# fboehm/DBSLMM

Hardware: AMD Instinct MI355X
Metric: SNPs solved/sec (whole node) + max-|Δβ| vs CPU ref, 1M SNP × 10k indiv (higher is better)
Workload: dtype f64

## Files before the change

dbslmm_amd/__init__.py:

```python
from __future__ import annotations

import ctypes as C
from dataclasses import dataclass, field

import numpy as np

from . import _lib
from ._lib import (WORKLOAD_LEN, BLOCK_EMPTY, BLOCK_MONOMORPHIC, BLOCK_NOT_CONVERGED, BLOCK_NOT_PD,
                   BLOCK_OK, KERNEL_NAMES, SOLVER_AUTO, SOLVER_FACTOR, SOLVER_PCG, DbslmmError)

__all__ = ["Context", "Plan", "DBSLMMFIT", "BlockProblem", "bed_maf", "read_snp_std", "valid_blocks",
           "DbslmmError", "BLOCK_OK", "BLOCK_EMPTY", "BLOCK_NOT_PD", "BLOCK_MONOMORPHIC",
           "BLOCK_NOT_CONVERGED", "KERNEL_NAMES", "SOLVER_AUTO", "SOLVER_FACTOR", "SOLVER_PCG"]


def _ptr(a):
    return None if a is None else a.ctypes.data_as(C.c_void_p)


class Context:

    def __init__(self, device=0):
        self.lib = _lib.load()
        h = C.c_void_p()
        if isinstance(device, (list, tuple)):
            ids = np.ascontiguousarray(device, dtype=np.int32)
            rc = self.lib.dbslmm_ctx_create_multi(len(ids), _ptr(ids), C.byref(h))
        else:
            rc = self.lib.dbslmm_ctx_create(int(device), C.byref(h))
        if rc != 0:
            raise DbslmmError(f"dbslmm_ctx_create(device={device}) failed rc={rc}")
        self.h = h
        self.device = device

    @property
    def num_devices(self) -> int:
        return int(self.lib.dbslmm_ctx_num_devices(self.h))

    def cache_bed(self, bed):
        if bed is None:
            self._cached_bed = None
            self.check(self.lib.dbslmm_ctx_cache_bed(self.h, None, 0), "ctx_cache_bed")
            return
        b = np.ascontiguousarray(bed, dtype=np.uint8)
        self.check(self.lib.dbslmm_ctx_cache_bed(self.h, _ptr(b), b.size), "ctx_cache_bed")
        self._cached_bed = b

    def row_stats(self, bed, n_ref: int, n_rows: int) -> np.ndarray:
        b = np.ascontiguousarray(bed, dtype=np.uint8)
        out = np.zeros((n_rows, 3), dtype=np.int32)
        self.check(self.lib.dbslmm_bed_row_stats(self.h, _ptr(b), b.size, n_ref, n_rows, _ptr(out)),
                   "bed_row_stats")
        return out

    def check(self, rc: int, what: str):
        if rc != 0:
            msg = self.lib.dbslmm_last_error(self.h).decode(errors="replace")
            raise DbslmmError(f"{what} failed rc={rc}: {msg}")

    def close(self):
        if self.h:
            self.lib.dbslmm_ctx_destroy(self.h)
            self.h = None

    def __del__(self):
        try:
            self.close()
        except Exception:
            pass


@dataclass
class BlockProblem:
    bed: np.ndarray
    n_ref: int
    n_obs: int
    sigma_s: float
    s_ptr: np.ndarray
    s_pos: np.ndarray
    z_s: np.ndarray
    l_ptr: np.ndarray | None = None
    l_pos: np.ndarray | None = None
    z_l: np.ndarray | None = None
    tau: float = 0.8
    opts: dict = field(default_factory=dict)

    def __post_init__(self):
        self.bed = np.ascontiguousarray(self.bed, dtype=np.uint8)
        self.s_ptr = np.ascontiguousarray(self.s_ptr, dtype=np.int64)
        self.s_pos = np.ascontiguousarray(self.s_pos, dtype=np.int32)
        self.z_s = np.ascontiguousarray(self.z_s, dtype=np.float64)
        if self.l_ptr is not None:
            self.l_ptr = np.ascontiguousarray(self.l_ptr, dtype=np.int64)
            self.l_pos = np.ascontiguousarray(self.l_pos, dtype=np.int32)
            self.z_l = np.ascontiguousarray(self.z_l, dtype=np.float64)
        nb = len(self.s_ptr) - 1
        if self.l_ptr is not None and len(self.l_ptr) != nb + 1:
            raise ValueError("s_ptr and l_ptr must have the same number of blocks")

    @property
    def num_block(self) -> int:
        return len(self.s_ptr) - 1

    @property
    def n_s(self) -> int:
        return int(self.s_ptr[-1])

    @property
    def n_l(self) -> int:
        return 0 if self.l_ptr is None else int(self.l_ptr[-1])

    def c_struct(self) -> _lib.Problem:
        unknown = set(self.opts) - {f[0] for f in _lib.Options._fields_}
        if unknown:
            raise ValueError(f"unknown dbslmm_options fields: {sorted(unknown)}")
        self._opts = _lib.Options(**self.opts)
        return _lib.Problem(
            _ptr(self.bed), self.bed.size, self.n_ref, self.n_obs, self.sigma_s, self.tau,
            self.num_block, _ptr(self.s_ptr), _ptr(self.s_pos), _ptr(self.z_s),
            _ptr(self.l_ptr), _ptr(self.l_pos), _ptr(self.z_l), C.pointer(self._opts))


class Plan:

    def __init__(self, ctx: Context, prob: BlockProblem):
        self.ctx, self.prob = ctx, prob
        self._cs = prob.c_struct()
        h = C.c_void_p()
        ctx.check(ctx.lib.dbslmm_plan_create(ctx.h, C.byref(self._cs), C.byref(h)), "plan_create")
        self.h = h

    @classmethod
    def units(cls, ctx: Context, prob: BlockProblem, unit_device, device_index: int):
        self = cls.__new__(cls)
        self.ctx, self.prob = ctx, prob
        ud = np.ascontiguousarray(unit_device, dtype=np.int32)
        if ud.ndim != 2 or ud.shape[0] != prob.num_block:
            raise ValueError("unit_device: [num_block, n_copies]")
        self._cs = prob.c_struct()
        self._ud = ud
        h = C.c_void_p()
        ctx.check(ctx.lib.dbslmm_plan_create_units(ctx.h, C.byref(self._cs), ud.shape[1], _ptr(ud),
                                                   int(device_index), C.byref(h)), "plan_create_units")
        self.h = h
        return self

    def run(self):
        self.ctx.check(self.ctx.lib.dbslmm_plan_run(self.h), "plan_run")

    def sync(self):
        self.ctx.check(self.ctx.lib.dbslmm_plan_sync(self.h), "plan_sync")

    def set_sigma(self, sigma_s: float):
        self.ctx.check(self.ctx.lib.dbslmm_plan_set_sigma(self.h, float(sigma_s)), "plan_set_sigma")

    def run_multi(self, sigmas, out=None):
        p = self.prob
        sig = np.ascontiguousarray(sigmas, dtype=np.float64)
        n = len(sig)
        if out is not None:
            bs, bl, st = out
            if (bs.shape != (n, p.n_s) or bl.shape != (n, p.n_l) or st.shape != (n, p.num_block)
                    or bs.dtype != np.float64 or bl.dtype != np.float64 or st.dtype != np.int32
                    or not all(a.flags.c_contiguous for a in out)):
                raise ValueError("out: C-contiguous float64 (n, n_s), (n, n_l) and int32 (n, num_block)")
        else:
            bs = np.zeros((n, p.n_s))
            bl = np.zeros((n, p.n_l))
            st = np.zeros((n, p.num_block), dtype=np.int32)
        self.ctx.check(self.ctx.lib.dbslmm_plan_run_multi(self.h, _ptr(sig), n, _ptr(bs), _ptr(bl),
                                                          _ptr(st)), "plan_run_multi")
        return [(bs[i], bl[i], st[i]) for i in range(n)]

    def enable_timing(self, on: bool = True):
        self.ctx.check(self.ctx.lib.dbslmm_plan_enable_timing(self.h, int(on)), "plan_enable_timing")

    def kernel_ms(self):
        out = np.zeros(len(KERNEL_NAMES))
        n = np.zeros(1, dtype=np.int32)
        self.ctx.check(self.ctx.lib.dbslmm_plan_kernel_ms(self.h, _ptr(out), _ptr(n)), "plan_kernel_ms")
        return out, int(n[0])

    def workload(self) -> dict:
        w = np.zeros(WORKLOAD_LEN)
        self.ctx.check(self.ctx.lib.dbslmm_plan_workload(self.h, _ptr(w)), "plan_workload")
        keys = ("snps", "unpack_read_bytes", "unpack_write_bytes", "gram_ops_alg",
                "gram_ops_exec", "chol_flops_large", "blocks", "gram_tiles", "chol_flops_small",
                "blocks_large", "chol_flops_tiled", "blocks_tiled", "tiled_launches", "trsv_bytes",
                "cheb_iters", "cheb_base", "h2f_pass_bytes", "pcg_route", "pcg_iters", "pcg_chip_bytes",
                "pcg_partial_bytes", "pcg_block_bytes")
        return dict(zip(keys, w.tolist()))

    def block_iters(self) -> np.ndarray:
        out = np.zeros(max(1, self.prob.num_block), dtype=np.int32)
        self.ctx.check(self.ctx.lib.dbslmm_plan_block_iters(self.h, _ptr(out)), "plan_block_iters")
        return out[:self.prob.num_block]

    def shard_info(self) -> np.ndarray:
        out = np.zeros(self.prob.num_block, dtype=np.int32)
        self.ctx.check(self.ctx.lib.dbslmm_plan_shard_info(self.h, _ptr(out)), "plan_shard_info")
        return out

    def block_matrix(self, block: int, copy: int = 0) -> np.ndarray:
        ld = C.c_int32()
        self.ctx.check(self.ctx.lib.dbslmm_plan_block_matrix(self.h, int(block), int(copy), None,
                                                             C.byref(ld)), "plan_block_matrix")
        out = np.empty((ld.value, ld.value))
        self.ctx.check(self.ctx.lib.dbslmm_plan_block_matrix(self.h, int(block), int(copy), _ptr(out),
                                                             None), "plan_block_matrix")
        return out

    def download(self):
        p = self.prob
        bs = np.zeros(p.n_s)
        bl = np.zeros(p.n_l)
        st = np.zeros(p.num_block, dtype=np.int32)
        self.ctx.check(self.ctx.lib.dbslmm_plan_download(self.h, _ptr(bs), _ptr(bl), _ptr(st)),
                       "plan_download")
        return bs, bl, st

    def variance(self, test_bed: np.ndarray, indicator, s_pos, l_pos=None) -> np.ndarray:
        tb = np.ascontiguousarray(test_bed, dtype=np.uint8)
        ind = np.ascontiguousarray(indicator, dtype=np.int32)
        sp = np.ascontiguousarray(s_pos, dtype=np.int32)
        lp = None if l_pos is None else np.ascontiguousarray(l_pos, dtype=np.int32)
        if sp.size != self.prob.n_s or (self.prob.n_l and (lp is None or lp.size != self.prob.n_l)):
            raise ValueError("test s_pos / l_pos must align with the plan's small / large SNPs")
        n_test = int((ind != 0).sum())
        out = np.zeros(n_test * self.prob.num_block)
        nt = np.zeros(1, dtype=np.int32)
        tp = _lib.TestPanel(_ptr(tb), tb.size, ind.size, _ptr(ind), _ptr(sp), _ptr(lp))
        self.ctx.check(self.ctx.lib.dbslmm_plan_variance(self.h, C.byref(tp), _ptr(out), _ptr(nt)),
                       "plan_variance")
        return out.reshape(self.prob.num_block, n_test).T

    def close(self):
        if self.h:
            self.ctx.lib.dbslmm_plan_destroy(self.h)
            self.h = None

    def __del__(self):
        try:
            self.close()
        except Exception:
            pass


class DBSLMMFIT:

    def __init__(self, device=0):
        self.ctx = Context(device)

    def est(self, prob: BlockProblem):
        bs = np.zeros(prob.n_s)
        bl = np.zeros(prob.n_l)
        st = np.zeros(prob.num_block, dtype=np.int32)
        cs = prob.c_struct()
        self.ctx.check(self.ctx.lib.dbslmm_est(self.ctx.h, C.byref(cs), _ptr(bs), _ptr(bl), _ptr(st)),
                       "dbslmm_est")
        return bs, bl, st


def bed_maf(ctx: Context, bed: np.ndarray, n_ref: int, n_snp: int) -> np.ndarray:
    bed = np.ascontiguousarray(bed, dtype=np.uint8)
    maf = np.zeros(n_snp)
    ctx.check(ctx.lib.dbslmm_bed_maf(ctx.h, _ptr(bed), bed.size, n_ref, n_snp, _ptr(maf)), "bed_maf")
    return maf


def read_snp_std(ctx: Context, bed: np.ndarray, n_ref: int, rows) -> tuple[np.ndarray, np.ndarray]:
    bed = np.ascontiguousarray(bed, dtype=np.uint8)
    rows = np.ascontiguousarray(rows, dtype=np.int32)
    out = np.zeros(n_ref * len(rows))
    maf = np.zeros(len(rows))
    ctx.check(ctx.lib.dbslmm_read_snp_std(ctx.h, _ptr(bed), bed.size, n_ref, _ptr(rows), len(rows),
                                          _ptr(out), _ptr(maf)), "read_snp_std")
    return out.reshape(len(rows), n_ref).T, maf


def valid_blocks(ctx: Context, bed: np.ndarray, n_ref: int, ptr, pos, z1, z2):
    bed = np.ascontiguousarray(bed, dtype=np.uint8)
    ptr = np.ascontiguousarray(ptr, dtype=np.int64)
    pos = np.ascontiguousarray(pos, dtype=np.int32)
    z1 = np.ascontiguousarray(z1, dtype=np.float64)
    z2 = np.ascontiguousarray(z2, dtype=np.float64)
    nb = len(ptr) - 1
    nume = np.zeros(nb)
    deno = np.zeros(nb)
    ctx.check(ctx.lib.dbslmm_valid_blocks(ctx.h, _ptr(bed), bed.size, n_ref, nb, _ptr(ptr), _ptr(pos),
                                          _ptr(z1), _ptr(z2), _ptr(nume), _ptr(deno)), "valid_blocks")
    return nume, deno
```

dbslmm_amd/_lib.py:

```python
from __future__ import annotations

import ctypes as C
import os

HERE = os.path.dirname(os.path.abspath(__file__))
LIB_PATH = os.path.join(HERE, "libdbslmm_hip.so")

EXPORTS = (
    "dbslmm_abi_version", "dbslmm_ctx_create", "dbslmm_ctx_destroy", "dbslmm_last_error",
    "dbslmm_est", "dbslmm_plan_create", "dbslmm_plan_run", "dbslmm_plan_sync",
    "dbslmm_plan_download", "dbslmm_plan_set_sigma", "dbslmm_plan_destroy", "dbslmm_plan_run_multi",
    "dbslmm_plan_enable_timing", "dbslmm_plan_kernel_ms", "dbslmm_plan_workload",
    "dbslmm_bed_maf", "dbslmm_read_snp_std", "dbslmm_valid_blocks", "dbslmm_plan_variance",
    "dbslmm_ctx_create_multi", "dbslmm_ctx_num_devices", "dbslmm_plan_shard_info",
    "dbslmm_ctx_cache_bed", "dbslmm_ctx_cache_bed_fd", "dbslmm_plan_block_matrix",
    "dbslmm_shard_plan", "dbslmm_plan_create_units", "dbslmm_shard_plan_problem",
    "dbslmm_plan_block_iters", "dbslmm_bed_row_stats",
)

ABI_VERSION = 16
K_UNPACK, K_GRAM, K_CHOL_LARGE, K_CHOL_SMALL, K_CHOL_TILED, K_TRSV, K_PCG, K_PCG_BLOCK = 0, 1, 2, 3, 4, 5, 6, 7
KERNEL_NAMES = ("dbslmm_unpack_stats", "dbslmm_gram", "dbslmm_chol_large", "dbslmm_chol_small",
                "dbslmm_tchol", "dbslmm_trsv", "dbslmm_pcg", "dbslmm_pcg_block")
WORKLOAD_LEN = 22
BLOCK_OK, BLOCK_EMPTY, BLOCK_NOT_PD, BLOCK_MONOMORPHIC, BLOCK_NOT_CONVERGED = 0, 1, 2, 3, 4
SOLVER_AUTO, SOLVER_FACTOR, SOLVER_PCG = 0, 1, 2


class Options(C.Structure):
    _fields_ = [
        ("tiled_min", C.c_int32), ("gram_big_min", C.c_int32), ("gram_huge_min", C.c_int32),
        ("h2f_mode", C.c_int32), ("cheb_tol", C.c_double), ("lead_min", C.c_int32),
        ("large_cheb", C.c_int32), ("cheb_fused", C.c_int32), ("debug_delay_us", C.c_int32),
        ("debug_stop", C.c_int32), ("sub_split", C.c_int32), ("sub_grid_lead", C.c_int32),
        ("sub_grid_rest", C.c_int32), ("shard_copies", C.c_int32), ("h2f_iter", C.c_int32),
        ("solver", C.c_int32), ("pcg_tol", C.c_double), ("pcg_maxit", C.c_int32),
        ("pcg_whole", C.c_int32),
    ]


class Problem(C.Structure):
    _fields_ = [
        ("bed", C.c_void_p), ("bed_len", C.c_int64), ("n_ref", C.c_int32), ("n_obs", C.c_int32),
        ("sigma_s", C.c_double), ("tau", C.c_double), ("num_block", C.c_int32),
        ("s_ptr", C.c_void_p), ("s_pos", C.c_void_p), ("z_s", C.c_void_p),
        ("l_ptr", C.c_void_p), ("l_pos", C.c_void_p), ("z_l", C.c_void_p),
        ("opts", C.POINTER(Options)),
    ]


class TestPanel(C.Structure):
    _fields_ = [
        ("bed", C.c_void_p), ("bed_len", C.c_int64), ("n_total", C.c_int32),
        ("indicator", C.c_void_p), ("s_pos", C.c_void_p), ("l_pos", C.c_void_p),
    ]


_lib = None


class DbslmmError(RuntimeError):
    pass


def load(path: str | None = None):
    global _lib
    if _lib is not None:
        return _lib
    p = path or os.environ.get("DBSLMM_LIB_PATH") or LIB_PATH
    if not os.path.exists(p):
        raise DbslmmError(f"{p} not found: build it with `python -c 'import __graft_entry__ as g; g.build()'`"
                          " (or `make -C dbslmm_amd/csrc`)")
    L = C.CDLL(p)
    V, P = C.c_void_p, C.POINTER
    L.dbslmm_abi_version.restype = C.c_int
    L.dbslmm_ctx_create.argtypes = [C.c_int, P(V)]
    L.dbslmm_ctx_create_multi.argtypes = [C.c_int32, V, P(V)]
    L.dbslmm_ctx_num_devices.argtypes = [V]
    L.dbslmm_plan_shard_info.argtypes = [V, V]
    L.dbslmm_ctx_destroy.argtypes = [V]
    L.dbslmm_ctx_destroy.restype = None
    L.dbslmm_last_error.argtypes = [V]
    L.dbslmm_last_error.restype = C.c_char_p
    L.dbslmm_est.argtypes = [V, P(Problem), V, V, V]
    L.dbslmm_plan_create.argtypes = [V, P(Problem), P(V)]
    L.dbslmm_plan_run.argtypes = [V]
    L.dbslmm_plan_sync.argtypes = [V]
    L.dbslmm_plan_download.argtypes = [V, V, V, V]
    L.dbslmm_plan_set_sigma.argtypes = [V, C.c_double]
    L.dbslmm_plan_run_multi.argtypes = [V, V, C.c_int32, V, V, V]
    L.dbslmm_plan_destroy.argtypes = [V]
    L.dbslmm_plan_destroy.restype = None
    L.dbslmm_plan_enable_timing.argtypes = [V, C.c_int]
    L.dbslmm_plan_kernel_ms.argtypes = [V, V, V]
    L.dbslmm_plan_workload.argtypes = [V, V]
    L.dbslmm_bed_maf.argtypes = [V, V, C.c_int64, C.c_int32, C.c_int64, V]
    L.dbslmm_bed_row_stats.argtypes = [V, V, C.c_int64, C.c_int32, C.c_int64, V]
    L.dbslmm_read_snp_std.argtypes = [V, V, C.c_int64, C.c_int32, V, C.c_int32, V, V]
    L.dbslmm_valid_blocks.argtypes = [V, V, C.c_int64, C.c_int32, C.c_int32, V, V, V, V, V, V]
    L.dbslmm_plan_variance.argtypes = [V, P(TestPanel), V, V]
    L.dbslmm_ctx_cache_bed.argtypes = [V, V, C.c_int64]
    L.dbslmm_ctx_cache_bed_fd.argtypes = [V, C.c_int, C.c_int64, V]
    L.dbslmm_shard_plan.argtypes = [C.c_int32, V, C.c_int32, C.c_int32, C.c_int32, V, V]
    L.dbslmm_plan_create_units.argtypes = [V, P(Problem), C.c_int32, V, C.c_int32, P(V)]
    L.dbslmm_shard_plan_problem.argtypes = [P(Problem), V, C.c_int32, C.c_int32, V, V]
    L.dbslmm_plan_block_iters.argtypes = [V, V]
    if hasattr(L, "dbslmm_plan_block_matrix"):
        L.dbslmm_plan_block_matrix.argtypes = [V, C.c_int32, C.c_int32, V, V]
    if L.dbslmm_abi_version() != ABI_VERSION:
        raise DbslmmError("ABI version mismatch")
    _lib = L
    return L
```

dbslmm_amd/csrc/pcg.hip:

```cpp
#include <hip/hip_runtime.h>
#include <stdint.h>

namespace pcg {
constexpr int kT = 128;
constexpr int kRunMax = 8;
constexpr int kMaxNC = 4;
constexpr int kWaves = 4;
constexpr int kVS = kT + 8;
constexpr int kNDot = 5;
constexpr int kQS = 8;
constexpr int kThreads = 256;
constexpr int kFTb = 8;
constexpr int kFRows = kFTb * kT;
constexpr int kFPer = kFRows / kThreads;
constexpr int wave_lds_doubles(int nc) { return 3 * nc * kVS + 4 * nc * 64; }
constexpr size_t lds_bytes(int nc) { return sizeof(double) * kWaves * wave_lds_doubles(nc); }
}

struct PcgBlk {
    int32_t blk, row0, m, ms;
    int32_t ld, Tb, Ns, sco;
    int64_t matoff, vo, po, dof;
    int64_t off16;
    int32_t nc;
    int32_t mshift;
    int32_t fused;
    int32_t pad_;
};

struct PcgArgs {
    const PcgBlk* blk;
    const uint16_t* G16;
    const double* M;
    const int32_t* flags;
    const double* S;
    const double* rsd;
    const double* z;
    const int32_t* slot_out;
    const int32_t* blk_id;
    const double* dshift;
    double *X, *R, *P, *Sv, *W;
    double* U;
    double* part;
    double* dot;
    double* qs;
    int32_t* cnv;
    int32_t* itb;
    int32_t* done;
    int32_t* active;
    double* beta_s;
    double* beta_l;
    int32_t* status;
    int64_t vstride;
    int64_t ns, nl, nbk;
    double tau, rn, c0, tol, inv_sqrt_n;
    int32_t ncopy;
    int32_t run;
    int32_t seed;
};

namespace pcg {

__device__ __forceinline__ void wave_fence() {
    __builtin_amdgcn_fence(__ATOMIC_RELEASE, "wavefront");
    __builtin_amdgcn_wave_barrier();
    __builtin_amdgcn_fence(__ATOMIC_ACQUIRE, "wavefront");
}

template <int Ctrl>
__device__ __forceinline__ double dpp_mov(double v) {
    const uint64_t b = __builtin_bit_cast(uint64_t, v);
    const int lo = __builtin_amdgcn_mov_dpp(static_cast<int>(b & 0xffffffffu), Ctrl, 0xf, 0xf, false);
    const int hi = __builtin_amdgcn_mov_dpp(static_cast<int>(b >> 32), Ctrl, 0xf, 0xf, false);
    return __builtin_bit_cast(double, (static_cast<uint64_t>(static_cast<uint32_t>(hi)) << 32) | static_cast<uint32_t>(lo));
}
template <int X>
__device__ __forceinline__ uint32_t swap_xor(uint32_t x, bool up) {
    if constexpr (X == 16) {
        const auto r = __builtin_amdgcn_permlane16_swap(x, x, false, false);
        return up ? r[0] : r[1];
    } else {
        const auto r = __builtin_amdgcn_permlane32_swap(x, x, false, false);
        return up ? r[0] : r[1];
    }
}
template <int X>
__device__ __forceinline__ double lane_xor(double v) {
#ifndef PCG_NO_DPP
    if constexpr (X == 1) return dpp_mov<0xB1>(v);
    else if constexpr (X == 2) return dpp_mov<0x4E>(v);
    else if constexpr (X == 4) return dpp_mov<0x1B>(dpp_mov<0x141>(v));
    else if constexpr (X == 8) return dpp_mov<0x128>(v);
#ifndef PCG_NO_PERMLANE
    else if constexpr (X == 16 || X == 32) {
        const uint64_t b = __builtin_bit_cast(uint64_t, v);
        const bool up = (__lane_id() & X) != 0;
        const uint32_t lo = swap_xor<X>(static_cast<uint32_t>(b & 0xffffffffu), up);
        const uint32_t hi = swap_xor<X>(static_cast<uint32_t>(b >> 32), up);
        return __builtin_bit_cast(double, (static_cast<uint64_t>(hi) << 32) | lo);
    }
#endif
    else
#endif
        return __shfl_xor(v, X);
}

template <int X2, int X1, int X0>
__device__ __forceinline__ double rscatter8(const double (&v)[8], int lane) {
    const bool h2 = (lane & X2) != 0, h1 = (lane & X1) != 0, h0 = (lane & X0) != 0;
    double u[4], w[2];
#pragma unroll
    for (int q = 0; q < 4; ++q) {
        const double send = h2 ? v[q] : v[q + 4], keep = h2 ? v[q + 4] : v[q];
        u[q] = keep + lane_xor<X2>(send);
    }
#pragma unroll
    for (int q = 0; q < 2; ++q) {
        const double send = h1 ? u[q] : u[q + 2], keep = h1 ? u[q + 2] : u[q];
        w[q] = keep + lane_xor<X1>(send);
    }
    const double send = h0 ? w[0] : w[1], keep = h0 ? w[1] : w[0];
    return keep + lane_xor<X0>(send);
}

__device__ __forceinline__ double wave_sum(double v) {
    v += lane_xor<32>(v);
    v += lane_xor<16>(v);
    v += lane_xor<8>(v);
    v += lane_xor<4>(v);
    v += lane_xor<2>(v);
    v += lane_xor<1>(v);
    return v;
}



__device__ __forceinline__ double ordered_sum(const double* __restrict__ p, int64_t st, int s0, int s1, double acc) {
    for (int s = s0; s < s1; s += 8) {
        double t[8];
#pragma unroll
        for (int u = 0; u < 8; ++u) t[u] = s + u < s1 ? p[static_cast<int64_t>(s + u) * st] : 0.0;
#pragma unroll
        for (int u = 0; u < 8; ++u) acc += t[u];
    }
    return acc;
}

__device__ __forceinline__ bool on_u16(const PcgArgs& a, const PcgBlk& B) {
    return a.G16 != nullptr && (a.flags[B.blk] & 1) == 0;
}

__device__ __forceinline__ double jdiag(const PcgArgs& a, const PcgBlk& B, int i, double dc) {
    return B.mshift ? 1.0 : i < B.ms ? a.c0 + dc : a.c0;
}
__device__ __forceinline__ double col_shift(const PcgArgs& a, const PcgBlk& B, int k) {
    return a.dshift[B.mshift ? a.seed : k];
}

__device__ __forceinline__ double cvt_lo(uint32_t w) {
    double g;
    uint32_t t;
    asm volatile("v_and_b32 %1, 0xffff, %2\n\tv_cvt_f64_u32 %0, %1" : "=v"(g), "=&v"(t) : "v"(w));
    return g;
}
__device__ __forceinline__ double cvt_hi(uint32_t w) {
    double g;
    uint32_t t;
    asm volatile("v_lshrrev_b32 %1, 16, %2\n\tv_cvt_f64_u32 %0, %1" : "=v"(g), "=&v"(t) : "v"(w));
    return g;
}

typedef uint32_t pcg_u4 __attribute__((ext_vector_type(4)));

__device__ __forceinline__ __amdgpu_buffer_rsrc_t g16_rsrc(const uint16_t* base, uint32_t bytes) {
    const uint64_t gb = reinterpret_cast<uint64_t>(base);
    const uint32_t lo = static_cast<uint32_t>(__builtin_amdgcn_readfirstlane(static_cast<int>(gb & 0xffffffffu)));
    const uint32_t hi = static_cast<uint32_t>(__builtin_amdgcn_readfirstlane(static_cast<int>(gb >> 32)));
    const int nb = __builtin_amdgcn_readfirstlane(static_cast<int>(bytes));
    return __builtin_amdgcn_make_buffer_rsrc(reinterpret_cast<void*>((static_cast<uint64_t>(hi) << 32) | lo),
                                             static_cast<short>(0), nb, 0x00020000);
}
constexpr uint32_t kG16Oob = 0x80000000u;

__device__ __forceinline__ void quad_mul16(const pcg_u4 (&raw)[8], bool diagq, int lane, int nc,
                                           const double* vI, const double* vJ, double* rsum, double* csum) {
    const int rg = lane >> 3, cg = lane & 7;
#pragma unroll 1
    for (int k = 0; k < nc; ++k) {
        double vi[8], vj[8], racc[8], cacc[8];
#pragma unroll
        for (int q = 0; q < 8; ++q) {
            vi[q] = vI[k * kVS + 8 * rg + q];
            vj[q] = vJ[k * kVS + 8 * cg + q];
            racc[q] = cacc[q] = 0.0;
        }
        if (!diagq) {
#pragma unroll
            for (int r = 0; r < 8; ++r)
#pragma unroll
                for (int c = 0; c < 8; ++c) {
                    const uint32_t w = raw[r][c >> 1];
                    const double g = (c & 1) ? cvt_hi(w) : cvt_lo(w);
                    racc[r] = __builtin_fma(g, vj[c], racc[r]);
                    cacc[c] = __builtin_fma(g, vi[r], cacc[c]);
                }
        } else {
#pragma unroll
            for (int r = 0; r < 8; ++r)
#pragma unroll
                for (int c = 0; c < 8; ++c) {
                    const uint32_t w = raw[r][c >> 1];
                    const double g = (c & 1) ? cvt_hi(w) : cvt_lo(w);
                    const int dd = 8 * (cg - rg) + c - r;
                    racc[r] = __builtin_fma(dd <= 0 ? g : 0.0, vj[c], racc[r]);
                    cacc[c] = __builtin_fma(dd < 0 ? g : 0.0, vi[r], cacc[c]);
                }
        }
        rsum[k * 64 + lane] += rscatter8<4, 2, 1>(racc, lane);
        csum[k * 64 + lane] += rscatter8<32, 16, 8>(cacc, lane);
    }
}

__device__ __forceinline__ void quad_mul64(const double* __restrict__ base, int64_t ld, int rows_ok, int cols_ok,
                                           bool diagq, int lane, int nc, const double* vI, const double* vJ,
                                           double* rsum, double* csum) {
    const int rg = lane >> 3, cg = lane & 7;
#pragma unroll 1
    for (int k = 0; k < nc; ++k) {
        double vi[8], vj[8], racc[8], cacc[8];
#pragma unroll
        for (int q = 0; q < 8; ++q) {
            vi[q] = vI[k * kVS + 8 * rg + q];
            vj[q] = vJ[k * kVS + 8 * cg + q];
            racc[q] = cacc[q] = 0.0;
        }
#pragma unroll 1
        for (int r = 0; r < 8; ++r)
#pragma unroll
            for (int c = 0; c < 8; ++c) {
                const double g = (r < rows_ok && c < cols_ok) ? base[r * ld + c] : 0.0;
                const int dd = 8 * (cg - rg) + c - r;
                const double gr = !diagq || dd <= 0 ? g : 0.0, gc = !diagq || dd < 0 ? g : 0.0;
#pragma unroll
                for (int q = 0; q < 8; ++q)
                    if (q == r) racc[q] = __builtin_fma(gr, vj[c], racc[q]);
                cacc[c] = __builtin_fma(gc, vi[r], cacc[c]);
            }
        rsum[k * 64 + lane] += rscatter8<4, 2, 1>(racc, lane);
        csum[k * 64 + lane] += rscatter8<32, 16, 8>(cacc, lane);
    }
}

__device__ __forceinline__ void stage_v(const PcgArgs& a, const PcgBlk& B, int T, int nc, int lane, double* v) {
    for (int k = 0; k < nc; ++k) {
        const double* src = a.U + k * a.vstride + B.vo + static_cast<int64_t>(T) * kT;
        const double x0 = src[lane], x1 = src[lane + 64];
        v[k * kVS + lane] = x0;
        v[k * kVS + lane + 64] = x1;
    }
}

__device__ __forceinline__ bool quad_active(const PcgBlk& B, int I, int J, int q) {
    const int qi = q >> 1, qj = q & 1;
    return !(J == I && qj > qi) && I * kT + 64 * qi < B.m && J * kT + 64 * qj < B.m;
}
__device__ __forceinline__ bool next_quad(const PcgBlk& B, int I, int J1, int& J, int& q) {
    for (;;) {
        if (++q == 4) {
            q = 0;
            if (++J > J1) return false;
        }
        if (quad_active(B, I, J, q)) return true;
    }
}

template <bool U16>
__device__ void symv_item(const PcgArgs& a, int4 item, int lane, double* vI, double* vJb, double* rsum,
                          double* csum) {
    const PcgBlk B = a.blk[item.x];
    if (a.done[item.x] || on_u16(a, B) != U16) return;
    const int I = item.y, J0 = item.z, J1 = item.w, nc = B.nc;
    const int64_t ld16 = static_cast<int64_t>(B.Tb) * kT;
    const int rg = lane >> 3, cg = lane & 7;
    auto vj_of = [&](int J) -> double* { return J == I ? vI : vJb + ((J - J0) & 1) * nc * kVS; };
    const __amdgpu_buffer_rsrc_t g16 =
        g16_rsrc(a.G16 + B.off16 + static_cast<int64_t>(I) * kT * ld16, U16 ? static_cast<uint32_t>(kT * ld16 * 2) : 0u);
    auto load = [&](int J, int q, pcg_u4 (&raw)[8], bool none) {
        if constexpr (U16) {
            const int i0 = 64 * (q >> 1) + 8 * rg, j0 = J * kT + 64 * (q & 1) + 8 * cg;
            const bool skip = none || j0 >= B.m || (J == I && (q == 0 || q == 3) && cg > rg);
            const uint32_t o = static_cast<uint32_t>((static_cast<int64_t>(i0) * ld16 + j0) * 2);
#pragma unroll
            for (int r = 0; r < 8; ++r)
                raw[r] = __builtin_amdgcn_raw_buffer_load_b128(
                    g16, (skip || I * kT + i0 + r >= B.m) ? kG16Oob : o + static_cast<uint32_t>(r * ld16 * 2), 0, 0);
        }
    };
    auto mult = [&](int J, int q, const pcg_u4 (&raw)[8]) {
        const int qi = q >> 1, qj = q & 1;
        const bool dq = J == I && qi == qj;
        const double* vj = vj_of(J);
        double* rs = rsum + qi * nc * 64;
        double* cs = csum + qj * nc * 64;
        if constexpr (U16) {
            quad_mul16(raw, dq, lane, nc, vI + 64 * qi, vj + 64 * qj, rs, cs);
        } else {
            const int ib = I * kT + 64 * qi + 8 * rg, jb = J * kT + 64 * qj + 8 * cg;
            quad_mul64(a.M + B.matoff + static_cast<int64_t>(ib) * B.ld + jb, B.ld, B.m - ib, B.m - jb, dq,
                       lane, nc, vI + 64 * qi, vj + 64 * qj, rs, cs);
        }
    };
    auto flush = [&](int J) {
        double* dst = a.part + B.po + (static_cast<int64_t>(J) * B.Ns + I) * nc * kT;
        for (int qj = 0; qj < 2; ++qj)
            for (int k = 0; k < nc; ++k) {
                dst[k * kT + 64 * qj + 8 * cg + rg] = csum[(qj * nc + k) * 64 + lane];
                csum[(qj * nc + k) * 64 + lane] = 0.0;
            }
    };
    pcg_u4 ra[8], rb[8];
    int J = J0, q = 0;
    load(J, q, ra, false);
    stage_v(a, B, I, nc, lane, vI);
    if (J != I) stage_v(a, B, J, nc, lane, vj_of(J));
    for (int t = 0; t < 2 * nc; ++t) rsum[t * 64 + lane] = csum[t * 64 + lane] = 0.0;
    wave_fence();
    auto step = [&](pcg_u4 (&cur)[8], pcg_u4 (&nxt)[8]) -> bool {
        int Jn = J, qn = q;
        const bool more = next_quad(B, I, J1, Jn, qn);
        load(more ? Jn : J, more ? qn : q, nxt, !more);
        if (more && Jn != J && Jn != I) stage_v(a, B, Jn, nc, lane, vj_of(Jn));
        mult(J, q, cur);
        if (!more || Jn != J) flush(J);
        wave_fence();
        J = Jn;
        q = qn;
        return more;
    };
    while (step(ra, rb) && step(rb, ra)) {
    }
    double* dst = a.part + B.po + (static_cast<int64_t>(I) * B.Ns + B.Tb + J0 / a.run) * nc * kT;
    for (int qi = 0; qi < 2; ++qi)
        for (int k = 0; k < nc; ++k) dst[k * kT + 64 * qi + 8 * rg + cg] = rsum[(qi * nc + k) * 64 + lane];
}

}

extern "C" __global__ __launch_bounds__(pcg::kThreads) void dbslmm_pcg_init(PcgArgs a, const int2* __restrict__ rows) {
    using namespace pcg;
    __shared__ double red[kThreads / 64][kMaxNC];
    __shared__ int mono_s;
    const int2 it = rows[blockIdx.x];
    const int bi = it.x, I = it.y, tid = threadIdx.x;
    const PcgBlk B = a.blk[bi];
    const bool u16 = on_u16(a, B);
    const int n = a.ncopy, nc = B.nc;
    if (I == 0) {
        if (tid == 0) mono_s = 0;
        __syncthreads();
        bool mono = false;
        for (int i = tid; i < B.m; i += kThreads) mono |= !(a.rsd[B.row0 + i] < INFINITY);
        if (mono) atomicOr(&mono_s, 1);
        __syncthreads();
        if (tid < n) {
            a.cnv[B.sco + tid] = 0;
            double* q = a.qs + static_cast<int64_t>(B.sco + tid) * kQS;
            q[4] = q[5] = 1.0;
        }
        if (tid == 0) {
            a.itb[bi] = 0;
            const bool fz = B.fused && u16;
            a.done[bi] = mono_s ? 2 : fz ? 3 : 0;
            if (!mono_s && !fz) atomicAdd(a.active, 1);
        }
    }
    const int r = tid & (kT - 1), h = tid >> 7, i = I * kT + r;
    const bool in = i < B.m;
    double sv[kMaxNC];
#pragma unroll
    for (int k = 0; k < kMaxNC; ++k) sv[k] = 0.0;
    for (int c = h; c < n; c += 2) {
        const int64_t o = c * a.vstride + B.vo + i;
        const double rhs = in ? a.z[B.row0 + i] : 0.0;
        a.X[o] = 0.0;
        a.P[o] = 0.0;
        if (c < nc) {
            a.Sv[o] = 0.0;
            a.W[o] = 0.0;
            a.R[o] = rhs;
            double uv = 0.0;
            if (in) {
                uv = rhs / jdiag(a, B, i, col_shift(a, B, c));
                if (u16) uv *= a.rsd[B.row0 + i];
            }
            a.U[o] = uv;
        }
    }
#pragma unroll
    for (int k = 0; k < kMaxNC; ++k)
        if (k < nc && (k & 1) == h && in && u16) {
            const double rhs = a.z[B.row0 + i];
            sv[k] = a.S[B.row0 + i] * a.rsd[B.row0 + i] * (rhs / jdiag(a, B, i, col_shift(a, B, k)));
        }
#pragma unroll
    for (int k = 0; k < kMaxNC; ++k) sv[k] = wave_sum(sv[k]);
    if ((tid & 63) == 0)
#pragma unroll
        for (int k = 0; k < kMaxNC; ++k) red[tid >> 6][k] = sv[k];
    __syncthreads();
    if (tid < nc) {
        const int hk = tid & 1;
        a.dot[B.dof + (static_cast<int64_t>(I) * kNDot + 4) * n + tid] = red[2 * hk][tid] + red[2 * hk + 1][tid];
    }
}

template <bool U16>
__device__ __forceinline__ void symv_body(const PcgArgs& a, const int4* __restrict__ items, int32_t n_items) {
    using namespace pcg;
    extern __shared__ double vlds[];
    const int wave = threadIdx.x >> 6, lane = threadIdx.x & 63;
    const int e = blockIdx.x * kWaves + wave;
    if (e >= n_items) return;
    const int nc = a.ncopy;
    double* w = vlds + wave * wave_lds_doubles(nc);
    symv_item<U16>(a, items[e], lane, w, w + nc * kVS, w + 3 * nc * kVS, w + 3 * nc * kVS + 2 * nc * 64);
}
#ifndef PCG_SYMV_WAVES
#define PCG_SYMV_WAVES 2
#endif
extern "C" __global__ __launch_bounds__(pcg::kThreads) __attribute__((amdgpu_waves_per_eu(PCG_SYMV_WAVES, 8)))
void dbslmm_pcg_symv16(PcgArgs a, const int4* __restrict__ items, int32_t n_items) {
    symv_body<true>(a, items, n_items);
}
extern "C" __global__ __launch_bounds__(pcg::kThreads)
void dbslmm_pcg_symv64(PcgArgs a, const int4* __restrict__ items, int32_t n_items) {
    symv_body<false>(a, items, n_items);
}

extern "C" __global__ __launch_bounds__(pcg::kThreads) void dbslmm_pcg_rows(PcgArgs a, const int2* __restrict__ rows) {
    using namespace pcg;
    __shared__ double red[kThreads / 64][kMaxNC][4];
    __shared__ double sig[kMaxNC];
    const int2 it = rows[blockIdx.x];
    const int bi = it.x, I = it.y, tid = threadIdx.x;
    if (a.done[bi]) return;
    const PcgBlk B = a.blk[bi];
    const bool u16 = on_u16(a, B);
    const int n = a.ncopy, nc = B.nc;
    if (tid < nc)
        sig[tid] = ordered_sum(a.dot + B.dof + 4 * n + tid, kNDot * n, 0, B.Tb, 0.0);
    __syncthreads();
    const int r = tid & (kT - 1), h = tid >> 7, i = I * kT + r;
    const bool in = i < B.m;
    const double Si = in ? a.S[B.row0 + i] : 0.0, ri = in ? a.rsd[B.row0 + i] : 0.0;
    const int nrun = (I + a.run) / a.run;
    double dv[kMaxNC][4];
#pragma unroll
    for (int k = 0; k < kMaxNC; ++k)
#pragma unroll
        for (int f = 0; f < 4; ++f) dv[k][f] = 0.0;
#pragma unroll
    for (int k = 0; k < kMaxNC; ++k) {
        if (k >= n || (k & 1) != h) continue;
        const int64_t o = k * a.vstride + B.vo + i;
        if (k < nc) {
            const double* pp = a.part + B.po + static_cast<int64_t>(I) * B.Ns * nc * kT + k * kT + r;
            double y = ordered_sum(pp, nc * kT, I, B.Tb, 0.0);
            y = ordered_sum(pp, nc * kT, B.Tb, B.Tb + nrun, y);
            const double dc = col_shift(a, B, k);
            const double rv = a.R[o];
            const double u = in ? rv / jdiag(a, B, i, dc) : 0.0;
            const double sh = i < B.ms ? dc : 0.0;
            double w = 0.0;
            if (in) {
                if (u16) w = a.tau * a.rn * ri * __builtin_fma(-Si, sig[k] * a.rn, y) + (1.0 - a.tau + sh) * u;
                else w = y + sh * u;
            }
            a.W[o] = w;
            dv[k][0] = rv * u;
            dv[k][1] = w * u;
            dv[k][2] = rv * rv;
        }
        const double xv = a.X[o];
        dv[k][3] = xv * xv;
    }
#pragma unroll
    for (int k = 0; k < kMaxNC; ++k)
#pragma unroll
        for (int f = 0; f < 4; ++f) dv[k][f] = wave_sum(dv[k][f]);
    if ((tid & 63) == 0)
#pragma unroll
        for (int k = 0; k < kMaxNC; ++k)
#pragma unroll
            for (int f = 0; f < 4; ++f) red[tid >> 6][k][f] = dv[k][f];
    __syncthreads();
    if (tid < 4 * n) {
        const int k = tid >> 2, f = tid & 3, hk = k & 1;
        if (f == 3 || k < nc)
            a.dot[B.dof + (static_cast<int64_t>(I) * kNDot + f) * n + k] = red[2 * hk][k][f] + red[2 * hk + 1][k][f];
    }
    if (I == 0 && tid == 0) a.itb[bi] += 1;
}

extern "C" __global__ __launch_bounds__(pcg::kThreads) void dbslmm_pcg_update(PcgArgs a, const int2* __restrict__ rows) {
    using namespace pcg;
    __shared__ double tot[kMaxNC][4];
    __shared__ double coef[kMaxNC][3];
    __shared__ double seedc[2];
    __shared__ int run_s[kMaxNC];
    __shared__ double red[kThreads / 64][kMaxNC];
    const int2 it = rows[blockIdx.x];
    const int bi = it.x, I = it.y, tid = threadIdx.x;
    if (a.done[bi]) return;
    const PcgBlk B = a.blk[bi];
    const bool u16 = on_u16(a, B);
    const int n = a.ncopy, nc = B.nc;
    const int itn = a.itb[bi] - 1;
    const int par = itn & 1;
    if (tid < 4 * n) {
        const int k = tid >> 2, f = tid & 3;
        tot[k][f] = (f == 3 || k < nc) ? ordered_sum(a.dot + B.dof + f * n + k, kNDot * n, 0, B.Tb, 0.0) : 0.0;
    }
    __syncthreads();
    if (B.mshift) {
        if (tid == 0) {
            const double gam = tot[0][0], del = tot[0][1];
            const double* q = a.qs + static_cast<int64_t>(B.sco) * kQS;
            double al, be = 0.0;
            if (itn == 0) {
                al = gam / del;
            } else {
                be = gam / q[2 * par];
                al = gam / (del - be * gam / q[2 * par + 1]);
            }
            seedc[0] = al;
            seedc[1] = be;
        }
        __syncthreads();
        if (tid < n) {
            const int c = tid;
            double* q = a.qs + static_cast<int64_t>(B.sco + c) * kQS;
            const double al = seedc[0], be = seedc[1];
            const double zk = q[4 + 2 * par], zk1 = q[4 + 2 * par + 1];
            const double rr = tot[0][2] * zk * zk, xx = tot[c][3];
            const double t = a.tol * (a.dshift[c] + 1.0 - a.tau);
            const bool conv = a.cnv[B.sco + c] != 0 || rr == 0.0 || rr <= t * t * xx;
            const double e = a.dshift[c] - a.dshift[a.seed];
            const double cp = itn == 0 ? 0.0 : al * be / a.qs[static_cast<int64_t>(B.sco) * kQS + 2 * par + 1];
            const double zn = zk * zk1 / ((1.0 + cp + al * e) * zk1 - cp * zk);
            coef[c][0] = al * zn / zk;
            coef[c][1] = zk1 != 0.0 ? (zk / zk1) * (zk / zk1) * be : 0.0;
            coef[c][2] = zk;
            run_s[c] = conv ? 0 : 1;
            if (I == 0) {
                if (conv && a.cnv[B.sco + c] == 0) a.cnv[B.sco + c] = itn + 1;
                q[4 + 2 * (par ^ 1)] = zn;
                q[4 + 2 * (par ^ 1) + 1] = zk;
            }
        }
        __syncthreads();
        if (I == 0 && tid == 0) {
            double* q = a.qs + static_cast<int64_t>(B.sco) * kQS;
            q[2 * (par ^ 1)] = tot[0][0];
            q[2 * (par ^ 1) + 1] = seedc[0];
        }
    } else {
        if (tid < n) {
            const int k = tid;
            const double gam = tot[k][0], del = tot[k][1], rr = tot[k][2], xx = tot[k][3];
            const double lam = B.ms == B.m ? a.dshift[k] + 1.0 - a.tau : 1.0 - a.tau;
            const double t = a.tol * lam;
            const bool conv = a.cnv[B.sco + k] != 0 || rr == 0.0 || rr <= t * t * xx;
            double al = 0.0, be = 0.0;
            if (!conv) {
                double* q = a.qs + static_cast<int64_t>(B.sco + k) * kQS;
                if (itn == 0) {
                    al = gam / del;
                } else {
                    be = gam / q[2 * par];
                    al = gam / (del - be * gam / q[2 * par + 1]);
                }
                if (I == 0) {
                    q[2 * (par ^ 1)] = gam;
                    q[2 * (par ^ 1) + 1] = al;
                }
            } else if (I == 0 && a.cnv[B.sco + k] == 0) {
                a.cnv[B.sco + k] = itn + 1;
            }
            coef[k][0] = al;
            coef[k][1] = be;
            coef[k][2] = 1.0;
            run_s[k] = conv ? 0 : 1;
        }
        __syncthreads();
    }
    int running = 0;
    for (int k = 0; k < n; ++k) running += run_s[k];
    if (running == 0) {
        if (I == 0 && tid == 0) {
            a.done[bi] = 1;
            atomicSub(a.active, 1);
        }
        return;
    }
    const int r = tid & (kT - 1), h = tid >> 7, i = I * kT + r;
    const bool in = i < B.m;
    double sv[kMaxNC];
#pragma unroll
    for (int k = 0; k < kMaxNC; ++k) sv[k] = 0.0;
    if (B.mshift) {
        if (in) {
            const int64_t o0 = B.vo + i;
            const double rv = a.R[o0];
#pragma unroll
            for (int c = 0; c < kMaxNC; ++c) {
                if (c >= n || (c & 1) != h || !run_s[c]) continue;
                const int64_t o = c * a.vstride + o0;
                const double p = __builtin_fma(coef[c][1], a.P[o], coef[c][2] * rv);
                a.P[o] = p;
                a.X[o] = __builtin_fma(coef[c][0], p, a.X[o]);
            }
            if (h == 0) {
                const double al = seedc[0], be = seedc[1];
                const double sn = __builtin_fma(be, a.Sv[o0], a.W[o0]);
                const double rn = __builtin_fma(-al, sn, rv);
                a.Sv[o0] = sn;
                a.R[o0] = rn;
                a.U[o0] = u16 ? rn * a.rsd[B.row0 + i] : rn;
                if (u16) sv[0] = a.S[B.row0 + i] * a.rsd[B.row0 + i] * rn;
            }
        }
    } else {
#pragma unroll
        for (int k = 0; k < kMaxNC; ++k) {
            if (k >= n || (k & 1) != h || !run_s[k] || !in) continue;
            const int64_t o = k * a.vstride + B.vo + i;
            const double al = coef[k][0], be = coef[k][1];
            const double dg = jdiag(a, B, i, a.dshift[k]);
            const double u = a.R[o] / dg;
            const double p = __builtin_fma(be, a.P[o], u);
            const double s = __builtin_fma(be, a.Sv[o], a.W[o]);
            const double x = __builtin_fma(al, p, a.X[o]);
            const double rn = __builtin_fma(-al, s, a.R[o]);
            a.P[o] = p;
            a.Sv[o] = s;
            a.X[o] = x;
            a.R[o] = rn;
            a.U[o] = u16 ? (rn / dg) * a.rsd[B.row0 + i] : rn / dg;
            if (u16) sv[k] = a.S[B.row0 + i] * a.rsd[B.row0 + i] * (rn / dg);
        }
    }
#pragma unroll
    for (int k = 0; k < kMaxNC; ++k) sv[k] = wave_sum(sv[k]);
    if ((tid & 63) == 0)
#pragma unroll
        for (int k = 0; k < kMaxNC; ++k) red[tid >> 6][k] = sv[k];
    __syncthreads();
    if (tid < nc && (B.mshift || run_s[tid])) {
        const int hk = tid & 1;
        a.dot[B.dof + (static_cast<int64_t>(I) * kNDot + 4) * n + tid] = red[2 * hk][tid] + red[2 * hk + 1][tid];
    }
}

#ifndef PCG_BLOCK_DEPTH
#define PCG_BLOCK_DEPTH 3
#endif
namespace pcg {
template <int N>
__device__ __forceinline__ void block_sum(double (&v)[N], double* red, int tid) {
#pragma unroll
    for (int k = 0; k < N; ++k) v[k] = wave_sum(v[k]);
    __syncthreads();
    if ((tid & 63) == 0)
#pragma unroll
        for (int k = 0; k < N; ++k) red[(tid >> 6) * N + k] = v[k];
    __syncthreads();
#pragma unroll
    for (int k = 0; k < N; ++k) v[k] = ((red[k] + red[N + k]) + red[2 * N + k]) + red[3 * N + k];
}
constexpr size_t block_lds_bytes(int n) {
    return sizeof(double) * ((5 + 2 * n) * kFRows + 4 * (3 + kMaxNC) + 12 + 3 * kMaxNC + 4);
}
}

__device__ __forceinline__ void pcg_block_solve(const PcgArgs& a, int bi, int cc, int32_t maxit) {
    using namespace pcg;
    extern __shared__ double blds[];
    double* yw = blds;
    double* Ul = blds + 4 * kFRows;
    const int n = a.ncopy;
    double* Xl = Ul + kFRows;
    double* Pl = Xl + n * kFRows;
    double* red = Pl + n * kFRows;
    if (a.done[bi] != 3) return;
    const PcgBlk B = a.blk[bi];
    const int tid = threadIdx.x, lane = tid & 63, wave = tid >> 6;
    const int m = B.m, Tb = B.Tb;
    const bool msh = cc < 0;
    const int nx = msh ? n : 1;
    const double dc = msh ? col_shift(a, B, 0) : a.dshift[cc];
    double r[kFPer], sv[kFPer], wv[kFPer], Sr[kFPer], Rr[kFPer], sg[1] = {0.0};
#pragma unroll
    for (int q = 0; q < kFPer; ++q) {
        const int i = tid + kThreads * q;
        const bool in = i < m;
        r[q] = in ? a.z[B.row0 + i] : 0.0;
        Sr[q] = in ? a.S[B.row0 + i] : 0.0;
        Rr[q] = in ? a.rsd[B.row0 + i] : 0.0;
        sv[q] = wv[q] = 0.0;
        double u = 0.0;
        if (in) {
            u = (r[q] / jdiag(a, B, i, dc)) * Rr[q];
            sg[0] += Sr[q] * u;
        }
        Ul[i] = u;
        for (int w = 0; w < 4; ++w) yw[w * kFRows + i] = 0.0;
        for (int c = 0; c < nx; ++c) Xl[c * kFRows + i] = Pl[c * kFRows + i] = 0.0;
    }
    block_sum(sg, red, tid);
    double sig = sg[0];
    const int Q = (m + 63) / 64;
    const int nq = Q * (Q + 1) / 2;
    const int64_t ld16 = static_cast<int64_t>(Tb) * kT;
    const int rg = lane >> 3, cg = lane & 7;
    auto quad_of = [&](int t, int& qi, int& qj) {
        qi = static_cast<int>((sqrtf(8.0f * t + 1.0f) - 1.0f) * 0.5f);
        while (qi * (qi + 1) / 2 > t) --qi;
        while ((qi + 1) * (qi + 2) / 2 <= t) ++qi;
        qj = t - qi * (qi + 1) / 2;
    };
    const __amdgpu_buffer_rsrc_t g16 = g16_rsrc(a.G16 + B.off16, static_cast<uint32_t>(ld16 * ld16 * 2));
    auto load = [&](int t, pcg_u4 (&raw)[8]) {
        int qi, qj;
        quad_of(t, qi, qj);
        const int r0 = 64 * qi + 8 * rg, c0 = 64 * qj + 8 * cg;
        const bool skip = t >= nq || c0 >= m || (qi == qj && cg > rg);
        const uint32_t o = static_cast<uint32_t>((r0 * static_cast<int>(ld16) + c0) * 2);
#pragma unroll
        for (int rr = 0; rr < 8; ++rr)
            raw[rr] = __builtin_amdgcn_raw_buffer_load_b128(
                g16, (skip || r0 + rr >= m) ? kG16Oob : o + static_cast<uint32_t>(rr * ld16 * 2), 0, 0);
    };
    auto mult = [&](int t, const pcg_u4 (&raw)[8]) {
        int qi, qj;
        quad_of(t, qi, qj);
        const bool dq = qi == qj;
        double vi[8], vj[8], racc[8], cacc[8];
#pragma unroll
        for (int q = 0; q < 8; ++q) {
            vi[q] = Ul[64 * qi + 8 * rg + q];
            vj[q] = Ul[64 * qj + 8 * cg + q];
            racc[q] = cacc[q] = 0.0;
        }
        if (!dq) {
// ... 36 lines not shown
    for (; it < maxit; ++it) {
        __syncthreads();
        {
#if PCG_BLOCK_DEPTH == 3
            pcg_u4 ra[8], rb[8], rc[8];
            int t = wave;
            load(t, ra);
            load(t + 4, rb);
            while (t < nq) {
                load(t + 8, rc);
                mult(t, ra);
                t += 4;
                if (t >= nq) break;
                load(t + 8, ra);
                mult(t, rb);
                t += 4;
                if (t >= nq) break;
                load(t + 8, rb);
                mult(t, rc);
                t += 4;
            }
#else
            pcg_u4 ra[8], rb[8];
            int t = wave;
            load(t, ra);
            while (t < nq) {
                load(t + 4, rb);
                mult(t, ra);
                t += 4;
                if (t >= nq) break;
                load(t + 4, ra);
                mult(t, rb);
                t += 4;
            }
#endif
        }
        __syncthreads();
        double d[3 + kMaxNC];
#pragma unroll
        for (int k = 0; k < 3 + kMaxNC; ++k) d[k] = 0.0;
#pragma unroll
        for (int q = 0; q < kFPer; ++q) {
            const int i = tid + kThreads * q;
            double y = 0.0;
            if (i < Tb * kT) {
                y = ((yw[i] + yw[kFRows + i]) + yw[2 * kFRows + i]) + yw[3 * kFRows + i];
#pragma unroll
                for (int w = 0; w < 4; ++w) yw[w * kFRows + i] = 0.0;
            }
            if (i < m) {
                const double Si = Sr[q], ri = Rr[q];
                const double u = r[q] / jdiag(a, B, i, dc);
                const double sh = i < B.ms ? dc : 0.0;
                const double w = a.tau * a.rn * ri * __builtin_fma(-Si, sig * a.rn, y) + (1.0 - a.tau + sh) * u;
                wv[q] = w;
                d[0] += r[q] * u;
                d[1] += w * u;
                d[2] += r[q] * r[q];
                for (int c = 0; c < nx; ++c) {
                    const double xv = Xl[c * kFRows + i];
                    d[3 + c] += xv * xv;
                }
            }
        }
        block_sum(d, red, tid);
        if (tid == 0) {
            const double gam = d[0], del = d[1], rr = d[2];
            double al, be = 0.0;
            if (it == 0) {
                al = gam / del;
            } else {
                be = gam / st[0];
                al = gam / (del - be * gam / st[1]);
            }
            int running = 0;
            if (msh) {
                const double cp = it == 0 ? 0.0 : al * be / st[1];
                for (int c = 0; c < n; ++c) {
                    const double zk = st[4 + c], zk1 = st[8 + c];
                    const double t = a.tol * (a.dshift[c] + 1.0 - a.tau);
                    const double rrc = rr * zk * zk;
                    if (!flag[c] && (rrc == 0.0 || rrc <= t * t * d[3 + c])) {
                        flag[c] = 1;
                        a.cnv[B.sco + c] = it + 1;
                    }
                    const double e = a.dshift[c] - a.dshift[a.seed];
                    const double zn = zk * zk1 / ((1.0 + cp + al * e) * zk1 - cp * zk);
                    st[12 + 3 * c] = al * zn / zk;
                    st[12 + 3 * c + 1] = zk1 != 0.0 ? (zk / zk1) * (zk / zk1) * be : 0.0;
                    st[12 + 3 * c + 2] = zk;
                    st[8 + c] = zk;
                    st[4 + c] = zn;
                    running += flag[c] ? 0 : 1;
                }
            } else {
                const double lam = B.ms == B.m ? dc + 1.0 - a.tau : 1.0 - a.tau;
                const double t = a.tol * lam;
                if (rr == 0.0 || rr <= t * t * d[3]) {
                    flag[0] = 1;
                    a.cnv[B.sco + cc] = it + 1;
                }
                running = flag[0] ? 0 : 1;
            }
            st[0] = gam;
            st[1] = al;
            st[2] = al;
            st[3] = be;
            flag[kMaxNC] = running;
        }
        __syncthreads();
        if (flag[kMaxNC] == 0) break;
        const double al = st[2], be = st[3];
        double sg2[1] = {0.0};
#pragma unroll
        for (int q = 0; q < kFPer; ++q) {
            const int i = tid + kThreads * q;
            if (i >= m) continue;
            const double rsd_i = Rr[q];
            double rn;
            if (msh) {
                for (int c = 0; c < n; ++c) {
                    if (flag[c]) continue;
                    const int o = c * kFRows + i;
                    const double pv = __builtin_fma(st[12 + 3 * c + 1], Pl[o], st[12 + 3 * c + 2] * r[q]);
                    Pl[o] = pv;
                    Xl[o] = __builtin_fma(st[12 + 3 * c], pv, Xl[o]);
                }
                const double sn = __builtin_fma(be, sv[q], wv[q]);
                rn = __builtin_fma(-al, sn, r[q]);
                sv[q] = sn;
                r[q] = rn;
                Ul[i] = rn * rsd_i;
            } else {
                const double dg = jdiag(a, B, i, dc);
                const double u = r[q] / dg;
                const double pv = __builtin_fma(be, Pl[i], u);
                const double sn = __builtin_fma(be, sv[q], wv[q]);
                Pl[i] = pv;
                Xl[i] = __builtin_fma(al, pv, Xl[i]);
                rn = __builtin_fma(-al, sn, r[q]);
                sv[q] = sn;
                r[q] = rn;
                Ul[i] = (rn / dg) * rsd_i;
            }
            sg2[0] += Sr[q] * Ul[i];
        }
        block_sum(sg2, red, tid);
        sig = sg2[0];
    }
#pragma unroll
    for (int q = 0; q < kFPer; ++q) {
        const int i = tid + kThreads * q;
        if (i < m)
            for (int c = 0; c < nx; ++c) a.X[(msh ? c : cc) * a.vstride + B.vo + i] = Xl[c * kFRows + i];
    }
    if (tid == 0) atomicMax(a.itb + bi, it + (it < maxit ? 1 : 0));
}

extern "C" __global__ __launch_bounds__(pcg::kThreads)
#if PCG_BLOCK_DEPTH == 3
__attribute__((amdgpu_waves_per_eu(1, 8), amdgpu_num_vgpr(312)))
#else
__attribute__((amdgpu_waves_per_eu(2, 8)))
#endif
void dbslmm_pcg_block(PcgArgs a, const int2* __restrict__ list, int32_t n_list, int32_t* __restrict__ next,
                      int32_t maxit) {
    __shared__ int e_s;
    for (;;) {
        __syncthreads();
        if (threadIdx.x == 0) e_s = atomicAdd(next, 1);
        __syncthreads();
        const int e = e_s;
        if (e >= n_list) break;
        pcg_block_solve(a, list[e].x, list[e].y, maxit);
    }
}

extern "C" __global__ __launch_bounds__(pcg::kThreads) void dbslmm_pcg_final(PcgArgs a, const int2* __restrict__ rows) {
    using namespace pcg;
    const int2 it = rows[blockIdx.x];
    const int bi = it.x, I = it.y, tid = threadIdx.x;
    const PcgBlk B = a.blk[bi];
    const bool mono = a.done[bi] == 2;
    const int r = tid & (kT - 1), h = tid >> 7, i = I * kT + r;
    if (i < B.m) {
        const int so = a.slot_out[B.row0 + i];
        for (int k = h; k < a.ncopy; k += 2) {
            const double bv = mono ? __builtin_nan("") : a.X[k * a.vstride + B.vo + i] * a.inv_sqrt_n;
            if (so >= 0) a.beta_s[k * a.ns + so] = bv;
            else a.beta_l[k * a.nl - 1 - so] = bv;
        }
    }
    if (I == 0 && tid < a.ncopy) {
        const int st = mono ? DBSLMM_BLOCK_MONOMORPHIC
                            : a.cnv[B.sco + tid] == 0 ? DBSLMM_BLOCK_NOT_CONVERGED : DBSLMM_BLOCK_OK;
        a.status[tid * a.nbk + a.blk_id[B.blk]] = st;
    }
}
```

dbslmm_amd/csrc/plan.hip:

```cpp
#include <hip/hip_runtime.h>
#include <unistd.h>

#include <algorithm>
#include <atomic>
#include <cmath>
#include <condition_variable>
#include <cstdio>
#include <cstdlib>
#include <cstring>
#include <numeric>
#include <string>
#include <memory>
#include <mutex>
#include <chrono>
#include <thread>
#include <unordered_map>
#include <vector>

#include "../../include/dbslmm_hip.h"

#include "kernels.hip"
#include "chol.hip"
#include "chol_tiled.hip"
#include "variance.hip"
#include "trsv.hip"
#include "pcg.hip"

namespace {
constexpr int kEvPerRun = 12;
constexpr size_t kCholLargeLds = sizeof(double) * chol::kLargeDoubles;
constexpr size_t kCholChebLds = sizeof(double) * chol::kChebLdsDoubles;
constexpr size_t kTiledLds = sizeof(double) * chol::kTiledDoubles;
constexpr size_t kRegionLds = sizeof(double) * chol::kRegionDoubles;
constexpr size_t kTrail3Lds = sizeof(double) * chol::kTrail3k16Doubles;
constexpr int kTiledMinDefault = 384;
constexpr int kTiledMinSmall = 256;
constexpr int kBedPad = 64;
constexpr int kGramBigMinDefault = 96;
constexpr int kGramHugeMinDefault = 384;
constexpr int kTChebMaxM = 4096;
constexpr int kLeadMinDefault = 1536;
constexpr int kXcd = 8;
constexpr int kEpochsPerRun = 1 << 14;

struct TLaunch {
    int kind;
    int step;
    int32_t off;
    int32_t n;
    int32_t items;
    int32_t nk = 1;
    int strm = 0;
};
constexpr int kTlRecord = 6, kTlWait = 7;
constexpr int kSuper = 2;
constexpr int kWideSuper = 4;
constexpr int kWideMin = 4096;
constexpr int kTiledMaxM = 255 * 128;
constexpr int kGramSq = 4;
constexpr int kTrailSq = 8;

int64_t round_up(int64_t x, int64_t a) { return (x + a - 1) / a * a; }
struct PanelImage {
    std::shared_ptr<uint8_t> mem;
    int64_t pitch = 0;
    int32_t n_rows = 0, n_ref = 0;
    int64_t image_bytes() const { return (static_cast<int64_t>(n_rows) + 1) * pitch; }
    const v4i* rows() const { return reinterpret_cast<const v4i*>(mem.get() + image_bytes()); }
};
std::mutex g_capture_mu;
}

struct dbslmm_ctx {
    int device = 0;
    hipStream_t stream = nullptr;
    hipStream_t stream2 = nullptr;
    hipStream_t stream3 = nullptr;
    hipStream_t stream4 = nullptr, stream5 = nullptr;
    hipEvent_t fork = nullptr, join = nullptr, join3 = nullptr, fork2 = nullptr, join4 = nullptr;
    int n_cu = 256;
    std::string err;
    const uint8_t* bed_host = nullptr;
    int64_t bed_host_len = 0;
    std::shared_ptr<uint8_t> bed_cache;
    PanelImage img_cache;
    bool bed_from_fd = false;
    std::vector<dbslmm_ctx*> subs;
    std::thread setup;
    std::mutex setup_mu;
    bool setup_ok = true;
};
struct dbslmm_plan;
struct DeviceShard {
    dbslmm_plan* plan = nullptr;
    dbslmm_ctx* ctx = nullptr;
    dbslmm_ctx* own_ctx = nullptr;
    int device_index = 0;
    int copy = -1;
    std::vector<int32_t> blocks;
    std::vector<int64_t> s_idx, l_idx;
    std::vector<int> run_copies;
    std::vector<double> dl_s, dl_l;
    std::vector<int32_t> dl_st;
};
struct dbslmm_mplan {
    std::vector<DeviceShard> shards;
    int32_t n_copies = 1;
    bool partial = false;
    std::vector<int32_t> unit_device;
};

struct dbslmm_plan {
    dbslmm_ctx* ctx = nullptr;
    dbslmm_mplan* mp = nullptr;
    int32_t n_ref = 0, n_obs = 0, num_block = 0;
    double sigma_s = 0.0, tau = 0.8;
    int64_t n_s = 0, n_l = 0, kpad = 0, bed_len = 0;
    int32_t n_slots = 0, n_nonempty = 0, n_tiles = 0;
    int64_t M_elems = 0;
    PanelImage img;
    const uint8_t* d_img = nullptr;
    int32_t *d_slot_pos = nullptr, *d_slot_block = nullptr, *d_slot_out = nullptr;
    double *d_z = nullptr, *d_S = nullptr, *d_mu = nullptr, *d_rsd = nullptr, *d_y = nullptr;
    int32_t *d_flags = nullptr, *d_status = nullptr, *d_order = nullptr, *d_blk_id = nullptr;
    int32_t n_large = 0, n_small = 0;
    int32_t n_tiled = 0;
    int32_t* d_tlist = nullptr;
    std::vector<TLaunch> tl;
    std::vector<TLaunch> tl_rest;
    hipGraphExec_t graph_exec = nullptr;
    int32_t *d_row0 = nullptr, *d_m = nullptr, *d_ms = nullptr, *d_ld = nullptr;
    int64_t* d_matoff = nullptr;
    GramTile* d_tiles = nullptr;
    GramTile* d_btiles = nullptr;
    int32_t n_btiles = 0;
    GramTile* d_htiles = nullptr;
    int32_t n_htiles = 0;
    int32_t n_htiles_lead = 0;
    int32_t n_htiles_tiled = 0;
    bool early_fork = false;
    double* d_M = nullptr;
    double *d_beta_s = nullptr, *d_beta_l = nullptr;
    double* d_dshift = nullptr;
    int32_t n_copies = 0;
    int64_t nbk = 1;
    std::vector<TLaunch> tl_multi;
    int32_t* d_tlist_multi = nullptr;
    int32_t multi_n = 0;
    hipGraphExec_t graph_multi = nullptr;
    int32_t var_copy = 0;
    std::vector<int32_t> h_ld;
    std::vector<int32_t> h_m;
    std::vector<int32_t> h_tb;
    std::vector<int32_t> h_empty;
    std::vector<int32_t> h_blk_id;
    std::vector<int64_t> h_matoff;
    void* h_pin = nullptr;
    size_t h_pin_bytes = 0;
    std::vector<int32_t> h_slot_out;
    double sigma_run = 0.0;
    double wl[DBSLMM_WORKLOAD_LEN] = {0};
    bool timing = false;
    std::vector<hipEvent_t> ev;
    std::vector<hipEvent_t> dl_ev;
    std::vector<hipEvent_t> tev;
    std::vector<hipEvent_t> tev_rest;
    int32_t *d_tri_f = nullptr, *d_tri_b = nullptr, *d_foff = nullptr, *d_tflags = nullptr, *d_tb = nullptr;
    int32_t n_titems = 0, n_tflags = 0;
    int32_t* d_tepi = nullptr;
    int32_t* d_cheb_items = nullptr;
    int32_t n_cheb_items = 0, cheb_items_K = -1;
    int32_t trsv_epoch = 0;
    int32_t tiled_min = 0;
    int32_t h2f_mode = 0;
    double cheb_tol = 1e-9;
    bool large_cheb_ok = true;
    bool cheb_fused = false;
    bool h2f_cg = false;
    double* d_cgrec = nullptr;
    int32_t* d_cgconv = nullptr;
    int32_t* d_cgit = nullptr;
    bool cg_ran = false;
    int32_t debug_delay_us = 0;
    int32_t debug_stop = 0;
    int64_t n_runs = 0;
    bool sub_split = false;
    int32_t n_titems_lead = 0, n_tb_lead = 0, sub_grid_lead = 0, sub_grid_rest = 0;
    bool sub_block = false;
    int32_t* d_tcheb_blocks = nullptr;
    int32_t n_tcheb = 0, tcheb_vld = 0;
    bool trsv_pending = false;
    bool trsv_failed = false;
    unsigned long long* d_stamps = nullptr;
    double* d_cheb = nullptr;
    double* d_coef = nullptr;
    int32_t coef_cap = 0;
    std::vector<double> h_coef;
    std::vector<hipGraphExec_t> graph_copy;
    std::vector<hipGraphExec_t> graph_rest;
    int32_t cheb_base = -1;
    bool cheb_pending_var = false;
    int runs_pending = 0;
    double ms_acc[DBSLMM_K_COUNT] = {0, 0, 0, 0, 0, 0};
    int32_t ms_runs = 0;
    bool ran = false;
    bool stopped = false;
    int32_t m_copies = 0;
    std::vector<int32_t> h_ms, h_row0;
    bool has_large = false;
    int32_t solver = 0;
    double pcg_tol = 1e-12;
    int32_t pcg_maxit = 1000;
    bool force_factor = false;
    bool pcg_g16 = false;
    int32_t pcg_m_blocks = -1;
    uint16_t* d_G16 = nullptr;
    int64_t* d_off16 = nullptr;
    int32_t* d_ld16 = nullptr;
    std::vector<int64_t> h_off16;
    int32_t pcg_n = 0;
    PcgBlk* d_pblk = nullptr;
    int4* d_pitem = nullptr;
    int2* d_prow = nullptr;
    int32_t n_pblk = 0, n_pitem = 0, n_prow = 0;
    int32_t n_pitem_chip = 0, n_prow_chip = 0;
    bool pcg_trim = false;
    int32_t pcg_run = pcg::kRunMax;
    bool pcg_fused = true;
    int2* d_pflist = nullptr;
    int32_t* d_pfnext = nullptr;
    int32_t n_pflist = 0;
    std::vector<char> h_pfused;
    std::vector<int32_t> h_pnseq;
    bool pcg_join = false;
    double *d_pvec = nullptr, *d_ppart = nullptr, *d_pdot = nullptr, *d_pqs = nullptr;
    int32_t *d_pcnv = nullptr, *d_pitb = nullptr, *d_pdone = nullptr, *d_pact = nullptr;
    int64_t pcg_vstride = 0;
    int32_t* h_pmon = nullptr;
    int32_t pcg_it = 0;
    int32_t pcg_need = -1;
    int32_t pcg_iters_max = 0;
    bool pcg_pending = false;
    bool pcg_ran = false;
    bool pcg_pending_var = false;
    std::vector<char> run_route;
    std::vector<double> h_pmat, h_ppart;
    std::vector<char> h_pmiss;
    double pcg_cbytes = 0.0, pcg_pbytes = 0.0, pcg_fbytes = 0.0;
    PcgArgs pcg_args{};
    hipEvent_t pcg_ev_end = nullptr;
};

#define HIP_TRY(ctx, expr)                                                               \
    do {                                                                                 \
        hipError_t e_ = (expr);                                                          \
        if (e_ != hipSuccess) {                                                          \
            (ctx)->err = std::string(#expr) + " (plan.hip:" + std::to_string(__LINE__) + "): " + \
                         hipGetErrorString(e_);                                          \
            return DBSLMM_E_HIP;                                                         \
        }                                                                                \
    } while (0)

#define ARG_CHECK(ctx, cond, msg)                   \
    do {                                            \
        if (!(cond)) {                              \
            (ctx)->err = msg;                       \
            return DBSLMM_E_ARG;                    \
        }                                           \
    } while (0)

static bool key_of_other_n_ref(dbslmm_ctx* ctx, const uint8_t* bed, int64_t bed_len, int32_t n_ref) {
    if (!ctx->bed_from_fd || bed != ctx->bed_host || bed_len != ctx->bed_host_len || ctx->bed_cache ||
        !ctx->img_cache.mem || ctx->img_cache.n_ref == n_ref)
        return false;
    ctx->err = "the image cached from a file descriptor was built for n_ref = " +
               std::to_string(ctx->img_cache.n_ref) + "; cache it again to use n_ref = " + std::to_string(n_ref);
    return true;
}
#define KEY_CHECK(ctx, bed, bed_len, nref)                                              \
    do {                                                                                \
        if (key_of_other_n_ref(ctx, bed, bed_len, nref)) return DBSLMM_E_STATE;         \
    } while (0)

static int mp_create(dbslmm_ctx* ctx, const dbslmm_problem* pr, dbslmm_plan** out);
static void mp_destroy(dbslmm_plan* p);
static int mp_download(dbslmm_plan* p, int copy, double* beta_s, double* beta_l, int32_t* block_status);
static int mp_download_all(dbslmm_plan* p, int n, double* beta_s, double* beta_l, int32_t* block_status);
static int mp_run(dbslmm_plan* p, const double* sigmas, int n, bool wait);
static int mp_sync(dbslmm_plan* p);
static int mp_block_iters(dbslmm_plan* p, int32_t* iters);
static int mp_variance(dbslmm_plan* p, const dbslmm_test_panel* tp, double* diags, int32_t* n_test_out);
static int mp_bed_maf(dbslmm_ctx* ctx, const uint8_t* bed, int32_t n_ref, int64_t n_snp, double* maf);
#define ON_FIRST_DEVICE(ctx, call)                                       \
    do {                                                                 \
        if (!(ctx)->subs.empty()) {                                      \
            dbslmm_ctx* ctx0_ = (ctx)->subs[0];                          \
            const int rc_ = call;                                        \
            if (rc_ != DBSLMM_OK) (ctx)->err = ctx0_->err;               \
            return rc_;                                                  \
        }                                                                \
    } while (0)

template <class P>
static void backoff_wait(P pred) {
    for (int i = 0; !pred(); ++i) {
        if (i < 256) std::this_thread::yield();
        else std::this_thread::sleep_for(std::chrono::microseconds(20));
    }
}

template <class Fill>
static hipError_t upload_pipelined(void* dst, size_t n, hipStream_t st, Fill fill) {
    constexpr size_t kChunk = size_t(16) << 20;
    constexpr int kStageBufs = 4;
    void* stage[kStageBufs] = {};
    hipEvent_t done[kStageBufs] = {};
    hipError_t e = hipSuccess;
    for (int b = 0; b < kStageBufs && e == hipSuccess; ++b) {
        e = hipHostMalloc(&stage[b], kChunk, hipHostMallocDefault);
        if (e == hipSuccess) e = hipEventCreateWithFlags(&done[b], hipEventDisableTiming);
    }
    const unsigned T = std::max(1u, std::min(16u, std::thread::hardware_concurrency()));
    const size_t nchunk = (n + kChunk - 1) / kChunk;
    std::atomic<int64_t> go{-1};
    std::atomic<bool> bad{false}, stop{false};
    std::unique_ptr<std::atomic<unsigned>[]> parts(new std::atomic<unsigned>[nchunk]);
    for (size_t k = 0; k < nchunk; ++k) parts[k].store(0, std::memory_order_relaxed);
    std::vector<std::thread> th;
    if (e == hipSuccess)
        for (unsigned t = 0; t < T; ++t)
            th.emplace_back([&, t] {
                for (size_t k = 0; k < nchunk; ++k) {
                    backoff_wait([&] {
                        return go.load(std::memory_order_acquire) >= static_cast<int64_t>(k) ||
                               stop.load(std::memory_order_relaxed);
                    });
                    if (go.load(std::memory_order_acquire) < static_cast<int64_t>(k)) return;
                    const size_t off = k * kChunk, len = std::min(kChunk, n - off);
                    const size_t part = (len + T - 1) / T, a0 = std::min(len, t * part), z = std::min(len, a0 + part);
                    if (!(a0 >= z || fill(static_cast<char*>(stage[k % kStageBufs]) + a0, off + a0, z - a0)))
                        bad.store(true, std::memory_order_relaxed);
                    parts[k].fetch_add(1, std::memory_order_release);
                }
            });
    int64_t released = -1;
    auto release_free = [&](size_t k) {
        for (size_t k2 = std::max<int64_t>(released + 1, k); k2 < std::min(nchunk, k + kStageBufs); ++k2) {
            if (k2 >= static_cast<size_t>(kStageBufs) && k2 != k &&
                hipEventQuery(done[k2 % kStageBufs]) != hipSuccess)
                break;
            released = static_cast<int64_t>(k2);
        }
        go.store(released, std::memory_order_release);
    };
    for (size_t k = 0; k < nchunk && e == hipSuccess; ++k) {
        const int b = static_cast<int>(k % kStageBufs);
        if (released < static_cast<int64_t>(k)) {
            if (k >= static_cast<size_t>(kStageBufs) && (e = hipEventSynchronize(done[b])) != hipSuccess) break;
            released = static_cast<int64_t>(k) - 1;
        }
        release_free(k);
        backoff_wait([&] { return parts[k].load(std::memory_order_acquire) == T; });
        if (bad.load(std::memory_order_relaxed)) { e = hipErrorInvalidValue; break; }
        const size_t off = k * kChunk, len = std::min(kChunk, n - off);
        e = hipMemcpyAsync(static_cast<char*>(dst) + off, stage[b], len, hipMemcpyHostToDevice, st);
        if (e == hipSuccess) e = hipEventRecord(done[b], st);
    }
    stop.store(true, std::memory_order_relaxed);
    for (auto& t : th) t.join();
    const hipError_t e2 = hipStreamSynchronize(st);
    for (int b = 0; b < kStageBufs; ++b) {
        if (done[b]) (void)hipEventDestroy(done[b]);
        if (stage[b]) (void)hipHostFree(stage[b]);
    }
    return e != hipSuccess ? e : e2;
}

static hipError_t upload_staged(void* dst, const void* src, size_t n, hipStream_t st) {
    if (n <= (size_t(128) << 20)) {
        const hipError_t e = hipMemcpyAsync(dst, src, n, hipMemcpyHostToDevice, st);
        return e != hipSuccess ? e : hipStreamSynchronize(st);
    }
    return upload_pipelined(dst, n, st, [src](char* d, size_t off, size_t len) {
        memcpy(d, static_cast<const char*>(src) + off, len);
        return true;
    });
}

static hipError_t upload_staged_fd(void* dst, int fd, size_t n, hipStream_t st) {
    if (n <= (size_t(32) << 20)) {
        std::vector<char> h(n);
        size_t got = 0;
        while (got < n) {
            const ssize_t r = pread(fd, h.data() + got, n - got, static_cast<off_t>(got));
            if (r <= 0) return hipErrorInvalidValue;
            got += static_cast<size_t>(r);
        }
        const hipError_t e = hipMemcpyAsync(dst, h.data(), n, hipMemcpyHostToDevice, st);
        return e != hipSuccess ? e : hipStreamSynchronize(st);
    }
    return upload_pipelined(dst, n, st, [fd](char* d, size_t off, size_t len) {
        size_t got = 0;
        while (got < len) {
            const ssize_t r = pread(fd, d + got, len - got, static_cast<off_t>(off + got));
            if (r <= 0) return false;
            got += static_cast<size_t>(r);
        }
        return true;
    });
}

static void par_memcpy(void* dst, const void* src, size_t n) {
    constexpr size_t kMin = size_t(2) << 20;
    const unsigned hw = std::max(1u, std::min(8u, std::thread::hardware_concurrency()));
    const unsigned nt = static_cast<unsigned>(std::min<size_t>(hw, std::max<size_t>(1, n / kMin)));
    if (nt <= 1) { if (n) memcpy(dst, src, n); return; }
    const size_t part = (n + nt - 1) / nt;
    std::vector<std::thread> th;
    for (unsigned t = 1; t < nt; ++t) {
        const size_t a = t * part, z = std::min(n, a + part);
        if (a < z) th.emplace_back([=] { memcpy(static_cast<char*>(dst) + a, static_cast<const char*>(src) + a, z - a); });
    }
    memcpy(dst, src, std::min(n, part));
    for (auto& t : th) t.join();
}

static hipError_t bed_to_device(dbslmm_ctx* ctx, uint8_t* dst, const uint8_t* bed, int64_t bed_len) {
    hipError_t e = hipMemsetAsync(dst + bed_len, 0, kBedPad, ctx->stream);
    if (e != hipSuccess) return e;
    e = hipStreamSynchronize(ctx->stream);
    return e != hipSuccess ? e : upload_staged(dst, bed, bed_len, ctx->stream);
}

static std::shared_ptr<uint8_t> dev_shared(uint8_t* d, int dev) {
    return std::shared_ptr<uint8_t>(d, [dev](uint8_t* q) {
        (void)hipSetDevice(dev);
        (void)hipFree(q);
    });
}

static hipError_t image_from_verbatim(dbslmm_ctx* ctx, const uint8_t* d_bed, int64_t bed_len, int32_t n_ref,
                                      PanelImage* out) {
    const int64_t bps = n_ref / 4 + (n_ref % 4 ? 1 : 0);
    const int64_t n_rows = (bed_len - 3) / bps;
    if (n_rows >= INT32_MAX) return hipErrorInvalidValue;
    const int64_t pitch = round_up(n_ref, gram::kKpadAlign) / 4;
    uint8_t* d = nullptr;
    hipError_t e = hipMalloc(&d, static_cast<size_t>(n_rows + 1) * (pitch + sizeof(v4i)));
    if (e != hipSuccess) return e;
    PanelImage im;
    im.mem = dev_shared(d, ctx->device);
    im.pitch = pitch;
    im.n_rows = static_cast<int32_t>(n_rows);
    im.n_ref = n_ref;
    hipLaunchKernelGGL(dbslmm_bed_repitch, dim3(static_cast<unsigned>((n_rows + 1 + 3) / 4)), dim3(256), 0,
                       ctx->stream, d_bed, n_ref, bps, im.n_rows, d, pitch, const_cast<v4i*>(im.rows()));
    if ((e = hipGetLastError()) != hipSuccess || (e = hipStreamSynchronize(ctx->stream)) != hipSuccess) return e;
    *out = std::move(im);
    return hipSuccess;
}

static hipError_t panel_image(dbslmm_ctx* ctx, const uint8_t* bed, int64_t bed_len, int32_t n_ref,
                              PanelImage* out) {
    if (bed == ctx->bed_host && bed_len == ctx->bed_host_len) {
        if (ctx->img_cache.mem && ctx->img_cache.n_ref == n_ref) {
            *out = ctx->img_cache;
            return hipSuccess;
        }
        if (ctx->bed_cache) {
            const hipError_t e = image_from_verbatim(ctx, ctx->bed_cache.get(), bed_len, n_ref, &ctx->img_cache);
            if (e != hipSuccess) return e;
            ctx->bed_cache.reset();
            *out = ctx->img_cache;
            return hipSuccess;
        }
    }
    uint8_t* d_bed = nullptr;
    hipError_t e = hipMalloc(&d_bed, bed_len + kBedPad);
    if (e != hipSuccess) return e;
    if ((e = bed_to_device(ctx, d_bed, bed, bed_len)) == hipSuccess) e = image_from_verbatim(ctx, d_bed, bed_len, n_ref, out);
    (void)hipFree(d_bed);
    return e;
}

template <typename T>
static hipError_t dev_upload(T** dst, const std::vector<T>& src, hipStream_t st) {
    size_t bytes = std::max<size_t>(sizeof(T), src.size() * sizeof(T));
    hipError_t e = hipMalloc(reinterpret_cast<void**>(dst), bytes);
    if (e != hipSuccess || src.empty()) return e;
    e = hipMemcpyAsync(*dst, src.data(), src.size() * sizeof(T), hipMemcpyHostToDevice, st);
    return e != hipSuccess ? e : hipStreamSynchronize(st);
}

static void build_tiled(const std::vector<int32_t>& mv, const std::vector<int32_t>& tb0, int copies,
                        int nb, std::vector<TLaunch>& tl, std::vector<int32_t>& tlist) {
    struct Blk { int32_t bq; int T64, Tz64, T2, Tz2, nr, R, S, off; };
    int Rmax = 1;
    const int run2 = chol::kRun2;
    std::vector<Blk> bl;
    int G = 0, Kmax = 0;
    for (int c = 0; c < copies; ++c)
        for (int32_t b : tb0) {
            Blk k;
            k.bq = b + c * nb;
            k.T64 = (mv[b] + chol::kBT - 1) / chol::kBT;
            k.Tz64 = mv[b] / chol::kBT;
            k.T2 = (mv[b] + 127) / 128;
            k.Tz2 = mv[b] / 128;
            k.nr = (k.T64 + 1) / 2;
            k.R = mv[b] >= kWideMin ? kWideSuper : kSuper;
            Rmax = std::max(Rmax, k.R);
            k.S = (k.nr + k.R - 1) / k.R;
            G = std::max(G, k.S);
            Kmax = std::max(Kmax, k.T64);
            bl.push_back(k);
        }
    for (auto& k : bl) k.off = 0;
    auto push_pairs = [&](int kind, const std::vector<int32_t>& v) {
        if (v.empty()) return;
        TLaunch L{kind, 0, static_cast<int32_t>(tlist.size()), static_cast<int32_t>(v.size() / 2),
                  static_cast<int32_t>(v.size() / 2)};
        tlist.insert(tlist.end(), v.begin(), v.end());
        tl.push_back(L);
    };
    auto region_launch = [&](const std::vector<int32_t>& v) { push_pairs(4, v); };
    auto panel_launch = [&](const std::vector<int32_t>& v) { push_pairs(1, v); };
    auto sync = [&](int kind, int ev, int strm) {
        TLaunch L{kind, ev, 0, 0, 0};
        L.strm = strm;
        tl.push_back(L);
    };
    auto trailing_launch = [&](std::vector<std::vector<int32_t>>& q, int run, int strm) {
        TLaunch L{5, 0, static_cast<int32_t>(tlist.size()), run, 0};
        L.strm = strm;
        size_t qmax = 0;
        for (const auto& v : q) qmax = std::max(qmax, v.size() / 2);
        for (size_t i = 0; i < qmax; ++i)
            for (int x = 0; x < kXcd; ++x) {
                if (2 * i < q[x].size()) {
                    tlist.push_back(q[x][2 * i]);
                    tlist.push_back(q[x][2 * i + 1]);
                } else {
                    tlist.push_back(-1);
                    tlist.push_back(0);
                }
            }
        L.items = static_cast<int32_t>((tlist.size() - L.off) / 2);
        if (L.items > 0) tl.push_back(L);
    };
    {
        std::vector<int32_t> v;
        for (const auto& k : bl)
            if (k.off == 0) { v.push_back(k.bq); v.push_back(0); }
        region_launch(v);
    }
    for (int g = 0; g < G; ++g) {
        auto active = [&](const Blk& k) { return g >= k.off && g - k.off < k.S; };
        std::vector<int32_t> v;
        for (const auto& k : bl)
            if (active(k)) {
                const int r0 = (g - k.off) * k.R;
                for (int i = 2 * r0 + 2; i <= k.Tz64; ++i) { v.push_back((k.bq << 16) | i); v.push_back(r0 << 8); }
            }
        panel_launch(v);
        for (int j = 1; j < Rmax; ++j) {
            std::vector<int32_t> rv, pv;
            for (const auto& k : bl)
                if (active(k) && j < k.R) {
                    const int r = (g - k.off) * k.R + j;
                    if (r >= k.nr) continue;
                    rv.push_back(k.bq);
                    rv.push_back((r << 8) | j);
                    for (int i = 2 * r + 2; i <= k.Tz64; ++i) { pv.push_back((k.bq << 16) | i); pv.push_back((r << 8) | j); }
                }
            region_launch(rv);
            panel_launch(pv);
// ... 92 lines not shown
        return DBSLMM_E_HIP;
    }
    return DBSLMM_OK;
}

extern "C" {

int dbslmm_abi_version(void) { return DBSLMM_ABI_VERSION; }

int dbslmm_ctx_create(int device, dbslmm_ctx** out) {
    if (!out) return DBSLMM_E_ARG;
    *out = nullptr;
    int n = 0;
    if (hipGetDeviceCount(&n) != hipSuccess || n <= 0) return DBSLMM_E_HIP;
    if (device < 0 || device >= n) return DBSLMM_E_ARG;
    auto* c = new dbslmm_ctx();
    c->device = device;
    if (hipSetDevice(device) != hipSuccess ||
        hipStreamCreateWithFlags(&c->stream, hipStreamNonBlocking) != hipSuccess ||
        hipDeviceGetAttribute(&c->n_cu, hipDeviceAttributeMultiprocessorCount, device) != hipSuccess) {
        dbslmm_ctx_destroy(c);
        return DBSLMM_E_HIP;
    }
    c->setup = std::thread([c, device] {
        int prio_lo = 0, prio_hi = 0;
        c->setup_ok =
            hipSetDevice(device) == hipSuccess &&
            hipDeviceGetStreamPriorityRange(&prio_lo, &prio_hi) == hipSuccess &&
            hipStreamCreateWithPriority(&c->stream2, hipStreamNonBlocking, prio_hi) == hipSuccess &&
            hipStreamCreateWithPriority(&c->stream3, hipStreamNonBlocking, prio_hi) == hipSuccess &&
            hipStreamCreateWithFlags(&c->stream4, hipStreamNonBlocking) == hipSuccess &&
            hipStreamCreateWithFlags(&c->stream5, hipStreamNonBlocking) == hipSuccess &&
            hipEventCreateWithFlags(&c->fork, hipEventDisableTiming) == hipSuccess &&
            hipEventCreateWithFlags(&c->fork2, hipEventDisableTiming) == hipSuccess &&
            hipEventCreateWithFlags(&c->join4, hipEventDisableTiming) == hipSuccess &&
            hipEventCreateWithFlags(&c->join, hipEventDisableTiming) == hipSuccess &&
            hipEventCreateWithFlags(&c->join3, hipEventDisableTiming) == hipSuccess &&
            hipFuncSetAttribute(reinterpret_cast<const void*>(dbslmm_chol_large),
                                hipFuncAttributeMaxDynamicSharedMemorySize,
                                static_cast<int>(kCholLargeLds)) == hipSuccess &&
            hipFuncSetAttribute(reinterpret_cast<const void*>(dbslmm_chol_cheb),
                                hipFuncAttributeMaxDynamicSharedMemorySize,
                                static_cast<int>(kCholChebLds)) == hipSuccess &&
            hipFuncSetAttribute(reinterpret_cast<const void*>(dbslmm_gram_big),
                                hipFuncAttributeMaxDynamicSharedMemorySize, gram::kLdsBytes) == hipSuccess &&
            hipFuncSetAttribute(reinterpret_cast<const void*>(dbslmm_gram_huge),
                                hipFuncAttributeMaxDynamicSharedMemorySize, gram::kHLdsBytes) == hipSuccess &&
            hipFuncSetAttribute(reinterpret_cast<const void*>(dbslmm_pcg_block),
                                hipFuncAttributeMaxDynamicSharedMemorySize,
                                static_cast<int>(pcg::block_lds_bytes(pcg::kMaxNC))) == hipSuccess &&
            hipFuncSetAttribute(reinterpret_cast<const void*>(dbslmm_tchol_region),
                                hipFuncAttributeMaxDynamicSharedMemorySize,
                                static_cast<int>(kRegionLds)) == hipSuccess &&
            hipFuncSetAttribute(reinterpret_cast<const void*>(dbslmm_tchol_panel),
                                hipFuncAttributeMaxDynamicSharedMemorySize,
                                static_cast<int>(kTiledLds)) == hipSuccess &&
            hipFuncSetAttribute(reinterpret_cast<const void*>(dbslmm_tchol_trailing3k16),
                                hipFuncAttributeMaxDynamicSharedMemorySize,
                                static_cast<int>(kTrail3Lds)) == hipSuccess &&
            set_trsv_lds<1>() == hipSuccess && set_trsv_lds<2>() == hipSuccess;
        double* d_warm = nullptr;
        if (c->setup_ok && hipMalloc(&d_warm, sizeof(double)) == hipSuccess) {
            hipLaunchKernelGGL(dbslmm_set_scalar, dim3(1), dim3(1), 0, c->stream2, d_warm, 0.0);
            c->setup_ok = hipStreamSynchronize(c->stream2) == hipSuccess;
            (void)hipFree(d_warm);
        }
    });
    *out = c;
    return DBSLMM_OK;
}

void dbslmm_ctx_destroy(dbslmm_ctx* ctx) {
    if (!ctx) return;
    if (ctx->setup.joinable()) ctx->setup.join();
    for (dbslmm_ctx* s : ctx->subs) dbslmm_ctx_destroy(s);
    if (ctx->device < 0) {
        delete ctx;
        return;
    }
    (void)hipSetDevice(ctx->device);
    ctx->bed_cache.reset();
    ctx->img_cache = PanelImage{};
    if (ctx->stream) (void)hipStreamDestroy(ctx->stream);
    if (ctx->stream2) (void)hipStreamDestroy(ctx->stream2);
    if (ctx->stream3) (void)hipStreamDestroy(ctx->stream3);
    if (ctx->stream4) (void)hipStreamDestroy(ctx->stream4);
    if (ctx->stream5) (void)hipStreamDestroy(ctx->stream5);
    if (ctx->fork2) (void)hipEventDestroy(ctx->fork2);
    if (ctx->join4) (void)hipEventDestroy(ctx->join4);
    if (ctx->fork) (void)hipEventDestroy(ctx->fork);
    if (ctx->join) (void)hipEventDestroy(ctx->join);
    if (ctx->join3) (void)hipEventDestroy(ctx->join3);
    delete ctx;
}

const char* dbslmm_last_error(const dbslmm_ctx* ctx) { return ctx ? ctx->err.c_str() : "null context"; }

int dbslmm_ctx_cache_bed(dbslmm_ctx* ctx, const uint8_t* bed, int64_t bed_len) {
    if (!ctx) return DBSLMM_E_ARG;
    if (!ctx->subs.empty()) return DBSLMM_OK;
    ARG_CHECK(ctx, (bed == nullptr) == (bed_len == 0) && bed_len >= 0, "bed / bed_len");
    HIP_TRY(ctx, hipSetDevice(ctx->device));
    ctx->bed_cache.reset();
    ctx->img_cache = PanelImage{};
    ctx->bed_host = nullptr;
    ctx->bed_host_len = 0;
    ctx->bed_from_fd = false;
    if (!bed) return DBSLMM_OK;
    uint8_t* d = nullptr;
    HIP_TRY(ctx, hipMalloc(&d, bed_len + kBedPad));
    ctx->bed_cache = dev_shared(d, ctx->device);
    HIP_TRY(ctx, hipMemsetAsync(d + bed_len, 0, kBedPad, ctx->stream));
    HIP_TRY(ctx, upload_staged(d, bed, bed_len, ctx->stream));
    ctx->bed_host = bed;
    ctx->bed_host_len = bed_len;
    return DBSLMM_OK;
}

int dbslmm_ctx_cache_bed_fd(dbslmm_ctx* ctx, int fd, int64_t bed_len, const uint8_t* key) {
    if (!ctx) return DBSLMM_E_ARG;
    if (!ctx->subs.empty()) return DBSLMM_OK;
    ARG_CHECK(ctx, fd >= 0 && key && bed_len > 0, "fd / bed_len / key");
    HIP_TRY(ctx, hipSetDevice(ctx->device));
    ctx->bed_cache.reset();
    ctx->img_cache = PanelImage{};
    ctx->bed_host = nullptr;
    ctx->bed_host_len = 0;
    ctx->bed_from_fd = false;
    uint8_t* d = nullptr;
    HIP_TRY(ctx, hipMalloc(&d, bed_len + kBedPad));
    ctx->bed_cache = dev_shared(d, ctx->device);
    HIP_TRY(ctx, hipMemsetAsync(d + bed_len, 0, kBedPad, ctx->stream));
    if (upload_staged_fd(d, fd, static_cast<size_t>(bed_len), ctx->stream) != hipSuccess) {
        ctx->bed_cache.reset();
        ctx->err = "reading / uploading the .bed from its file descriptor failed";
        return DBSLMM_E_HIP;
    }
    ctx->bed_host = key;
    ctx->bed_host_len = bed_len;
    ctx->bed_from_fd = true;
    return DBSLMM_OK;
}

void dbslmm_plan_destroy(dbslmm_plan* p) {
    if (!p) return;
    if (p->mp) {
        mp_destroy(p);
        delete p;
        return;
    }
    (void)hipSetDevice(p->ctx->device);
    if (p->h_pin) (void)hipHostFree(p->h_pin);
    if (p->h_pmon) (void)hipHostFree(p->h_pmon);
    p->img = PanelImage{};
    void* bufs[] = {p->d_slot_pos, p->d_slot_block, p->d_slot_out, p->d_z,
                    p->d_S, p->d_mu, p->d_rsd, p->d_y, p->d_flags, p->d_status, p->d_order,
                    p->d_blk_id, p->d_row0, p->d_m, p->d_ms, p->d_ld, p->d_matoff, p->d_tiles,
                    p->d_M, p->d_beta_s, p->d_beta_l, p->d_tlist, p->d_btiles, p->d_htiles, p->d_dshift,
                    p->d_tlist_multi, p->d_tri_f, p->d_tri_b, p->d_foff, p->d_tflags, p->d_tb,
                    p->d_cheb, p->d_coef, p->d_stamps, p->d_tepi, p->d_cheb_items,
                    p->d_tcheb_blocks, p->d_cgrec, p->d_cgconv, p->d_cgit, p->d_G16, p->d_pblk,
                    p->d_pitem, p->d_prow, p->d_pvec, p->d_ppart, p->d_pdot, p->d_pqs, p->d_pcnv,
                    p->d_pitb, p->d_pdone, p->d_pact, p->d_off16, p->d_ld16, p->d_pflist, p->d_pfnext};
    for (void* b : bufs)
        if (b) {
            const hipError_t e = hipFree(b);
#ifdef DBSLMM_DIAG
            if (e != hipSuccess) fprintf(stderr, "plan_destroy: hipFree(%p) -> %s\n", b, hipGetErrorString(e));
#endif
            (void)e;
        }
    for (hipEvent_t e : p->ev) (void)hipEventDestroy(e);
    for (hipEvent_t e : p->dl_ev) (void)hipEventDestroy(e);
    for (hipEvent_t e : p->tev) (void)hipEventDestroy(e);
    for (hipEvent_t e : p->tev_rest) (void)hipEventDestroy(e);
    if (p->graph_exec) (void)hipGraphExecDestroy(p->graph_exec);
    if (p->graph_multi) (void)hipGraphExecDestroy(p->graph_multi);
    for (hipGraphExec_t g : p->graph_copy)
        if (g) (void)hipGraphExecDestroy(g);
    for (hipGraphExec_t g : p->graph_rest)
        if (g) (void)hipGraphExecDestroy(g);
    delete p;
}

int dbslmm_plan_create(dbslmm_ctx* ctx, const dbslmm_problem* pr, dbslmm_plan** out) {
    if (!ctx) return DBSLMM_E_ARG;
    if (!ctx->subs.empty()) return mp_create(ctx, pr, out);
    ARG_CHECK(ctx, pr && out, "null problem/out");
    *out = nullptr;
    if (const int rc = ctx_ready(ctx)) return rc;
    ARG_CHECK(ctx, pr->bed && pr->n_ref > 1 && pr->n_obs > 0 && pr->num_block >= 0, "bad sizes");
    ARG_CHECK(ctx, 9 * round_up(pr->n_ref, gram::kKpadAlign) < (int64_t(1) << 24),
              "n_ref must be at most 1,863,936 (exact FP4 Gram accumulation)");
    ARG_CHECK(ctx, pr->s_ptr && (pr->s_ptr[pr->num_block] == 0 || (pr->s_pos && pr->z_s)), "bad small CSR");
    ARG_CHECK(ctx, pr->sigma_s > 0.0 && std::isfinite(pr->sigma_s), "sigma_s must be > 0");
    const int64_t bps = pr->n_ref / 4 + (pr->n_ref % 4 ? 1 : 0);
    const int64_t n_snp_bed = (pr->bed_len - 3) / bps;
    ARG_CHECK(ctx, pr->bed_len >= 3 + bps, "bed image shorter than one SNP row");
    KEY_CHECK(ctx, pr->bed, pr->bed_len, pr->n_ref);
    const bool has_l = pr->l_ptr != nullptr;
    if (has_l) ARG_CHECK(ctx, pr->l_ptr[pr->num_block] == 0 || (pr->l_pos && pr->z_l), "bad large CSR");

    auto* p = new dbslmm_plan();
    p->ctx = ctx;
    p->n_ref = pr->n_ref;
    p->n_obs = pr->n_obs;
    p->num_block = pr->num_block;
    p->sigma_s = pr->sigma_s;
    p->tau = pr->tau;
    p->kpad = round_up(pr->n_ref, gram::kKpadAlign);
    p->bed_len = pr->bed_len;
    const dbslmm_options op = pr->opts ? *pr->opts : dbslmm_options{};
    ARG_CHECK(ctx, op.tiled_min >= 0 && op.gram_big_min >= 0 && op.gram_huge_min >= 0 &&
                   (op.h2f_mode == 0 || op.h2f_mode == 1) && op.cheb_tol >= 0.0 &&
                   (op.large_cheb == 0 || op.large_cheb == -1) && (op.cheb_fused == 0 || op.cheb_fused == 1) &&
                   op.debug_delay_us >= -100000 && op.debug_delay_us <= 100000 &&
                   (op.debug_stop == 0 || op.debug_stop == 1) && op.sub_split >= -1 && op.sub_split <= 2 &&
                   op.sub_grid_lead >= 0 && op.sub_grid_rest >= 0 && op.shard_copies >= 0 &&
                   op.shard_copies <= 64 && op.h2f_iter >= 0 && op.h2f_iter <= 2 && op.solver >= 0 &&
                   op.solver <= 2 && op.pcg_tol >= 0.0 && op.pcg_maxit >= 0, "bad dbslmm_options");
    p->solver = op.solver;
    p->pcg_fused = op.pcg_whole >= 0;
    if (op.pcg_tol > 0.0) p->pcg_tol = std::max(1e-15, op.pcg_tol);
    if (op.pcg_maxit > 0) p->pcg_maxit = op.pcg_maxit;
    p->pcg_g16 = 4 * static_cast<int64_t>(pr->n_ref) <= 65535;
    p->h2f_mode = op.h2f_mode;
    p->cheb_fused = op.cheb_fused == 1;
    p->h2f_cg = op.h2f_iter != 1;
    p->debug_delay_us = op.debug_delay_us;
    p->debug_stop = op.debug_stop;
    if (op.cheb_tol > 0.0) p->cheb_tol = std::max(1e-16, op.cheb_tol);
    p->n_s = pr->s_ptr[pr->num_block];
    p->n_l = has_l ? pr->l_ptr[pr->num_block] : 0;

    std::vector<int32_t> slot_pos, slot_block, slot_out, row0, mv, msv, ldv, blk_id;
    std::vector<double> z;
    std::vector<int64_t> matoff;
    std::vector<GramTile> tiles;
    const int64_t gram_big_min = op.gram_big_min > 0 ? op.gram_big_min : kGramBigMinDefault;
    const int64_t gram_huge_min = op.gram_huge_min > 0 ? op.gram_huge_min
                                  : p->kpad >= 4096 ? kGramHugeMinDefault : 2 * kGramHugeMinDefault;
    std::vector<std::vector<GramTile>> xq(kXcd), hq(kXcd), lq(kXcd), nq(kXcd);
    std::vector<double> xload(kXcd, 0.0), hload(kXcd, 0.0), lload(kXcd, 0.0), nload(kXcd, 0.0);
    int64_t moff = 0;
    double ops_alg = 0, ops_exec = 0, chol_flops_large = 0, chol_flops_small = 0, chol_flops_tiled = 0;
    int64_t tiled_min = kTiledMinDefault;
    if (op.tiled_min > 0) {
        tiled_min = std::max<int64_t>(64, op.tiled_min);
    } else {
        int64_t mmax = 0;
        for (int b = 0; b < pr->num_block; ++b)
            mmax = std::max<int64_t>(mmax, pr->s_ptr[b + 1] - pr->s_ptr[b] +
                                               (has_l ? pr->l_ptr[b + 1] - pr->l_ptr[b] : 0));
        if (mmax < 512) tiled_min = kTiledMinSmall;
    }
    p->tiled_min = static_cast<int32_t>(std::min<int64_t>(tiled_min, INT32_MAX));
    int64_t lead_min = INT64_MAX;
    {
        int64_t mmax = 0, n_lead = 0, n_rest = 0;
        for (int b = 0; b < pr->num_block; ++b)
            mmax = std::max<int64_t>(mmax, pr->s_ptr[b + 1] - pr->s_ptr[b] +
                                               (has_l ? pr->l_ptr[b + 1] - pr->l_ptr[b] : 0));
        if (op.lead_min >= 0) {
            lead_min = op.lead_min > 0 ? op.lead_min : std::max<int64_t>(kLeadMinDefault, mmax / 8);
            lead_min = std::max({lead_min, tiled_min, gram_huge_min});
            for (int b = 0; b < pr->num_block; ++b) {
                const int64_t m = pr->s_ptr[b + 1] - pr->s_ptr[b] + (has_l ? pr->l_ptr[b + 1] - pr->l_ptr[b] : 0);
                if (m >= lead_min) ++n_lead;
                else if (m >= tiled_min) ++n_rest;
            }
            if (n_lead == 0 || n_rest == 0) lead_min = INT64_MAX;
        }
    }
    std::vector<char> is_tiled;
    for (int b = 0; b < pr->num_block; ++b) {
        const int64_t s0 = pr->s_ptr[b], ms = pr->s_ptr[b + 1] - s0;
        const int64_t l0 = has_l ? pr->l_ptr[b] : 0, ml = has_l ? pr->l_ptr[b + 1] - l0 : 0;
        if (ms < 0 || ml < 0) { ctx->err = "CSR offsets not monotone"; dbslmm_plan_destroy(p); return DBSLMM_E_ARG; }
        const int64_t m = ms + ml;
        if (m == 0) { p->h_empty.push_back(b); continue; }
        const int nb = static_cast<int>(row0.size());
        const bool tiled = m >= tiled_min;
        if (tiled && (m >= kTiledMaxM || nb >= 32767)) {
            ctx->err = "LD block too large for the tiled path (m must be < 32640 SNPs)";
            dbslmm_plan_destroy(p);
            return DBSLMM_E_ARG;
        }
        is_tiled.push_back(tiled);
        const int64_t ld = round_up(m + 1, tiled ? 2 * chol::kBT : kTile);
        row0.push_back(static_cast<int32_t>(slot_pos.size()));
        mv.push_back(static_cast<int32_t>(m));
        msv.push_back(static_cast<int32_t>(ms));
        ldv.push_back(static_cast<int32_t>(ld));
        blk_id.push_back(b);
        matoff.push_back(moff);
        moff += ld * ld;
        for (int64_t i = 0; i < ms; ++i) {
            const int32_t r = pr->s_pos[s0 + i];
            if (r < 0 || r >= n_snp_bed) { ctx->err = "small SNP bed row out of range"; dbslmm_plan_destroy(p); return DBSLMM_E_ARG; }
            slot_pos.push_back(r);
            slot_block.push_back(nb);
            slot_out.push_back(static_cast<int32_t>(s0 + i));
            z.push_back(pr->z_s[s0 + i]);
        }
        for (int64_t i = 0; i < ml; ++i) {
            const int32_t r = pr->l_pos[l0 + i];
            if (r < 0 || r >= n_snp_bed) { ctx->err = "large SNP bed row out of range"; dbslmm_plan_destroy(p); return DBSLMM_E_ARG; }
            slot_pos.push_back(r);
            slot_block.push_back(nb);
            slot_out.push_back(static_cast<int32_t>(-1 - (l0 + i)));
            z.push_back(pr->z_l[l0 + i]);
        }
        for (int64_t i = m; i < ld; ++i) {
            slot_pos.push_back(-1);
            slot_block.push_back(nb);
            slot_out.push_back(INT32_MIN);
            z.push_back(0.0);
        }
        if (m >= gram_huge_min) {
            const int T = static_cast<int>((m + gram::kHT - 1) / gram::kHT);
            auto& q = m >= lead_min ? lq : tiled ? hq : nq;
            auto& ld_ = m >= lead_min ? lload : tiled ? hload : nload;
            for (int si = 0; si < T; si += kGramSq)
                for (int sj = 0; sj <= si; sj += kGramSq) {
                    const int x = static_cast<int>(std::min_element(ld_.begin(), ld_.end()) - ld_.begin());
                    for (int ti = si; ti < std::min(T, si + kGramSq); ++ti)
                        for (int tj = sj; tj < std::min(ti + 1, sj + kGramSq); ++tj) {
                            q[x].push_back({nb, ti, tj, 0});
                            ld_[x] += 1;
                        }
                }
            int64_t sub = 0;
            for (int ti = 0; ti < T; ++ti)
                for (int tj = 0; tj <= ti; ++tj) {
                    const int64_t rv = std::min<int64_t>(gram::kHT, m - int64_t(gram::kHT) * ti);
                    const int64_t cv = std::min<int64_t>(gram::kHT, m - int64_t(gram::kHT) * tj);
                    const int64_t ni = (rv + 31) / 32, nj = (cv + 31) / 32;
                    sub += ti != tj ? ni * nj : ni * (ni + 1) / 2;
                }
            ops_exec += 2.0 * p->kpad * 32 * 32 * sub;
        } else if (m >= gram_big_min) {
            const int T = static_cast<int>((m + gram::kGT - 1) / gram::kGT);
            const int x = static_cast<int>(std::min_element(xload.begin(), xload.end()) - xload.begin());
            for (int ti = 0; ti < T; ++ti)
                for (int tj = 0; tj <= ti; ++tj) xq[x].push_back({nb, ti, tj, 0});
            xload[x] += T * (T + 1) / 2;
            ops_exec += 2.0 * p->kpad * gram::kGT * gram::kGT * (T * (T - 1) / 2 + 0.75 * T);
        } else {
            const int T = static_cast<int>((m + kTile - 1) / kTile);
            for (int ti = 0; ti < T; ++ti)
                for (int tj = 0; tj <= ti; ++tj) tiles.push_back({nb, ti, tj, 0});
            ops_exec += 2.0 * p->kpad * kTile * kTile * (T * (T + 1) / 2);
        }
        ops_alg += static_cast<double>(pr->n_ref) * m * (m + 1);
        (tiled ? chol_flops_tiled : ld > chol::kSmallLd ? chol_flops_large : chol_flops_small) +=
            m * static_cast<double>(m) * m / 3.0 + 2.0 * m * m;
    }
    p->n_nonempty = static_cast<int32_t>(row0.size());
    p->n_slots = static_cast<int32_t>(slot_pos.size());
    p->h_ms = msv;
    p->h_row0 = row0;
    for (size_t b = 0; b < mv.size(); ++b) p->has_large = p->has_large || mv[b] > msv[b];
    p->h_slot_out = slot_out;
    p->n_tiles = static_cast<int32_t>(tiles.size());
    std::vector<GramTile> btiles;
    {
        size_t qmax = 0;
        for (const auto& q : xq) qmax = std::max(qmax, q.size());
        btiles.assign(qmax * kXcd, GramTile{-1, 0, 0, 0});
        for (int x = 0; x < kXcd; ++x)
            for (size_t i = 0; i < xq[x].size(); ++i) btiles[i * kXcd + x] = xq[x][i];
        p->n_btiles = static_cast<int32_t>(btiles.size());
    }
    std::vector<GramTile> htiles;
    for (const auto* qs : {&lq, &hq, &nq}) {
        size_t qmax = 0;
        for (const auto& q : *qs) qmax = std::max(qmax, q.size());
        const size_t base = htiles.size();
        htiles.resize(base + qmax * kXcd, GramTile{-1, 0, 0, 0});
        for (int x = 0; x < kXcd; ++x)
            for (size_t i = 0; i < (*qs)[x].size(); ++i) htiles[base + i * kXcd + x] = (*qs)[x][i];
        if (qs == &lq) p->n_htiles_lead = static_cast<int32_t>(htiles.size());
        if (qs == &hq) p->n_htiles_tiled = static_cast<int32_t>(htiles.size());
    }
    {
        bool all_huge = true, any_tiled = false;
        for (size_t b = 0; b < mv.size(); ++b) {
            any_tiled = any_tiled || is_tiled[b];
            if (is_tiled[b] && mv[b] < gram_huge_min) all_huge = false;
        }
        p->early_fork = all_huge && any_tiled && op.lead_min >= 0;
    }
    p->n_htiles = static_cast<int32_t>(htiles.size());
    p->M_elems = moff;
    p->h_ld = ldv;
    p->h_blk_id = blk_id;
    p->h_matoff = matoff;
    std::vector<int32_t> order(p->n_nonempty);
    std::iota(order.begin(), order.end(), 0);
    std::stable_sort(order.begin(), order.end(), [&](int a, int c) { return mv[a] > mv[c]; });
    order.erase(std::remove_if(order.begin(), order.end(), [&](int b) { return is_tiled[b] != 0; }),
                order.end());
    int32_t large_ld_max = 0;
    for (int32_t b : order) {
        (ldv[b] > chol::kSmallLd ? p->n_large : p->n_small)++;
        if (ldv[b] > chol::kSmallLd) large_ld_max = std::max(large_ld_max, ldv[b]);
    }
    p->large_cheb_ok = op.large_cheb == 0 && large_ld_max <= chol::kChebMaxM;
    std::vector<int32_t> tlist;
    {
        std::vector<int32_t> tb, tb_lead, tb_rest;
        for (int b = 0; b < p->n_nonempty; ++b)
            if (is_tiled[b]) {
                tb.push_back(b);
                (mv[b] >= lead_min ? tb_lead : tb_rest).push_back(b);
            }
        p->n_tiled = static_cast<int32_t>(tb.size());
        p->h_m = mv;
        p->h_tb = tb;
        if (tb_lead.empty()) {
            build_tiled(mv, tb, 1, p->n_nonempty, p->tl, tlist);
        } else {
            build_tiled(mv, tb_lead, 1, p->n_nonempty, p->tl, tlist);
            build_tiled(mv, tb_rest, 1, p->n_nonempty, p->tl_rest, tlist);
        }
    }
    std::vector<int32_t> tri_f, tri_b, foff(std::max(1, p->n_nonempty), 0), tcheb_list;
    {
        int32_t nf = 0, tmax = 0;
        for (int32_t b : p->h_tb) {
            foff[b] = nf;
            const int T = (mv[b] + trsv::kT - 1) / trsv::kT;
            nf += T;
            tmax = std::max(tmax, T);
        }
        p->n_tflags = nf;
        (void)tmax;
        p->sub_split = op.sub_split >= 0 && !p->tl_rest.empty() && !p->cheb_fused;
        {
            double lb = 0.0, ab = 0.0;
            for (int32_t b : p->h_tb) {
                const double T = (mv[b] + trsv::kT - 1) / trsv::kT, by = T * (T + 1) / 2;
                ab += by;
                if (mv[b] >= lead_min) lb += by;
            }
            const double share = ab > 0 ? lb / ab : 0.0;
            const int g = static_cast<int>(std::lround(ctx->n_cu * 2.05 * share * std::sqrt(share)));
            p->sub_grid_lead = op.sub_grid_lead > 0 ? op.sub_grid_lead
                                                    : std::clamp(g, std::max(1, ctx->n_cu / 16), std::max(1, ctx->n_cu / 2));
        }
        p->sub_grid_rest = op.sub_grid_rest > 0 ? op.sub_grid_rest : std::max(1, ctx->n_cu - p->sub_grid_lead);
        auto grp_of = [&](int32_t b) { return p->sub_split && mv[b] < lead_min ? 1 : 0; };
        struct It { int grp; double key; int T; int32_t b, I; };
        std::vector<It> v;
        constexpr double alpha = 0.25;
        int tmx = 1;
        for (int32_t b : p->h_tb) tmx = std::max(tmx, (mv[b] + trsv::kT - 1) / trsv::kT);
        for (int32_t b : p->h_tb) {
            const int T = (mv[b] + trsv::kT - 1) / trsv::kT;
            for (int I = 0; I < T; ++I) v.push_back({grp_of(b), static_cast<double>(I) / T - alpha * T / tmx, T, b, I});
        }
        std::stable_sort(v.begin(), v.end(), [&](const It& x, const It& y) {
            return x.grp != y.grp ? x.grp < y.grp : x.key != y.key ? x.key < y.key : x.T > y.T;
        });
        p->n_titems_lead = static_cast<int32_t>(std::count_if(v.begin(), v.end(), [](const It& x) { return x.grp == 0; }));
        if (p->sub_split) {
            std::stable_partition(p->h_tb.begin(), p->h_tb.end(), [&](int32_t b) { return grp_of(b) == 0; });
            p->n_tb_lead = static_cast<int32_t>(std::count_if(p->h_tb.begin(), p->h_tb.end(),
                                                              [&](int32_t b) { return grp_of(b) == 0; }));
        }
        if (p->sub_split && op.sub_split == 2) {
            std::vector<int32_t> rb(p->h_tb.begin() + p->n_tb_lead, p->h_tb.end());
            int32_t tmax_r = 0;
            for (int32_t b : rb) tmax_r = std::max(tmax_r, (mv[b] + trsv::kT - 1) / trsv::kT);
            if (!rb.empty() && tmax_r * trsv::kT <= kTChebMaxM) {
                std::stable_sort(rb.begin(), rb.end(), [&](int32_t x, int32_t y) { return mv[x] > mv[y]; });
                tcheb_list = rb;
                p->sub_block = true;
                p->n_tcheb = static_cast<int32_t>(rb.size());
                p->tcheb_vld = tmax_r * trsv::kT;
            }
        }
        for (const It& x : v) {
            tri_f.push_back(x.b);
            tri_f.push_back(x.I);
            tri_b.push_back(x.b);
            tri_b.push_back(x.T - 1 - x.I);
        }
        p->n_titems = static_cast<int32_t>(tri_f.size() / 2);
        double tb = 0.0;
        for (int32_t b : p->h_tb) {
            const double T = (mv[b] + trsv::kT - 1) / trsv::kT;
            tb += T * (T + 1) / 2 * trsv::kT * trsv::kT * sizeof(double);
        }
        p->wl[13] = tb;
    }
    const double n_snp = static_cast<double>(p->n_s + p->n_l);
    p->wl[0] = n_snp;
    p->wl[1] = static_cast<double>(p->n_slots) * (sizeof(int32_t) + sizeof(v4i) + sizeof(int32_t));
    p->wl[2] = static_cast<double>(p->n_slots) * 3 * sizeof(double) + static_cast<double>(p->n_nonempty) * sizeof(int32_t);
    p->wl[3] = ops_alg;
    p->wl[4] = ops_exec;
    p->wl[5] = chol_flops_large;
    p->wl[6] = p->n_nonempty;
    p->wl[7] = p->n_tiles + p->n_btiles + p->n_htiles;
    p->wl[8] = chol_flops_small;
    p->wl[9] = p->n_large;
    p->wl[10] = chol_flops_tiled;
    p->wl[11] = p->n_tiled;
    p->wl[12] = static_cast<double>(std::count_if(p->tl.begin(), p->tl.end(),
                                                  [](const TLaunch& L) { return L.kind < kTlRecord; }) +
                                    std::count_if(p->tl_rest.begin(), p->tl_rest.end(),
                                                  [](const TLaunch& L) { return L.kind < kTlRecord; }));
    p->wl[14] = 0;
    p->wl[15] = -1;

    hipError_t e = hipSetDevice(ctx->device);
    auto fail = [&](const char* what) {
        ctx->err = std::string(what) + ": " + hipGetErrorString(e);
        dbslmm_plan_destroy(p);
        return DBSLMM_E_HIP;
    };
    if (e != hipSuccess) return fail("hipSetDevice");
    if ((e = panel_image(ctx, pr->bed, pr->bed_len, pr->n_ref, &p->img)) != hipSuccess) return fail("upload bed");
    p->d_img = p->img.mem.get();
    if ((e = dev_upload(&p->d_slot_pos, slot_pos, ctx->stream)) != hipSuccess) return fail("upload slots");
    if ((e = dev_upload(&p->d_slot_block, slot_block, ctx->stream)) != hipSuccess) return fail("upload slots");
    if ((e = dev_upload(&p->d_slot_out, slot_out, ctx->stream)) != hipSuccess) return fail("upload slots");
    if ((e = dev_upload(&p->d_z, z, ctx->stream)) != hipSuccess) return fail("upload z");
    if ((e = dev_upload(&p->d_row0, row0, ctx->stream)) != hipSuccess) return fail("upload blocks");
    if ((e = dev_upload(&p->d_m, mv, ctx->stream)) != hipSuccess) return fail("upload blocks");
    if ((e = dev_upload(&p->d_ms, msv, ctx->stream)) != hipSuccess) return fail("upload blocks");
    if ((e = dev_upload(&p->d_ld, ldv, ctx->stream)) != hipSuccess) return fail("upload blocks");
    if ((e = dev_upload(&p->d_matoff, matoff, ctx->stream)) != hipSuccess) return fail("upload blocks");
    if ((e = dev_upload(&p->d_blk_id, blk_id, ctx->stream)) != hipSuccess) return fail("upload blocks");
    if ((e = dev_upload(&p->d_order, order, ctx->stream)) != hipSuccess) return fail("upload order");
    if ((e = dev_upload(&p->d_tiles, tiles, ctx->stream)) != hipSuccess) return fail("upload tiles");
    if ((e = dev_upload(&p->d_btiles, btiles, ctx->stream)) != hipSuccess) return fail("upload tiles");
    if ((e = dev_upload(&p->d_htiles, htiles, ctx->stream)) != hipSuccess) return fail("upload tiles");
    if ((e = dev_upload(&p->d_tlist, tlist, ctx->stream)) != hipSuccess) return fail("upload tiled lists");
    if ((e = dev_upload(&p->d_tri_f, tri_f, ctx->stream)) != hipSuccess) return fail("upload trsv lists");
    if ((e = dev_upload(&p->d_tri_b, tri_b, ctx->stream)) != hipSuccess) return fail("upload trsv lists");
    if ((e = dev_upload(&p->d_foff, foff, ctx->stream)) != hipSuccess) return fail("upload trsv lists");
    if ((e = dev_upload(&p->d_tb, p->h_tb, ctx->stream)) != hipSuccess) return fail("upload trsv lists");
    if (!tcheb_list.empty() && (e = dev_upload(&p->d_tcheb_blocks, tcheb_list, ctx->stream)) != hipSuccess)
        return fail("upload trsv lists");
    if ((e = hipMalloc(&p->d_tflags, (p->n_tflags + 3) * sizeof(int32_t))) != hipSuccess) return fail("hipMalloc trsv flags");
    if ((e = hipMemsetAsync(p->d_tflags, 0, (p->n_tflags + 3) * sizeof(int32_t), ctx->stream)) != hipSuccess) return fail("hipMemset trsv flags");
    if ((e = hipMalloc(&p->d_tepi, std::max(1, p->n_tflags) * sizeof(int32_t))) != hipSuccess) return fail("hipMalloc trsv flags");
    if ((e = hipMemsetAsync(p->d_tepi, 0, std::max(1, p->n_tflags) * sizeof(int32_t), ctx->stream)) != hipSuccess) return fail("hipMemset trsv flags");
// ... 457 lines not shown
            a.n_items = grp.n_items;
            trsv::CGArgs ca{};
            if (cg) {
                a.mode = 2;
                a.conv = p->d_cgconv;
                ca.tb = p->d_tb + grp.tb_off;
                ca.row0 = p->d_row0;
                ca.m = p->d_m;
                ca.ms = p->d_ms;
                ca.blk_id = p->d_blk_id;
                ca.slot_out = p->d_slot_out;
                ca.st_base = a.status;
                ca.nr = nr;
                ca.vs = vs;
                ca.Z = Z;
                ca.X = X;
                ca.R = R;
                ca.D = D;
                ca.S = S;
                for (int j = 0; j < nr; ++j) {
                    ca.delta[j] = cp.coef[cp.coef_off[g] + 3 * j + 2];
                    ca.floor_s[j] = cp.db + ca.delta[j] + 1.0 - p->tau;
                    ca.cix[j] = cix[j];
                }
                ca.floor_l = 1.0 - p->tau;
                ca.tol = p->cheb_tol;
                ca.rec = p->d_cgrec;
                ca.conv = p->d_cgconv;
                ca.iters = p->d_cgit;
                ca.inv_sqrt_n = isn;
                ca.beta_s = p->d_beta_s;
                ca.beta_l = p->d_beta_l;
                ca.ns_stride = p->n_s;
                ca.nl_stride = p->n_l;
                ca.status = p->d_status;
                ca.st_stride = p->nbk;
            }
            for (int k = 0; k < K; ++k) {
                for (int pass = 0; pass < 2; ++pass) {
                    const bool fwd = pass == 0;
                    if (const int rc = next_epoch(p, 1)) return rc;
                    a.epoch = p->trsv_epoch;
                    a.items = (fwd ? p->d_tri_f : p->d_tri_b) + 2 * grp.item_off;
                    a.src = fwd ? R : Y;
                    a.dst = fwd ? Y : Z;
                    a.coef = coef + static_cast<int64_t>(k) * nr * 3;
                    a.last = k == K - 1;
                    if (nr == 1) launch_trsv<1>(fwd, a.grid, st, a);
                    else launch_trsv<2>(fwd, a.grid, st, a);
                    HIP_TRY(ctx, hipGetLastError());
                    p->trsv_pending = true;
                }
                if (cg) {
                    ca.k = k;
                    ca.last = k == K - 1;
                    hipLaunchKernelGGL(dbslmm_cg_update, dim3(grp.n_tb), dim3(trsv::kCGThreads), 0, st, ca);
                    HIP_TRY(ctx, hipGetLastError());
                }
            }
            continue;
        }
        a.fused = 1;
        a.items = p->d_cheb_items;
        a.n_items = p->n_cheb_items;
        a.grid = std::max(1, std::min(ctx->n_cu, p->n_cheb_items));
        a.epoch = p->trsv_epoch + 1;
        if (const int rc = next_epoch(p, 2 * K)) return rc;
        if (nr == 1) hipLaunchKernelGGL(dbslmm_trsv_cheb<1>, dim3(a.grid), dim3(trsv::kThreads), trsv::kLdsBytes, st, a);
        else hipLaunchKernelGGL(dbslmm_trsv_cheb<2>, dim3(a.grid), dim3(trsv::kThreads), trsv::kLdsBytes, st, a);
        HIP_TRY(ctx, hipGetLastError());
        p->trsv_pending = true;
    }
    return DBSLMM_OK;
}

static int run_tcheb(dbslmm_plan* p, double isn, const ChebPlan& cp, hipStream_t st) {
    dbslmm_ctx* ctx = p->ctx;
    const int64_t vs = std::max<int64_t>(1, p->n_slots);
    const int64_t blk = trsv::kMaxR * vs;
    double *X = p->d_cheb + 2 * blk, *R = X + blk, *D = R + blk, *S = D + blk;
    for (size_t g = 0; g < cp.iters.size(); ++g) {
        const size_t g0 = g * trsv::kMaxR;
        const int nr = static_cast<int>(std::min<size_t>(trsv::kMaxR, cp.others.size() - g0));
        TChebArgs a{};
        a.M = p->d_M + static_cast<int64_t>(cp.base) * p->M_elems;
        a.matoff = p->d_matoff;
        a.ld = p->d_ld;
        a.m = p->d_m;
        a.ms = p->d_ms;
        a.row0 = p->d_row0;
        a.blk_id = p->d_blk_id;
        a.slot_out = p->d_slot_out;
        a.blocks = p->d_tcheb_blocks;
        a.n_blocks = p->n_tcheb;
        a.iters = cp.iters[g];
        a.vld = p->tcheb_vld;
        a.vs = vs;
        a.x_base = p->d_y + static_cast<int64_t>(cp.base) * p->n_slots;
        a.X = X;
        a.R = R;
        a.D = D;
        a.S = S;
        a.coef = p->d_coef + cp.coef_off[g];
        a.inv_sqrt_n = isn;
        a.beta_s = p->d_beta_s;
        a.beta_l = p->d_beta_l;
        a.ns_stride = p->n_s;
        a.nl_stride = p->n_l;
        for (int j = 0; j < trsv::kMaxR; ++j) a.cix[j] = j < nr ? cp.others[g0 + j] : cp.others[g0];
        a.st_base = p->d_status + cp.base * p->nbk;
        a.status = p->d_status;
        a.st_stride = p->nbk;
        const size_t lds = (static_cast<size_t>(nr) * a.vld + trsv::kT * nr) * sizeof(double);
        if (nr == 1) hipLaunchKernelGGL(dbslmm_tcheb<1>, dim3(p->n_tcheb), dim3(trsv::kBThreads), lds, st, a);
        else hipLaunchKernelGGL(dbslmm_tcheb<2>, dim3(p->n_tcheb), dim3(trsv::kBThreads), lds, st, a);
        HIP_TRY(ctx, hipGetLastError());
    }
    return DBSLMM_OK;
}

constexpr double kPcgDmin = 2.0;
static bool pcg_route(const dbslmm_plan* p, const double* sigmas, int n) {
    if (p->force_factor || p->solver == 1 || p->n_nonempty == 0 || p->debug_stop) return false;
    if (n > pcg::kMaxNC || !(p->tau > 0.0 && p->tau <= 1.0) || (p->tau >= 1.0 && p->has_large)) return false;
    if (p->solver == 2) return true;
    for (int c = 0; c < n; ++c)
        if (1.0 / (sigmas[c] * static_cast<double>(p->n_obs)) < kPcgDmin) return false;
    return true;
}

static int pcg_layout(dbslmm_plan* p, int n) {
    dbslmm_ctx* ctx = p->ctx;
    if (p->pcg_g16 && !p->d_G16) {
        std::vector<int64_t> off;
        std::vector<int32_t> ldv;
        int64_t o = 0;
        for (int b = 0; b < p->n_nonempty; ++b) {
            const int64_t l = (p->h_m[b] + pcg::kT - 1) / pcg::kT * pcg::kT;
            off.push_back(o);
            ldv.push_back(static_cast<int32_t>(l));
            o += l * l;
        }
        const size_t e = static_cast<size_t>(o) + 256;
        HIP_TRY(ctx, hipMalloc(&p->d_G16, e * sizeof(uint16_t)));
        HIP_TRY(ctx, hipMemsetAsync(p->d_G16, 0, e * sizeof(uint16_t), ctx->stream));
        HIP_TRY(ctx, dev_upload(&p->d_off16, off, ctx->stream));
        HIP_TRY(ctx, dev_upload(&p->d_ld16, ldv, ctx->stream));
        p->h_off16 = off;
    }
    if (!p->h_pmon) HIP_TRY(ctx, hipHostMalloc(&p->h_pmon, (1 + std::max(1, p->n_nonempty)) * sizeof(int32_t),
                                               hipHostMallocDefault));
    if (p->pcg_n == n) return DBSLMM_OK;
    void* old[] = {p->d_pblk, p->d_pitem, p->d_prow, p->d_pvec, p->d_ppart, p->d_pdot, p->d_pqs, p->d_pcnv,
                   p->d_pitb, p->d_pdone, p->d_pact, p->d_pflist};
    HIP_TRY(ctx, hipStreamSynchronize(ctx->stream));
    for (void* q : old)
        if (q) (void)hipFree(q);
    p->d_pflist = nullptr;
    p->pcg_trim = false;
    using namespace pcg;
    std::vector<PcgBlk> blk;
    std::vector<int2> flist;
    std::vector<double> mat, part;
    std::vector<int4> items;
    std::vector<int2> rows;
    int64_t vo = 0, po = 0, dof = 0;
    int32_t sco = 0;
    const double esz = p->pcg_g16 ? 2.0 : 8.0;
    int run = 1;
    p->pcg_run = run;
    for (int b = 0; b < p->n_nonempty; ++b) {
        const int32_t m = p->h_m[b], Tb = (m + kT - 1) / kT, nrun = (Tb + run - 1) / run;
        const bool msh = n > 1 && p->h_ms[b] == m;
        const int32_t nc = msh ? 1 : n;
        const bool fused = p->pcg_fused && Tb <= kFTb && !p->h_off16.empty();
        PcgBlk k{b, p->h_row0[b], m, p->h_ms[b], p->h_ld[b], Tb, Tb + nrun, sco, p->h_matoff[b], vo, po, dof,
                 p->h_off16.empty() ? 0 : p->h_off16[b], nc, msh ? 1 : 0, fused ? 1 : 0, 0};
        if (fused) {
            const int32_t bi = static_cast<int32_t>(blk.size());
            if (nc == 1) flist.push_back(int2{bi, msh ? -1 : 0});
            else for (int c = 0; c < nc; ++c) flist.push_back(int2{bi, c});
        }
        const int bi = static_cast<int>(blk.size());
        blk.push_back(k);
        vo += static_cast<int64_t>(Tb) * kT;
        po += static_cast<int64_t>(Tb) * k.Ns * nc * kT;
        dof += static_cast<int64_t>(Tb) * kNDot * n;
        sco += n;
        for (int I = 0; I < Tb; ++I) {
            rows.push_back(int2{bi, I});
            for (int J0 = 0; J0 <= I; J0 += run) items.push_back(int4{bi, I, J0, std::min(I, J0 + run - 1)});
        }
        mat.push_back(0.5 * m * (m + 1.0) * esz);
        double runs = 0.0;
        for (int I = 0; I < Tb; ++I) runs += I / run + 1;
        part.push_back(fused ? 0.0 : 2.0 * 8.0 * nc * kT * (0.5 * Tb * (Tb + 1.0) + runs));
    }
    std::stable_sort(items.begin(), items.end(), [&](const int4& x, const int4& y) {
        return blk[x.x].fused != blk[y.x].fused ? blk[x.x].fused < blk[y.x].fused : blk[x.x].Tb > blk[y.x].Tb;
    });
    std::stable_sort(flist.begin(), flist.end(), [&](const int2& x, const int2& y) { return blk[x.x].Tb > blk[y.x].Tb; });
    std::stable_sort(rows.begin(), rows.end(), [&](const int2& x, const int2& y) { return blk[x.x].fused < blk[y.x].fused; });
    p->n_prow_chip = p->n_pitem_chip = 0;
    for (const int2& r : rows) p->n_prow_chip += blk[r.x].fused ? 0 : 1;
    for (const int4& e : items) p->n_pitem_chip += blk[e.x].fused ? 0 : 1;
    p->h_pfused.assign(blk.size(), 0);
    p->h_pnseq.assign(blk.size(), 0);
    for (const int2& f : flist) {
        p->h_pfused[f.x] = 1;
        p->h_pnseq[f.x] += 1;
    }
    p->n_pflist = static_cast<int32_t>(flist.size());
    if (!flist.empty()) HIP_TRY(ctx, dev_upload(&p->d_pflist, flist, ctx->stream));
    if (!flist.empty() && !p->d_pfnext) HIP_TRY(ctx, hipMalloc(&p->d_pfnext, 16));
    p->n_pblk = static_cast<int32_t>(blk.size());
    p->n_pitem = static_cast<int32_t>(items.size());
    p->n_prow = static_cast<int32_t>(rows.size());
    p->pcg_vstride = vo;
    p->h_pmat = mat;
    p->h_ppart = part;
    HIP_TRY(ctx, dev_upload(&p->d_pblk, blk, ctx->stream));
    HIP_TRY(ctx, dev_upload(&p->d_pitem, items, ctx->stream));
    HIP_TRY(ctx, dev_upload(&p->d_prow, rows, ctx->stream));
    HIP_TRY(ctx, hipMalloc(&p->d_pvec, std::max<int64_t>(1, 6 * n * vo) * sizeof(double)));
    HIP_TRY(ctx, hipMalloc(&p->d_ppart, std::max<int64_t>(1, po) * sizeof(double)));
    HIP_TRY(ctx, hipMalloc(&p->d_pdot, std::max<int64_t>(1, dof) * sizeof(double)));
    HIP_TRY(ctx, hipMalloc(&p->d_pqs, std::max<int32_t>(1, sco) * pcg::kQS * sizeof(double)));
    HIP_TRY(ctx, hipMalloc(&p->d_pcnv, std::max<int32_t>(1, sco) * sizeof(int32_t)));
    HIP_TRY(ctx, hipMalloc(&p->d_pitb, std::max<int32_t>(1, p->n_pblk) * sizeof(int32_t)));
    HIP_TRY(ctx, hipMalloc(&p->d_pdone, std::max<int32_t>(1, p->n_pblk) * sizeof(int32_t)));
    HIP_TRY(ctx, hipMalloc(&p->d_pact, sizeof(int32_t)));
    p->pcg_n = n;
    return DBSLMM_OK;
}

static int pcg_first_chunk(const dbslmm_plan* p, const double* sigmas, int n) {
    if (p->pcg_need >= 0) return std::min(p->pcg_need, p->pcg_maxit);
    double dmin = INFINITY;
    for (int c = 0; c < n; ++c) dmin = std::min(dmin, 1.0 / (sigmas[c] * static_cast<double>(p->n_obs)));
    const double kap = 1.0 + 12.0 / std::max(1e-3, dmin + 1.0 - p->tau);
    const double q = (std::sqrt(kap) - 1.0) / (std::sqrt(kap) + 1.0);
    const int k = static_cast<int>(std::ceil(std::log(2.0 / p->pcg_tol) / -std::log(q))) + 2 + (p->has_large ? 4 : 0);
    return std::clamp(k, 1, p->pcg_maxit);
}

static int pcg_iters(dbslmm_plan* p, int K) {
    dbslmm_ctx* ctx = p->ctx;
    hipStream_t s = ctx->stream;
    for (int k = 0; k < K; ++k) {
        const int32_t ni = p->pcg_trim ? p->n_pitem_chip : p->n_pitem, nr = p->pcg_trim ? p->n_prow_chip : p->n_prow;
        if (ni == 0 && nr == 0) continue;
        const dim3 g((std::max(1, ni) + pcg::kWaves - 1) / pcg::kWaves);
        if (p->pcg_g16)
            hipLaunchKernelGGL(dbslmm_pcg_symv16, g, dim3(pcg::kThreads), pcg::lds_bytes(p->pcg_n), s, p->pcg_args,
                               p->d_pitem, ni);
        if (!p->pcg_g16 || p->pcg_m_blocks != 0)
            hipLaunchKernelGGL(dbslmm_pcg_symv64, g, dim3(pcg::kThreads), pcg::lds_bytes(p->pcg_n), s, p->pcg_args,
                               p->d_pitem, ni);
        hipLaunchKernelGGL(dbslmm_pcg_rows, dim3(std::max(1, nr)), dim3(pcg::kThreads), 0, s, p->pcg_args, p->d_prow);
        hipLaunchKernelGGL(dbslmm_pcg_update, dim3(std::max(1, nr)), dim3(pcg::kThreads), 0, s, p->pcg_args, p->d_prow);
    }
    HIP_TRY(ctx, hipGetLastError());
    p->pcg_it += K;
    if (p->pcg_join) {
        HIP_TRY(ctx, hipStreamWaitEvent(s, ctx->join, 0));
        p->pcg_join = false;
    }
    hipLaunchKernelGGL(dbslmm_pcg_final, dim3(p->n_prow), dim3(pcg::kThreads), 0, s, p->pcg_args, p->d_prow);
    HIP_TRY(ctx, hipGetLastError());
    HIP_TRY(ctx, hipMemcpyAsync(p->h_pmon, p->d_pact, sizeof(int32_t), hipMemcpyDeviceToHost, s));
    HIP_TRY(ctx, hipMemcpyAsync(p->h_pmon + 1, p->d_pitb, p->n_pblk * sizeof(int32_t), hipMemcpyDeviceToHost, s));
    if (p->pcg_ev_end) HIP_TRY(ctx, hipEventRecord(p->pcg_ev_end, s));
    return DBSLMM_OK;
}

static int pcg_finish(dbslmm_plan* p) {
    dbslmm_ctx* ctx = p->ctx;
    while (p->pcg_pending) {
        HIP_TRY(ctx, hipSetDevice(ctx->device));
        HIP_TRY(ctx, hipStreamSynchronize(ctx->stream));
        int32_t need = 0;
        for (int b = 0; b < p->n_pblk; ++b)
            if (p->h_pfused.empty() || !p->h_pfused[b]) need = std::max(need, p->h_pmon[1 + b]);
        if (p->h_pmon[0] <= 0 || p->pcg_it >= p->pcg_maxit) {
            p->pcg_pending = false;
            p->pcg_need = p->h_pmon[0] <= 0 ? need : p->pcg_maxit;
            p->pcg_iters_max = 0;
            for (int b = 0; b < p->n_pblk; ++b) p->pcg_iters_max = std::max(p->pcg_iters_max, p->h_pmon[1 + b]);
            if (p->pcg_m_blocks < 0) {
                std::vector<int32_t> fl(std::max(1, p->n_nonempty));
                HIP_TRY(ctx, hipMemcpy(fl.data(), p->d_flags, fl.size() * sizeof(int32_t), hipMemcpyDeviceToHost));
                p->pcg_m_blocks = 0;
                p->h_pmiss.assign(p->n_pblk, 0);
                for (int b = 0; b < p->n_nonempty; ++b) {
                    p->pcg_m_blocks += fl[b] & 1;
                    if (b < p->n_pblk) p->h_pmiss[b] = fl[b] & 1;
                }
            }
            p->pcg_trim = true;
            for (int b = 0; b < p->n_pblk && b < static_cast<int>(p->h_pfused.size()); ++b)
                if (p->h_pfused[b] && p->h_pmiss[b]) p->pcg_trim = false;
            p->pcg_cbytes = p->pcg_pbytes = p->pcg_fbytes = 0.0;
            for (int b = 0; b < p->n_pblk && b < static_cast<int>(p->h_pmat.size()); ++b) {
                const double it = p->h_pmon[1 + b];
                const bool miss = !p->h_pmiss.empty() && p->h_pmiss[b];
                const double mb = p->h_pmat[b] * (miss && p->pcg_g16 ? 4.0 : 1.0);
                if (!p->h_pfused.empty() && p->h_pfused[b] && !miss) {
                    p->pcg_fbytes += it * mb * p->h_pnseq[b];
                } else {
                    p->pcg_cbytes += it * mb;
                    p->pcg_pbytes += it * p->h_ppart[b];
                }
            }
            break;
        }
        const int K = std::min(std::max(4, p->pcg_it / 4), p->pcg_maxit - p->pcg_it);
        if (const int rc = pcg_iters(p, K)) return rc;
    }
    return DBSLMM_OK;
}

static int run_pcg(dbslmm_plan* p, const double* sigmas, int n) {
    dbslmm_ctx* ctx = p->ctx;
#ifdef DBSLMM_DIAG
    {
        const hipError_t e = hipGetLastError();
        if (e != hipSuccess) fprintf(stderr, "run_pcg: stale error on entry: %s\n", hipGetErrorString(e));
    }
#endif
    if (const int rc = ensure_copies(p, n, 1)) return rc;
#ifdef DBSLMM_DIAG
    {
        const hipError_t e = hipGetLastError();
        if (e != hipSuccess) fprintf(stderr, "run_pcg: error after ensure_copies: %s\n", hipGetErrorString(e));
    }
#endif
    if (const int rc = pcg_layout(p, n)) return rc;
#ifdef DBSLMM_DIAG
    {
        const hipError_t e = hipGetLastError();
        if (e != hipSuccess) fprintf(stderr, "run_pcg: error after pcg_layout: %s\n", hipGetErrorString(e));
    }
#endif
    hipStream_t s = ctx->stream;
    hipEvent_t* ev = nullptr;
    if (p->timing) {
        const size_t need = kEvPerRun * static_cast<size_t>(p->runs_pending + 1);
        while (p->ev.size() < need) {
            hipEvent_t e;
            HIP_TRY(ctx, hipEventCreate(&e));
            p->ev.push_back(e);
        }
        ev = &p->ev[kEvPerRun * p->runs_pending];
        p->runs_pending++;
        p->run_route.resize(p->runs_pending);
        p->run_route.back() = 1;
    }
    p->pcg_ev_end = ev ? ev[7] : nullptr;
    p->trsv_failed = false;
    p->stopped = false;
    const size_t nbk = static_cast<size_t>(p->nbk);
    HIP_TRY(ctx, hipMemsetAsync(p->d_flags, 0, nbk * sizeof(int32_t), s));
    HIP_TRY(ctx, hipMemsetAsync(p->d_status, 0, n * nbk * sizeof(int32_t), s));
    HIP_TRY(ctx, hipMemsetAsync(p->d_pact, 0, sizeof(int32_t), s));
    if (ev) HIP_TRY(ctx, hipEventRecord(ev[0], s));
    for (int c = 0; c < n; ++c)
        hipLaunchKernelGGL(dbslmm_set_scalar, dim3(1), dim3(1), 0, s, p->d_dshift + c,
                           1.0 / (sigmas[c] * static_cast<double>(p->n_obs)));
    if (p->n_slots > 0)
        hipLaunchKernelGGL(dbslmm_slot_stats, dim3((p->n_slots + 255) / 256), dim3(256), 0, s, p->img.rows(),
                           p->n_ref, p->d_slot_pos, p->d_slot_block, p->n_slots, p->d_S, p->d_mu, p->d_rsd,
                           p->d_flags);
    HIP_TRY(ctx, hipGetLastError());
    if (ev) for (int k : {1, 9, 10}) HIP_TRY(ctx, hipEventRecord(ev[k], s));
    uint16_t* g16 = p->pcg_g16 ? p->d_G16 : nullptr;
    const double nrd = static_cast<double>(p->n_ref), padk = static_cast<double>(p->kpad - p->n_ref);
    auto gram = [&](hipStream_t st, const GramTile* ti, int32_t nt, const GramTile* tb, int32_t nb,
                    const GramTile* th, int32_t nh) {
        if (nh > 0)
            hipLaunchKernelGGL(dbslmm_gram_huge, dim3(nh), dim3(512), gram::kHLdsBytes, st, p->d_img, p->kpad,
                               p->d_slot_pos, p->img.n_rows, th, nh,
                               p->d_row0, p->d_m, p->d_ld, p->d_matoff, p->d_flags, p->d_S, p->d_mu, p->d_rsd, nrd,
                               padk, p->tau, p->d_M, 1, p->M_elems, INT32_MAX, -1, g16, p->d_off16, p->d_ld16);
        if (nt > 0)
            hipLaunchKernelGGL(dbslmm_gram_i8, dim3((nt + 3) / 4), dim3(256), 0, st, p->d_img, p->kpad, p->d_slot_pos,
                               p->img.n_rows, ti, nt, p->d_row0,
                               p->d_m, p->d_ld, p->d_matoff, p->d_flags, p->d_S, p->d_mu, p->d_rsd, nrd, padk, p->tau,
                               p->d_M, 1, p->M_elems, INT32_MAX, -1, g16, p->d_off16, p->d_ld16);
        if (nb > 0)
            hipLaunchKernelGGL(dbslmm_gram_big, dim3(nb), dim3(256), gram::kLdsBytes, st, p->d_img, p->kpad,
                               p->d_slot_pos, p->img.n_rows, tb, nb,
                               p->d_row0, p->d_m, p->d_ld, p->d_matoff, p->d_flags, p->d_S, p->d_mu, p->d_rsd, nrd,
                               padk, p->tau, p->d_M, 1, p->M_elems, INT32_MAX, -1, g16, p->d_off16, p->d_ld16);
        return hipGetLastError();
    };
    HIP_TRY(ctx, gram(s, p->d_tiles, p->n_tiles, p->d_btiles, p->n_btiles, p->d_htiles, p->n_htiles));
    if (ev) for (int k : {2, 5, 6, 8, 11}) HIP_TRY(ctx, hipEventRecord(ev[k], s));
    PcgArgs a{};
    a.blk = p->d_pblk;
    a.G16 = g16;
    a.M = p->d_M;
    a.flags = p->d_flags;
    a.S = p->d_S;
    a.rsd = p->d_rsd;
    a.z = p->d_z;
    a.slot_out = p->d_slot_out;
    a.blk_id = p->d_blk_id;
    a.dshift = p->d_dshift;
    const int64_t vs = static_cast<int64_t>(n) * p->pcg_vstride;
    a.X = p->d_pvec;
    a.R = a.X + vs;
    a.P = a.R + vs;
    a.Sv = a.P + vs;
    a.W = a.Sv + vs;
    a.U = a.W + vs;
    a.part = p->d_ppart;
    a.dot = p->d_pdot;
    a.qs = p->d_pqs;
    a.cnv = p->d_pcnv;
    a.itb = p->d_pitb;
    a.done = p->d_pdone;
    a.active = p->d_pact;
    a.beta_s = p->d_beta_s;
    a.beta_l = p->d_beta_l;
    a.status = p->d_status;
    a.vstride = p->pcg_vstride;
    a.ns = p->n_s;
    a.nl = p->n_l;
    a.nbk = p->nbk;
    a.tau = p->tau;
    a.rn = 1.0 / nrd;
    a.c0 = p->tau * (nrd - 1.0) / nrd + 1.0 - p->tau;
    a.tol = p->pcg_tol;
    a.inv_sqrt_n = 1.0 / std::sqrt(static_cast<double>(p->n_obs));
    a.ncopy = n;
    a.run = p->pcg_run;
    for (int c = 1; c < n; ++c)
        if (sigmas[c] > sigmas[a.seed]) a.seed = c;
    p->pcg_args = a;
    hipLaunchKernelGGL(dbslmm_pcg_init, dim3(p->n_prow), dim3(pcg::kThreads), 0, s, a, p->d_prow);
    HIP_TRY(ctx, hipGetLastError());
    p->pcg_join = false;
    if (p->n_pflist > 0) {
        HIP_TRY(ctx, hipEventRecord(ctx->fork, s));
        HIP_TRY(ctx, hipStreamWaitEvent(ctx->stream2, ctx->fork, 0));
        if (ev) HIP_TRY(ctx, hipEventRecord(ev[3], ctx->stream2));
        const int grid = std::max(1, std::min(p->n_pflist, ctx->n_cu));
        HIP_TRY(ctx, hipMemsetAsync(p->d_pfnext, 0, 16, ctx->stream2));
        hipLaunchKernelGGL(dbslmm_pcg_block, dim3(grid), dim3(pcg::kThreads), pcg::block_lds_bytes(n), ctx->stream2, a,
                           p->d_pflist, p->n_pflist, p->d_pfnext, p->pcg_maxit);
        HIP_TRY(ctx, hipGetLastError());
        if (ev) HIP_TRY(ctx, hipEventRecord(ev[4], ctx->stream2));
        HIP_TRY(ctx, hipEventRecord(ctx->join, ctx->stream2));
        p->pcg_join = true;
    } else if (ev) {
        for (int k : {3, 4}) HIP_TRY(ctx, hipEventRecord(ev[k], s));
    }
    p->pcg_it = 0;
    p->pcg_pending = true;
    if (const int rc = pcg_iters(p, pcg_first_chunk(p, sigmas, n))) return rc;
    p->ran = true;
    p->n_runs++;
    p->sigma_run = sigmas[n - 1];
    p->var_copy = n - 1;
    p->pcg_ran = true;
    p->pcg_pending_var = true;
    p->cheb_base = -1;
    p->cg_ran = false;
    p->cheb_pending_var = false;
    p->wl[14] = 0;
    p->wl[15] = -1;
    p->wl[16] = 0;
    return DBSLMM_OK;
}

static int run_impl(dbslmm_plan* p, bool front, const double* sigmas, int n) {
    dbslmm_ctx* ctx = p->ctx;
    HIP_TRY(ctx, hipSetDevice(ctx->device));
    if (const int rc = pcg_finish(p)) return rc;
    if (front && pcg_route(p, sigmas, n)) return run_pcg(p, sigmas, n);
    if (const int rc = ensure_copies(p, n, n)) return rc;
    if (n > 1) {
        if (p->multi_n != n) {
            std::lock_guard<std::mutex> lk(g_capture_mu);
            std::vector<int32_t> tlist;
            p->tl_multi.clear();
            build_tiled(p->h_m, p->h_tb, n, p->n_nonempty, p->tl_multi, tlist);
            if (p->d_tlist_multi) (void)hipFree(p->d_tlist_multi);
            p->d_tlist_multi = nullptr;
            HIP_TRY(ctx, dev_upload(&p->d_tlist_multi, tlist, ctx->stream));
            if (p->graph_multi) (void)hipGraphExecDestroy(p->graph_multi);
            p->graph_multi = nullptr;
            p->multi_n = n;
        }
    }
    p->trsv_failed = false;
    ChebPlan cp;
    const bool cheb = front && p->n_nonempty > 0 && cheb_plan(p, sigmas, n, cp);
    const int32_t tcopy = cheb ? cp.base : -1;
    const bool large_cheb = cheb && p->large_cheb_ok;
    const int32_t tmin_copy = large_cheb ? chol::kSmallLd : p->tiled_min;
    hipStream_t s = ctx->stream;
    hipEvent_t* ev = nullptr;
    if (p->timing) {
        const size_t need = kEvPerRun * static_cast<size_t>(p->runs_pending + 1);
        while (p->ev.size() < need) {
            hipEvent_t e;
            HIP_TRY(ctx, hipEventCreate(&e));
            p->ev.push_back(e);
        }
        ev = &p->ev[kEvPerRun * p->runs_pending];
        p->runs_pending++;
        p->run_route.resize(p->runs_pending);
        p->run_route.back() = 0;
    }
    p->pcg_ran = false;
    p->pcg_pending_var = false;
    const size_t nbk = static_cast<size_t>(p->nbk);
    if (p->n_tflags > 0 && p->trsv_epoch > INT32_MAX - kEpochsPerRun) {
        HIP_TRY(ctx, hipMemsetAsync(p->d_tflags, 0, p->n_tflags * sizeof(int32_t), s));
        HIP_TRY(ctx, hipMemsetAsync(p->d_tepi, 0, p->n_tflags * sizeof(int32_t), s));
        p->trsv_epoch = 0;
    }
    p->stopped = false;
    if (front) HIP_TRY(ctx, hipMemsetAsync(p->d_flags, 0, nbk * sizeof(int32_t), s));
    HIP_TRY(ctx, hipMemsetAsync(p->d_status, 0, n * nbk * sizeof(int32_t), s));
    if (ev) HIP_TRY(ctx, hipEventRecord(ev[0], s));
    if (front && p->n_slots > 0) {
        hipLaunchKernelGGL(dbslmm_slot_stats, dim3((p->n_slots + 255) / 256), dim3(256), 0, s, p->img.rows(),
                           p->n_ref, p->d_slot_pos, p->d_slot_block, p->n_slots, p->d_S, p->d_mu, p->d_rsd,
                           p->d_flags);
        HIP_TRY(ctx, hipGetLastError());
    }
    if (ev) HIP_TRY(ctx, hipEventRecord(ev[9], s));
    if (!front && n > 1)
        return (ctx->err = "a multi-copy run needs the Gram front", DBSLMM_E_STATE);
    const std::vector<TLaunch>& tl = n > 1 && !cheb ? p->tl_multi : p->tl;
    const bool lead = !p->tl_rest.empty() && (n == 1 || cheb);
    const int fcopy = cheb ? cp.base : 0;
    const double isn = 1.0 / std::sqrt(static_cast<double>(p->n_obs));
    if (p->n_nonempty > 0) {
        for (int c = 0; c < n; ++c) {
            const double dshift = 1.0 / (sigmas[c] * static_cast<double>(p->n_obs));
            hipLaunchKernelGGL(dbslmm_set_scalar, dim3(1), dim3(1), 0, s, p->d_dshift + c, dshift);
        }
        if (cheb) {
            const int rc = cheb_prepare(p, cp, s);
            if (rc != DBSLMM_OK) return rc;
        }
    }
    auto gram_huge = [&](int32_t t0, int32_t nt) {
        hipLaunchKernelGGL(dbslmm_gram_huge, dim3(nt), dim3(512), gram::kHLdsBytes, s, p->d_img,
                           p->kpad, p->d_slot_pos, p->img.n_rows, p->d_htiles + t0, nt, p->d_row0, p->d_m, p->d_ld,
                           p->d_matoff, p->d_flags, p->d_S, p->d_mu, p->d_rsd,
                           static_cast<double>(p->n_ref), static_cast<double>(p->kpad - p->n_ref),
                           p->tau, p->d_M, n, p->M_elems, tmin_copy, tcopy, nullptr, nullptr, nullptr);
    };
    if (front && p->n_htiles_lead > 0) {
        gram_huge(0, p->n_htiles_lead);
        HIP_TRY(ctx, hipGetLastError());
    }
    if (ev) HIP_TRY(ctx, hipEventRecord(ev[10], s));
    if (lead) {
        HIP_TRY(ctx, hipEventRecord(ctx->fork, s));
        debug_spin(p, s, 1);
    }
    if (ev) HIP_TRY(ctx, hipEventRecord(ev[1], s));
    if (front && p->n_htiles_tiled > p->n_htiles_lead) {
        gram_huge(p->n_htiles_lead, p->n_htiles_tiled - p->n_htiles_lead);
        HIP_TRY(ctx, hipGetLastError());
    }
    const bool early = p->early_fork && p->n_nonempty > 0;
    if (early) {
        HIP_TRY(ctx, hipEventRecord(ctx->fork2, s));
        HIP_TRY(ctx, hipStreamWaitEvent(lead ? ctx->stream4 : ctx->stream2, ctx->fork2, 0));
    }
    if (front && p->n_tiles > 0) {
        dim3 grid((p->n_tiles + 3) / 4);
// ... 80 lines not shown
        if (lead) {
            HIP_TRY(ctx, hipStreamWaitEvent(ctx->stream2, ctx->fork, 0));
            if (ev) HIP_TRY(ctx, hipEventRecord(ev[6], ctx->stream2));
            debug_spin(p, ctx->stream2, -1);
            debug_spin(p, ctx->stream4, 1);
            int rc = run_tiled_copy(p, isn, fcopy);
            if (rc == DBSLMM_OK) rc = run_rest_copy(p, isn, fcopy);
            if (rc != DBSLMM_OK) return rc;
        } else if (ev) {
            HIP_TRY(ctx, hipEventRecord(ev[6], ctx->stream2));
        }
        if (!tl.empty()) {
            if (n == 1 || cheb) {
                int rc = lead ? DBSLMM_OK : run_tiled_copy(p, isn, fcopy);
                if (lead && p->sub_split) {
                    const TGroup gr = tgroup_rest(p), gl = tgroup_lead(p);
                    if (rc == DBSLMM_OK && gr.n_items > 0) rc = run_pbwd(p, isn, fcopy, gr);
                    if (ev && cheb) HIP_TRY(ctx, hipEventRecord(ev[11], gr.st));
                    if (rc == DBSLMM_OK && cheb && gr.n_items > 0)
                        rc = p->sub_block ? run_tcheb(p, isn, cp, gr.st) : run_cheb(p, isn, cp, gr);
                    if (rc == DBSLMM_OK) rc = run_pbwd(p, isn, fcopy, gl);
                    if (rc != DBSLMM_OK) return rc;
                    if (cheb) {
                        if (ev) HIP_TRY(ctx, hipEventRecord(ev[8], ctx->stream2));
                        rc = run_cheb(p, isn, cp, gl);
                        if (rc != DBSLMM_OK) return rc;
                    }
                    HIP_TRY(ctx, hipEventRecord(ctx->join4, ctx->stream4));
                    HIP_TRY(ctx, hipStreamWaitEvent(ctx->stream2, ctx->join4, 0));
                } else {
                    if (lead) {
                        HIP_TRY(ctx, hipEventRecord(ctx->join4, ctx->stream4));
                        HIP_TRY(ctx, hipStreamWaitEvent(ctx->stream2, ctx->join4, 0));
                    }
                    if (rc == DBSLMM_OK) rc = run_pbwd(p, isn, fcopy, tgroup_all(p));
                    if (rc != DBSLMM_OK) return rc;
                    if (cheb) {
                        if (ev) HIP_TRY(ctx, hipEventRecord(ev[8], ctx->stream2));
                        if (ev) HIP_TRY(ctx, hipEventRecord(ev[11], ctx->stream2));
                        rc = run_cheb(p, isn, cp, tgroup_all(p));
                        if (rc != DBSLMM_OK) return rc;
                    }
                }
            } else {
                int rc = launch_graph(p, isn, tl, p->d_tlist_multi, 0, p->graph_multi, seq_main(p));
                for (int c = 0; c < n && rc == DBSLMM_OK; ++c) rc = run_pbwd(p, isn, c, tgroup_all(p));
                if (rc != DBSLMM_OK) return rc;
            }
        }
        if (ev && !cheb) HIP_TRY(ctx, hipEventRecord(ev[8], ctx->stream2));
        if (ev && !cheb) HIP_TRY(ctx, hipEventRecord(ev[11], ctx->stream2));
        if (ev) HIP_TRY(ctx, hipEventRecord(ev[7], ctx->stream2));
        HIP_TRY(ctx, hipEventRecord(ctx->join3, ctx->stream2));
        if (ss != s) HIP_TRY(ctx, hipStreamWaitEvent(s, ctx->join, 0));
        HIP_TRY(ctx, hipStreamWaitEvent(s, ctx->join3, 0));
    }
    else if (ev) {
        HIP_TRY(ctx, hipEventRecord(ev[3], s));
        HIP_TRY(ctx, hipEventRecord(ev[4], s));
        HIP_TRY(ctx, hipEventRecord(ev[5], s));
        HIP_TRY(ctx, hipEventRecord(ev[6], s));
        HIP_TRY(ctx, hipEventRecord(ev[8], s));
        HIP_TRY(ctx, hipEventRecord(ev[11], s));
        HIP_TRY(ctx, hipEventRecord(ev[7], s));
    }
    p->ran = true;
    p->n_runs++;
    p->sigma_run = sigmas[n - 1];
    p->var_copy = n - 1;
    {
        p->cheb_base = cheb ? cp.base : -1;
        int iters = 0;
        for (int k : cp.iters) iters += k;
        p->wl[14] = cheb ? iters : 0;
        p->wl[15] = p->cheb_base;
        p->cg_ran = cheb && p->h2f_cg && !p->cheb_fused;
        p->wl[16] = cheb ? 2.0 * iters * p->wl[13] : 0.0;
        p->cheb_pending_var = cheb && cp.base != n - 1;
    }
    return DBSLMM_OK;
}

static int check_trsv(dbslmm_plan* p) {
    dbslmm_ctx* ctx = p->ctx;
    if (p->trsv_pending) {
        std::lock_guard<std::mutex> lk(g_capture_mu);
        int32_t werr = 0;
        HIP_TRY(ctx, hipMemcpy(&werr, p->d_tflags + p->n_tflags + 1, sizeof(int32_t), hipMemcpyDeviceToHost));
        if (werr) {
            HIP_TRY(ctx, hipMemsetAsync(p->d_tflags + p->n_tflags + 1, 0, sizeof(int32_t), ctx->stream));
            HIP_TRY(ctx, hipStreamSynchronize(ctx->stream));
        }
        p->trsv_pending = false;
        p->trsv_failed = p->trsv_failed || werr != 0;
    }
    if (p->trsv_failed) {
        ctx->err = "substitution hand-off wait gave up (trsv): the tiled blocks' betas of this run are invalid";
        return DBSLMM_E_HIP;
    }
    return DBSLMM_OK;
}

static int download_copies(dbslmm_plan* p, int c0, int n, double* beta_s, double* beta_l, int32_t* block_status) {
    dbslmm_ctx* ctx = p->ctx;
    if (!p->ran) { ctx->err = "plan_download before plan_run"; return DBSLMM_E_STATE; }
    if (p->stopped) { ctx->err = "plan_download after a run stopped at the Gram (debug_stop)"; return DBSLMM_E_STATE; }
    HIP_TRY(ctx, hipSetDevice(ctx->device));
    if (const int rc = pcg_finish(p)) return rc;
    HIP_TRY(ctx, hipStreamSynchronize(ctx->stream));
    if (const int rc = check_trsv(p)) return rc;
    const size_t nbs = beta_s ? static_cast<size_t>(n) * p->n_s : 0;
    const size_t nbl = beta_l ? static_cast<size_t>(n) * p->n_l : 0;
    const size_t nst = block_status && p->num_block ? static_cast<size_t>(n) * p->nbk : 0;
    const size_t bytes = (nbs + nbl) * sizeof(double) + nst * sizeof(int32_t);
    if (bytes == 0) return DBSLMM_OK;
    if (bytes > p->h_pin_bytes) {
        if (p->h_pin) HIP_TRY(ctx, hipHostFree(p->h_pin));
        p->h_pin = nullptr;
        p->h_pin_bytes = 0;
        HIP_TRY(ctx, hipHostMalloc(&p->h_pin, bytes, hipHostMallocDefault));
        p->h_pin_bytes = bytes;
    }
    double* ps = static_cast<double*>(p->h_pin);
    double* pl = ps + nbs;
    int32_t* pt = reinterpret_cast<int32_t*>(pl + nbl);
    while (static_cast<int>(p->dl_ev.size()) < n) {
        hipEvent_t e;
        HIP_TRY(ctx, hipEventCreateWithFlags(&e, hipEventDisableTiming));
        p->dl_ev.push_back(e);
    }
    if (nst) HIP_TRY(ctx, hipMemcpyAsync(pt, p->d_status + c0 * p->nbk, nst * sizeof(int32_t),
                                         hipMemcpyDeviceToHost, ctx->stream));
    const size_t cs = nbs / n, cl = nbl / n;
    for (int c = 0; c < n; ++c) {
        if (cs) HIP_TRY(ctx, hipMemcpyAsync(ps + c * cs, p->d_beta_s + static_cast<int64_t>(c0 + c) * p->n_s,
                                            cs * sizeof(double), hipMemcpyDeviceToHost, ctx->stream));
        if (cl) HIP_TRY(ctx, hipMemcpyAsync(pl + c * cl, p->d_beta_l + static_cast<int64_t>(c0 + c) * p->n_l,
                                            cl * sizeof(double), hipMemcpyDeviceToHost, ctx->stream));
        HIP_TRY(ctx, hipEventRecord(p->dl_ev[c], ctx->stream));
    }
    for (int c = 0; c < n; ++c) {
        HIP_TRY(ctx, hipEventSynchronize(p->dl_ev[c]));
        if (cs) par_memcpy(beta_s + c * cs, ps + c * cs, cs * sizeof(double));
        if (cl) par_memcpy(beta_l + c * cl, pl + c * cl, cl * sizeof(double));
    }
    for (int c = 0; c < n && nst; ++c) {
        int32_t* out = block_status + static_cast<int64_t>(c) * p->num_block;
        memcpy(out, pt + c * p->nbk, p->num_block * sizeof(int32_t));
        for (int32_t b : p->h_empty) out[b] = DBSLMM_BLOCK_EMPTY;
    }
    return DBSLMM_OK;
}

static int download_copy(dbslmm_plan* p, int c, double* beta_s, double* beta_l, int32_t* block_status) {
    return download_copies(p, c, 1, beta_s, beta_l, block_status);
}

int dbslmm_plan_run(dbslmm_plan* p) {
    if (!p) return DBSLMM_E_ARG;
    if (p->mp) return mp_run(p, &p->sigma_s, 1, false);
    return run_impl(p, true, &p->sigma_s, 1);
}

int dbslmm_plan_run_multi(dbslmm_plan* p, const double* sigmas, int32_t n_sigma, double* beta_s,
                          double* beta_l, int32_t* block_status) {
    if (!p) return DBSLMM_E_ARG;
    dbslmm_ctx* ctx = p->ctx;
    ARG_CHECK(ctx, sigmas && n_sigma > 0 && n_sigma <= 64, "sigmas / n_sigma (1..64)");
    for (int i = 0; i < n_sigma; ++i)
        ARG_CHECK(ctx, sigmas[i] > 0.0 && std::isfinite(sigmas[i]), "sigma_s must be > 0");
    if (p->mp) {
        for (auto& sh : p->mp->shards)
            ARG_CHECK(ctx, static_cast<int64_t>(sh.plan->n_nonempty) * n_sigma < 32768,
                      "blocks x sigmas per device must stay below 32768 (packed work items)");
        int rc = mp_run(p, sigmas, n_sigma, true);
        if (rc == DBSLMM_OK) rc = mp_download_all(p, n_sigma, beta_s, beta_l, block_status);
        return rc;
    }
    ARG_CHECK(ctx, static_cast<int64_t>(p->n_nonempty) * n_sigma < 32768,
              "blocks x sigmas must stay below 32768 (packed work items)");
    int rc = run_impl(p, true, sigmas, n_sigma);
    if (!rc) rc = dbslmm_plan_sync(p);
    if (!rc) rc = download_copies(p, 0, n_sigma, beta_s, beta_l, block_status);
    return rc;
}

int dbslmm_plan_sync(dbslmm_plan* p) {
    if (!p) return DBSLMM_E_ARG;
    if (p->mp) return mp_sync(p);
    HIP_TRY(p->ctx, hipSetDevice(p->ctx->device));
    if (const int rc = pcg_finish(p)) return rc;
    HIP_TRY(p->ctx, hipStreamSynchronize(p->ctx->stream));
    if (const int rc = check_trsv(p)) return rc;
    if (p->timing) return collect_timing(p);
    p->runs_pending = 0;
    p->run_route.clear();
    return DBSLMM_OK;
}

int dbslmm_plan_kernel_ms(dbslmm_plan* p, double* ms_out, int32_t* launches_out) {
    if (!p || !ms_out) return DBSLMM_E_ARG;
    if (p->mp) {
        int32_t runs = INT32_MAX;
        for (int k = 0; k < DBSLMM_K_COUNT; ++k) ms_out[k] = 0.0;
        for (auto& sh : p->mp->shards) {
            if (p->ran && sh.run_copies.empty()) continue;
            double ms[DBSLMM_K_COUNT];
            int32_t n = 0;
            dbslmm_plan_kernel_ms(sh.plan, ms, &n);
            for (int k = 0; k < DBSLMM_K_COUNT; ++k) ms_out[k] = std::max(ms_out[k], ms[k]);
            runs = std::min(runs, n);
        }
        if (launches_out) *launches_out = runs == INT32_MAX ? 0 : runs;
        return DBSLMM_OK;
    }
    for (int k = 0; k < DBSLMM_K_COUNT; ++k) ms_out[k] = p->ms_runs ? p->ms_acc[k] / p->ms_runs : 0.0;
    if (launches_out) *launches_out = p->ms_runs;
    return DBSLMM_OK;
}

#ifdef DBSLMM_DIAG
extern "C" int dbslmm_diag_trsv_stamps(dbslmm_plan* p, unsigned long long* out, int n) {
    if (!p || !p->d_stamps) return DBSLMM_E_STATE;
    if (hipDeviceSynchronize() != hipSuccess) return DBSLMM_E_HIP;
    return hipMemcpy(out, p->d_stamps, n * sizeof(unsigned long long), hipMemcpyDeviceToHost) == hipSuccess
               ? DBSLMM_OK : DBSLMM_E_HIP;
}
#endif

int dbslmm_plan_block_iters(dbslmm_plan* p, int32_t* iters) {
    if (!p || !iters) return DBSLMM_E_ARG;
    if (p->mp) return mp_block_iters(p, iters);
    HIP_TRY(p->ctx, hipSetDevice(p->ctx->device));
    if (const int rc = pcg_finish(p)) return rc;
    HIP_TRY(p->ctx, hipStreamSynchronize(p->ctx->stream));
    std::fill(iters, iters + p->num_block, 0);
    if (!p->pcg_ran) return DBSLMM_OK;
    for (int b = 0; b < p->n_pblk; ++b) iters[p->h_blk_id[b]] = p->h_pmon[1 + b];
    return DBSLMM_OK;
}

int dbslmm_plan_workload(const dbslmm_plan* p, double* out) {
    if (!p || !out) return DBSLMM_E_ARG;
    if (p->mp) {
        for (int i = 0; i < DBSLMM_WORKLOAD_LEN; ++i) out[i] = 0.0;
        out[15] = -1;
        if (p->mp->shards.empty()) return DBSLMM_OK;
        for (auto& sh : p->mp->shards) {
            if (p->ran && sh.run_copies.empty()) continue;
            double w[DBSLMM_WORKLOAD_LEN];
            dbslmm_plan_workload(sh.plan, w);
            for (int i = 0; i < DBSLMM_WORKLOAD_LEN; ++i)
                out[i] = (i == 12 || i == 14 || i == 17 || i == 18) ? std::max(out[i], w[i])
                         : ((i == 0 || i == 6) && sh.copy > 0) ? out[i] : out[i] + w[i];
        }
        double w0[DBSLMM_WORKLOAD_LEN];
        dbslmm_plan_workload(p->mp->shards[0].plan, w0);
        out[15] = w0[15];
        return DBSLMM_OK;
    }
    for (int i = 0; i < DBSLMM_WORKLOAD_LEN; ++i) out[i] = p->wl[i];
    out[17] = p->pcg_ran ? 1.0 : 0.0;
    out[18] = p->pcg_ran ? p->pcg_iters_max : 0.0;
    out[19] = p->pcg_ran ? p->pcg_cbytes : 0.0;
    out[20] = p->pcg_ran ? p->pcg_pbytes : 0.0;
    out[21] = p->pcg_ran ? p->pcg_fbytes : 0.0;
    if (p->cg_ran && p->d_cgit) {
        std::vector<int32_t> it(std::max(1, p->n_nonempty));
        if (hipSetDevice(p->ctx->device) != hipSuccess ||
            hipMemcpy(it.data(), p->d_cgit, it.size() * sizeof(int32_t), hipMemcpyDeviceToHost) != hipSuccess)
            return DBSLMM_E_HIP;
        double bytes = 0.0;
        for (int32_t b : p->h_tb) {
            const double T = (p->h_m[b] + trsv::kT - 1) / trsv::kT;
            bytes += 2.0 * it[b] * T * (T + 1) / 2 * trsv::kT * trsv::kT * sizeof(double);
        }
        out[16] = bytes;
    }
    return DBSLMM_OK;
}

int dbslmm_plan_block_matrix(dbslmm_plan* p, int32_t block, int32_t copy, double* out, int32_t* ld_out) {
    if (!p) return DBSLMM_E_ARG;
    dbslmm_ctx* ctx = p->ctx;
    ARG_CHECK(ctx, block >= 0 && block < p->num_block, "block out of range");
    if (p->mp) {
        for (auto& sh : p->mp->shards)
            for (size_t j = 0; j < sh.blocks.size(); ++j)
                if (sh.blocks[j] == block) {
                    const int rc = dbslmm_plan_block_matrix(sh.plan, static_cast<int32_t>(j), copy, out, ld_out);
                    if (rc != DBSLMM_OK) ctx->err = sh.plan->ctx->err;
                    return rc;
                }
        ARG_CHECK(ctx, false, "block has no SNPs");
    }
    ARG_CHECK(ctx, copy >= 0 && copy < p->m_copies, "copy out of range");
    const auto it = std::find(p->h_blk_id.begin(), p->h_blk_id.end(), block);
    ARG_CHECK(ctx, it != p->h_blk_id.end(), "block has no SNPs");
    const size_t nb = static_cast<size_t>(it - p->h_blk_id.begin());
    const int64_t ld = p->h_ld[nb];
    if (ld_out) *ld_out = static_cast<int32_t>(ld);
    if (!out) return DBSLMM_OK;
    HIP_TRY(ctx, hipSetDevice(ctx->device));
    if (const int rc = pcg_finish(p)) return rc;
    std::lock_guard<std::mutex> lk(g_capture_mu);
    HIP_TRY(ctx, hipDeviceSynchronize());
    HIP_TRY(ctx, hipMemcpy(out, p->d_M + static_cast<int64_t>(copy) * p->M_elems + p->h_matoff[nb],
                           ld * ld * sizeof(double), hipMemcpyDeviceToHost));
    return DBSLMM_OK;
}

int dbslmm_plan_download(dbslmm_plan* p, double* beta_s, double* beta_l, int32_t* block_status) {
    if (!p) return DBSLMM_E_ARG;
    if (p->mp) {
        if (!p->ran) { p->ctx->err = "plan_download before plan_run"; return DBSLMM_E_STATE; }
        return mp_download(p, p->var_copy, beta_s, beta_l, block_status);
    }
    return download_copy(p, p->var_copy, beta_s, beta_l, block_status);
}

int dbslmm_est(dbslmm_ctx* ctx, const dbslmm_problem* pr, double* beta_s, double* beta_l,
               int32_t* block_status) {
    if (!ctx) return DBSLMM_E_ARG;
    dbslmm_plan* p = nullptr;
    int rc = dbslmm_plan_create(ctx, pr, &p);
    if (rc) return rc;
    rc = dbslmm_plan_run(p);
    if (!rc) rc = dbslmm_plan_sync(p);
    if (!rc) rc = dbslmm_plan_download(p, beta_s, beta_l, block_status);
    dbslmm_plan_destroy(p);
    return rc;
}

static int variance_factor(dbslmm_plan* p) {
    if (const int rc = pcg_finish(p)) return rc;
    if (!p->cheb_pending_var && !p->pcg_pending_var) return DBSLMM_OK;
    const double sg = p->sigma_run;
    p->cheb_pending_var = false;
    p->pcg_pending_var = false;
    p->force_factor = true;
    const int rc = run_impl(p, true, &sg, 1);
    p->force_factor = false;
    return rc;
}

int dbslmm_plan_variance(dbslmm_plan* p, const dbslmm_test_panel* tp, double* diags,
                         int32_t* n_test_out) {
    if (!p) return DBSLMM_E_ARG;
    dbslmm_ctx* ctx = p->ctx;
    if (!p->ran) { ctx->err = "plan_variance before plan_run"; return DBSLMM_E_STATE; }
    if (p->stopped) { ctx->err = "plan_variance after a run stopped at the Gram (debug_stop)"; return DBSLMM_E_STATE; }
    if (p->mp) return mp_variance(p, tp, diags, n_test_out);
    ARG_CHECK(ctx, tp && tp->bed && tp->indicator && tp->n_total > 0, "bad test panel");
    if (const int rc = variance_factor(p)) return rc;
    ARG_CHECK(ctx, p->n_s == 0 || tp->s_pos, "test panel s_pos missing");
    ARG_CHECK(ctx, p->n_l == 0 || tp->l_pos, "test panel l_pos missing");
    std::vector<int32_t> sel;
    for (int32_t i = 0; i < tp->n_total; ++i)
        if (tp->indicator[i] != 0) sel.push_back(i);
    const int32_t n_test = static_cast<int32_t>(sel.size());
    if (n_test_out) *n_test_out = n_test;
    if (n_test == 0 || p->num_block == 0) return DBSLMM_OK;
    ARG_CHECK(ctx, diags, "null diags");
    const int64_t tbps = (tp->n_total + 3) / 4;
    const int64_t n_rows = (tp->bed_len - 3) / tbps;
    ARG_CHECK(ctx, tp->bed_len >= 3 + tbps, "test bed image shorter than one SNP row");
    std::vector<int32_t> tpos(p->n_slots);
    for (int32_t s = 0; s < p->n_slots; ++s) {
        const int32_t o = p->h_slot_out[s];
        int32_t r = -1;
        if (o >= 0) r = tp->s_pos[o];
        else if (o != INT32_MIN) r = tp->l_pos[-1 - o];
        ARG_CHECK(ctx, o == INT32_MIN || (r >= 0 && r < n_rows), "test SNP bed row out of range");
        tpos[s] = r;
    }
    const int64_t nt_pad = round_up(n_test, 64);
    const int64_t cpitch = nt_pad / 4;
    const int64_t cbytes = std::max<int64_t>(1, p->n_slots) * cpitch;
    HIP_TRY(ctx, hipSetDevice(ctx->device));
    hipStream_t st = ctx->stream;
    uint8_t *d_tbed = nullptr, *d_cbed = nullptr;
    int32_t *d_tpos = nullptr, *d_sel = nullptr, *d_cpos = nullptr;
    double *d_mu = nullptr, *d_rsd = nullptr, *d_Y = nullptr, *d_diags = nullptr;
    std::vector<int32_t> cpos(p->n_slots);
    for (int32_t s = 0; s < p->n_slots; ++s) cpos[s] = tpos[s] >= 0 ? s : -1;
    const size_t ndiag = static_cast<size_t>(n_test) * p->num_block;
    int rc = DBSLMM_OK;
    std::lock_guard<std::mutex> lk(g_capture_mu);
    do {
        hipError_t e;
        if ((e = hipMalloc(&d_tbed, tp->bed_len + kBedPad)) != hipSuccess ||
// ... 241 lines not shown
```

include/dbslmm_hip.h:

```cpp
#ifndef DBSLMM_HIP_H_
#define DBSLMM_HIP_H_

#include <stdint.h>

#ifdef __cplusplus
extern "C" {
#endif

#define DBSLMM_ABI_VERSION 16

enum {
    DBSLMM_OK = 0,
    DBSLMM_E_ARG = -1,
    DBSLMM_E_HIP = -2,
    DBSLMM_E_STATE = -3
};

enum {
    DBSLMM_BLOCK_OK = 0,
    DBSLMM_BLOCK_EMPTY = 1,
    DBSLMM_BLOCK_NOT_PD = 2,
    DBSLMM_BLOCK_MONOMORPHIC = 3,
    DBSLMM_BLOCK_NOT_CONVERGED = 4
};

typedef struct dbslmm_ctx dbslmm_ctx;
typedef struct dbslmm_plan dbslmm_plan;

typedef struct dbslmm_options {
    int32_t tiled_min;
    int32_t gram_big_min;
    int32_t gram_huge_min;
    int32_t h2f_mode;
    double cheb_tol;
    int32_t lead_min;
    int32_t large_cheb;
    int32_t cheb_fused;
    int32_t debug_delay_us;
    int32_t debug_stop;
    int32_t sub_split;
    int32_t sub_grid_lead;
    int32_t sub_grid_rest;
    int32_t shard_copies;
    int32_t h2f_iter;
    int32_t solver;
    double pcg_tol;
    int32_t pcg_maxit;
    int32_t pcg_whole;
} dbslmm_options;

typedef struct dbslmm_problem {
    const uint8_t* bed;
    int64_t bed_len;
    int32_t n_ref;
    int32_t n_obs;
    double sigma_s;
    double tau;
    int32_t num_block;
    const int64_t* s_ptr;
    const int32_t* s_pos;
    const double* z_s;
    const int64_t* l_ptr;
    const int32_t* l_pos;
    const double* z_l;
    const dbslmm_options* opts;
} dbslmm_problem;

enum {
    DBSLMM_K_UNPACK = 0,
    DBSLMM_K_GRAM = 1,
    DBSLMM_K_CHOL_LARGE = 2,
    DBSLMM_K_CHOL_SMALL = 3,
    DBSLMM_K_CHOL_TILED = 4,
    DBSLMM_K_TRSV = 5,
    DBSLMM_K_PCG = 6,
    DBSLMM_K_PCG_BLOCK = 7,
    DBSLMM_K_COUNT = 8
};

int dbslmm_abi_version(void);

int dbslmm_ctx_create(int device, dbslmm_ctx** out);

int dbslmm_ctx_create_multi(int32_t n_dev, const int32_t* device_ids, dbslmm_ctx** out);
int dbslmm_shard_plan(int32_t num_block, const int32_t* m, int32_t n_ref, int32_t n_dev, int32_t n_copies,
                      int32_t* unit_device, double* dev_ms);
int dbslmm_shard_plan_problem(const dbslmm_problem* p, const double* sigma_s, int32_t n_sigma, int32_t n_dev,
                              int32_t* unit_device, double* dev_ms);
int dbslmm_plan_create_units(dbslmm_ctx* ctx, const dbslmm_problem* p, int32_t n_copies,
                             const int32_t* unit_device, int32_t device_index, dbslmm_plan** out);
int dbslmm_ctx_num_devices(const dbslmm_ctx* ctx);
int dbslmm_plan_shard_info(const dbslmm_plan* plan, int32_t* block_device);
void dbslmm_ctx_destroy(dbslmm_ctx* ctx);
const char* dbslmm_last_error(const dbslmm_ctx* ctx);
int dbslmm_ctx_cache_bed(dbslmm_ctx* ctx, const uint8_t* bed, int64_t bed_len);
int dbslmm_ctx_cache_bed_fd(dbslmm_ctx* ctx, int fd, int64_t bed_len, const uint8_t* key);

int dbslmm_est(dbslmm_ctx* ctx, const dbslmm_problem* p, double* beta_s, double* beta_l,
               int32_t* block_status);

int dbslmm_plan_create(dbslmm_ctx* ctx, const dbslmm_problem* p, dbslmm_plan** out);
int dbslmm_plan_run(dbslmm_plan* plan);
int dbslmm_plan_sync(dbslmm_plan* plan);
int dbslmm_plan_download(dbslmm_plan* plan, double* beta_s, double* beta_l, int32_t* block_status);
int dbslmm_plan_run_multi(dbslmm_plan* plan, const double* sigma_s, int32_t n_sigma,
                          double* beta_s, double* beta_l, int32_t* block_status);

int dbslmm_plan_set_sigma(dbslmm_plan* plan, double sigma_s);
void dbslmm_plan_destroy(dbslmm_plan* plan);

int dbslmm_plan_enable_timing(dbslmm_plan* plan, int enable);
int dbslmm_plan_kernel_ms(dbslmm_plan* plan, double* ms_out , int32_t* launches_out);

#define DBSLMM_WORKLOAD_LEN 22
int dbslmm_plan_workload(const dbslmm_plan* plan, double* out );
int dbslmm_plan_block_iters(dbslmm_plan* plan, int32_t* iters);

int dbslmm_plan_block_matrix(dbslmm_plan* plan, int32_t block, int32_t copy, double* out,
                             int32_t* ld_out);

typedef struct dbslmm_test_panel {
    const uint8_t* bed;
    int64_t bed_len;
    int32_t n_total;
    const int32_t* indicator;
    const int32_t* s_pos;
    const int32_t* l_pos;
} dbslmm_test_panel;

int dbslmm_plan_variance(dbslmm_plan* plan, const dbslmm_test_panel* test, double* diags,
                         int32_t* n_test_out);

int dbslmm_bed_maf(dbslmm_ctx* ctx, const uint8_t* bed, int64_t bed_len, int32_t n_ref,
                   int64_t n_snp, double* maf);

int dbslmm_bed_row_stats(dbslmm_ctx* ctx, const uint8_t* bed, int64_t bed_len, int32_t n_ref,
                         int64_t n_rows, int32_t* out );

int dbslmm_read_snp_std(dbslmm_ctx* ctx, const uint8_t* bed, int64_t bed_len, int32_t n_ref,
                        const int32_t* pos, int32_t n_rows, double* out, double* maf);

int dbslmm_valid_blocks(dbslmm_ctx* ctx, const uint8_t* bed, int64_t bed_len, int32_t n_ref,
                        int32_t num_block, const int64_t* ptr, const int32_t* pos,
                        const double* z1, const double* z2, double* nume, double* deno);

#ifdef __cplusplus
}
#endif
#endif
```

Measured before the change: 143.2 million.

## Stream PCG results to mapped host memory as blocks converge

PCG kernels now write each converged block's betas and status directly into a coherent host-mapped mirror buffer and set per-block/copy flags. The host polls these flags while the solve is still running and copies finished ranges into the output arrays. After completion it copies only the remaining ranges in parallel. This overlaps device-to-host result transfer with computation. The cost is extra PCIe writes from the kernels, host polling overhead, and added synchronisation complexity. The feature is on by default for run_multi.

After: 155.6 million, median of 6. +8.7%, better.

```diff
diff --git a/dbslmm_amd/__init__.py b/dbslmm_amd/__init__.py
--- a/dbslmm_amd/__init__.py
+++ b/dbslmm_amd/__init__.py
@@ -114,7 +114,10 @@
         unknown = set(self.opts) - {f[0] for f in _lib.Options._fields_}
         if unknown:
             raise ValueError(f"unknown dbslmm_options fields: {sorted(unknown)}")
-        self._opts = _lib.Options(**self.opts)
+        o = dict(self.opts)
+        if "stream_out" in o and int(o["stream_out"]) == 0:
+            o["stream_out"] = -1
+        self._opts = _lib.Options(**o)
         return _lib.Problem(
             _ptr(self.bed), self.bed.size, self.n_ref, self.n_obs, self.sigma_s, self.tau,
             self.num_block, _ptr(self.s_ptr), _ptr(self.s_pos), _ptr(self.z_s),
@@ -261,6 +264,19 @@
         return bs, bl, st
 
 
+def out_ranges(s_ptr, l_ptr=None) -> np.ndarray:
+    lib = _lib.load()
+    sp = np.ascontiguousarray(s_ptr, dtype=np.int64)
+    lp = None if l_ptr is None else np.ascontiguousarray(l_ptr, dtype=np.int64)
+    nb = len(sp) - 1
+    out = np.zeros((max(1, nb), 5), dtype=np.int64)
+    n = np.zeros(1, dtype=np.int32)
+    rc = lib.dbslmm_out_ranges(nb, _ptr(sp), _ptr(lp), _ptr(out), _ptr(n))
+    if rc != 0:
+        raise DbslmmError(f"dbslmm_out_ranges failed rc={rc}")
+    return out[:int(n[0])]
+
+
 def bed_maf(ctx: Context, bed: np.ndarray, n_ref: int, n_snp: int) -> np.ndarray:
     bed = np.ascontiguousarray(bed, dtype=np.uint8)
     maf = np.zeros(n_snp)
diff --git a/dbslmm_amd/_lib.py b/dbslmm_amd/_lib.py
--- a/dbslmm_amd/_lib.py
+++ b/dbslmm_amd/_lib.py
@@ -15,10 +15,10 @@
     "dbslmm_ctx_create_multi", "dbslmm_ctx_num_devices", "dbslmm_plan_shard_info",
     "dbslmm_ctx_cache_bed", "dbslmm_ctx_cache_bed_fd", "dbslmm_plan_block_matrix",
     "dbslmm_shard_plan", "dbslmm_plan_create_units", "dbslmm_shard_plan_problem",
-    "dbslmm_plan_block_iters", "dbslmm_bed_row_stats",
+    "dbslmm_plan_block_iters", "dbslmm_bed_row_stats", "dbslmm_out_ranges",
 )
 
-ABI_VERSION = 16
+ABI_VERSION = 17
 K_UNPACK, K_GRAM, K_CHOL_LARGE, K_CHOL_SMALL, K_CHOL_TILED, K_TRSV, K_PCG, K_PCG_BLOCK = 0, 1, 2, 3, 4, 5, 6, 7
 KERNEL_NAMES = ("dbslmm_unpack_stats", "dbslmm_gram", "dbslmm_chol_large", "dbslmm_chol_small",
                 "dbslmm_tchol", "dbslmm_trsv", "dbslmm_pcg", "dbslmm_pcg_block")
@@ -35,7 +35,7 @@
         ("debug_stop", C.c_int32), ("sub_split", C.c_int32), ("sub_grid_lead", C.c_int32),
         ("sub_grid_rest", C.c_int32), ("shard_copies", C.c_int32), ("h2f_iter", C.c_int32),
         ("solver", C.c_int32), ("pcg_tol", C.c_double), ("pcg_maxit", C.c_int32),
-        ("pcg_whole", C.c_int32),
+        ("pcg_whole", C.c_int32), ("stream_out", C.c_int32),
     ]
 
 
@@ -105,6 +105,7 @@
     L.dbslmm_plan_create_units.argtypes = [V, P(Problem), C.c_int32, V, C.c_int32, P(V)]
     L.dbslmm_shard_plan_problem.argtypes = [P(Problem), V, C.c_int32, C.c_int32, V, V]
     L.dbslmm_plan_block_iters.argtypes = [V, V]
+    L.dbslmm_out_ranges.argtypes = [C.c_int32, V, V, V, V]
     if hasattr(L, "dbslmm_plan_block_matrix"):
         L.dbslmm_plan_block_matrix.argtypes = [V, C.c_int32, C.c_int32, V, V]
     if L.dbslmm_abi_version() != ABI_VERSION:
diff --git a/dbslmm_amd/csrc/out_ranges.hpp b/dbslmm_amd/csrc/out_ranges.hpp
--- /dev/null
+++ b/dbslmm_amd/csrc/out_ranges.hpp
@@ -0,0 +1,23 @@
+#pragma once
+#include <stdint.h>
+
+#include <vector>
+
+struct OutRange {
+    int64_t s0, s1;
+    int64_t l0, l1;
+    int32_t blk;
+};
+
+inline bool build_out_ranges(int32_t num_block, const int64_t* s_ptr, const int64_t* l_ptr, std::vector<OutRange>& out) {
+    out.clear();
+    if (num_block < 0 || !s_ptr) return false;
+    for (int32_t b = 0; b < num_block; ++b) {
+        const int64_t s0 = s_ptr[b], s1 = s_ptr[b + 1];
+        const int64_t l0 = l_ptr ? l_ptr[b] : 0, l1 = l_ptr ? l_ptr[b + 1] : 0;
+        if (s1 < s0 || l1 < l0) return false;
+        if (s1 == s0 && l1 == l0) continue;
+        out.push_back(OutRange{s0, s1, l0, l1, b});
+    }
+    return true;
+}
diff --git a/dbslmm_amd/csrc/pcg.hip b/dbslmm_amd/csrc/pcg.hip
--- a/dbslmm_amd/csrc/pcg.hip
+++ b/dbslmm_amd/csrc/pcg.hip
@@ -48,9 +48,15 @@
     int32_t* itb;
     int32_t* done;
     int32_t* active;
+    int32_t* fin;
     double* beta_s;
     double* beta_l;
     int32_t* status;
+    double* mir_s;
+    double* mir_l;
+    int32_t* mir_st;
+    int32_t* mir_flag;
+    int32_t run_no;
     int64_t vstride;
     int64_t ns, nl, nbk;
     double tau, rn, c0, tol, inv_sqrt_n;
@@ -155,6 +161,25 @@
 }
 __device__ __forceinline__ double col_shift(const PcgArgs& a, const PcgBlk& B, int k) {
     return a.dshift[B.mshift ? a.seed : k];
+}
+
+__device__ __forceinline__ void put_beta(const PcgArgs& a, const PcgBlk& B, int i, int k, double x, bool mono) {
+    const int so = a.slot_out[B.row0 + i];
+    const double bv = mono ? __builtin_nan("") : x * a.inv_sqrt_n;
+    if (so >= 0) {
+        a.beta_s[k * a.ns + so] = bv;
+        if (a.mir_s) a.mir_s[k * a.ns + so] = bv;
+    } else {
+        a.beta_l[k * a.nl - 1 - so] = bv;
+        if (a.mir_l) a.mir_l[k * a.nl - 1 - so] = bv;
+    }
+}
+__device__ __forceinline__ void put_status(const PcgArgs& a, const PcgBlk& B, int k, bool mono) {
+    const int st = mono ? DBSLMM_BLOCK_MONOMORPHIC
+                        : a.cnv[B.sco + k] == 0 ? DBSLMM_BLOCK_NOT_CONVERGED : DBSLMM_BLOCK_OK;
+    const int64_t o = k * a.nbk + a.blk_id[B.blk];
+    a.status[o] = st;
+    if (a.mir_st) a.mir_st[o] = st;
 }
 
 __device__ __forceinline__ double cvt_lo(uint32_t w) {
@@ -369,6 +394,7 @@
         }
         if (tid == 0) {
             a.itb[bi] = 0;
+            a.fin[bi] = 0;
             const bool fz = B.fused && u16;
             a.done[bi] = mono_s ? 2 : fz ? 3 : 0;
             if (!mono_s && !fz) atomicAdd(a.active, 1);
@@ -597,9 +623,19 @@
     int running = 0;
     for (int k = 0; k < n; ++k) running += run_s[k];
     if (running == 0) {
-        if (I == 0 && tid == 0) {
+        const int r = tid & (kT - 1), h = tid >> 7, i = I * kT + r;
+        if (i < B.m)
+            for (int k = h; k < n; k += 2) put_beta(a, B, i, k, a.X[k * a.vstride + B.vo + i], false);
+        if (I == 0 && tid < n) put_status(a, B, tid, false);
+        __syncthreads();
+        if (tid == 0 &&
+            __hip_atomic_fetch_add(a.fin + bi, 1, __ATOMIC_ACQ_REL, __HIP_MEMORY_SCOPE_AGENT) == B.Tb - 1) {
             a.done[bi] = 1;
             atomicSub(a.active, 1);
+            if (a.mir_flag)
+                for (int c = 0; c < n; ++c)
+                    __hip_atomic_store(a.mir_flag + static_cast<int64_t>(bi) * n + c, a.run_no, __ATOMIC_RELEASE,
+                                       __HIP_MEMORY_SCOPE_SYSTEM);
         }
         return;
     }
@@ -942,9 +978,19 @@
     for (int q = 0; q < kFPer; ++q) {
         const int i = tid + kThreads * q;
         if (i < m)
-            for (int c = 0; c < nx; ++c) a.X[(msh ? c : cc) * a.vstride + B.vo + i] = Xl[c * kFRows + i];
-    }
-    if (tid == 0) atomicMax(a.itb + bi, it + (it < maxit ? 1 : 0));
+            for (int c = 0; c < nx; ++c) put_beta(a, B, i, msh ? c : cc, Xl[c * kFRows + i], false);
+    }
+    if (tid == 0) {
+        atomicMax(a.itb + bi, it + (it < maxit ? 1 : 0));
+        for (int c = 0; c < nx; ++c) put_status(a, B, msh ? c : cc, false);
+    }
+    if (a.mir_flag) {
+        __syncthreads();
+        if (tid == 0)
+            for (int c = 0; c < nx; ++c)
+                __hip_atomic_store(a.mir_flag + static_cast<int64_t>(bi) * n + (msh ? c : cc), a.run_no,
+                                   __ATOMIC_RELEASE, __HIP_MEMORY_SCOPE_SYSTEM);
+    }
 }
 
 extern "C" __global__ __launch_bounds__(pcg::kThreads)
@@ -970,20 +1016,12 @@
     using namespace pcg;
     const int2 it = rows[blockIdx.x];
     const int bi = it.x, I = it.y, tid = threadIdx.x;
+    const int done = a.done[bi];
+    if (done == 3 || done == 1) return;
     const PcgBlk B = a.blk[bi];
-    const bool mono = a.done[bi] == 2;
+    const bool mono = done == 2;
     const int r = tid & (kT - 1), h = tid >> 7, i = I * kT + r;
-    if (i < B.m) {
-        const int so = a.slot_out[B.row0 + i];
-        for (int k = h; k < a.ncopy; k += 2) {
-            const double bv = mono ? __builtin_nan("") : a.X[k * a.vstride + B.vo + i] * a.inv_sqrt_n;
-            if (so >= 0) a.beta_s[k * a.ns + so] = bv;
-            else a.beta_l[k * a.nl - 1 - so] = bv;
-        }
-    }
-    if (I == 0 && tid < a.ncopy) {
-        const int st = mono ? DBSLMM_BLOCK_MONOMORPHIC
-                            : a.cnv[B.sco + tid] == 0 ? DBSLMM_BLOCK_NOT_CONVERGED : DBSLMM_BLOCK_OK;
-        a.status[tid * a.nbk + a.blk_id[B.blk]] = st;
-    }
-}
+    if (i < B.m)
+        for (int k = h; k < a.ncopy; k += 2) put_beta(a, B, i, k, a.X[k * a.vstride + B.vo + i], mono);
+    if (I == 0 && tid < a.ncopy) put_status(a, B, tid, mono);
+}
diff --git a/dbslmm_amd/csrc/plan.hip b/dbslmm_amd/csrc/plan.hip
--- a/dbslmm_amd/csrc/plan.hip
+++ b/dbslmm_amd/csrc/plan.hip
@@ -18,6 +18,7 @@
 #include <vector>
 
 #include "../../include/dbslmm_hip.h"
+#include "out_ranges.hpp"
 
 #include "kernels.hip"
 #include "chol.hip"
@@ -234,7 +235,7 @@
     std::vector<int32_t> h_pnseq;
     bool pcg_join = false;
     double *d_pvec = nullptr, *d_ppart = nullptr, *d_pdot = nullptr, *d_pqs = nullptr;
-    int32_t *d_pcnv = nullptr, *d_pitb = nullptr, *d_pdone = nullptr, *d_pact = nullptr;
+    int32_t *d_pcnv = nullptr, *d_pitb = nullptr, *d_pdone = nullptr, *d_pact = nullptr, *d_pfin = nullptr;
     int64_t pcg_vstride = 0;
     int32_t* h_pmon = nullptr;
     int32_t pcg_it = 0;
@@ -249,6 +250,18 @@
     double pcg_cbytes = 0.0, pcg_pbytes = 0.0, pcg_fbytes = 0.0;
     PcgArgs pcg_args{};
     hipEvent_t pcg_ev_end = nullptr;
+    bool stream_out = true;
+    bool so_want = false;
+    bool so_active = false;
+    void* h_mir = nullptr;
+    size_t h_mir_bytes = 0;
+    int32_t* h_mflag = nullptr;
+    int32_t so_n = 0;
+    int32_t so_run = 0;
+    hipEvent_t so_ev = nullptr;
+    std::vector<OutRange> h_orange;
+    std::vector<int2> h_pfpairs;
+    std::vector<int32_t> so_done;
 };
 
 #define HIP_TRY(ctx, expr)                                                               \
@@ -422,6 +435,34 @@
         if (a < z) th.emplace_back([=] { memcpy(static_cast<char*>(dst) + a, static_cast<const char*>(src) + a, z - a); });
     }
     memcpy(dst, src, std::min(n, part));
+    for (auto& t : th) t.join();
+}
+
+struct CopySeg {
+    void* dst;
+    const void* src;
+    size_t n;
+};
+static void par_memcpy_list(const std::vector<CopySeg>& segs) {
+    constexpr size_t kMin = size_t(512) << 10;
+    size_t total = 0;
+    for (const CopySeg& s : segs) total += s.n;
+    const unsigned hw = std::max(1u, std::min(8u, std::thread::hardware_concurrency()));
+    const unsigned nt = static_cast<unsigned>(std::min<size_t>(hw, std::max<size_t>(1, total / kMin)));
+    const size_t part = (total + nt - 1) / nt;
+    auto work = [&segs, part](unsigned t) {
+        const size_t lo = t * part, hi = lo + part;
+        size_t off = 0;
+        for (const CopySeg& s : segs) {
+            const size_t a = std::max(lo, off), z = std::min(hi, off + s.n);
+            if (a < z) memcpy(static_cast<char*>(s.dst) + (a - off), static_cast<const char*>(s.src) + (a - off), z - a);
+            off += s.n;
+            if (off >= hi) break;
+        }
+    };
+    std::vector<std::thread> th;
+    for (unsigned t = 1; t < nt; ++t) th.emplace_back(work, t);
+    work(0);
     for (auto& t : th) t.join();
 }
 
@@ -820,6 +861,9 @@
     (void)hipSetDevice(p->ctx->device);
     if (p->h_pin) (void)hipHostFree(p->h_pin);
     if (p->h_pmon) (void)hipHostFree(p->h_pmon);
+    if (p->h_mir) (void)hipHostFree(p->h_mir);
+    if (p->h_mflag) (void)hipHostFree(p->h_mflag);
+    if (p->so_ev) (void)hipEventDestroy(p->so_ev);
     p->img = PanelImage{};
     void* bufs[] = {p->d_slot_pos, p->d_slot_block, p->d_slot_out, p->d_z,
                     p->d_S, p->d_mu, p->d_rsd, p->d_y, p->d_flags, p->d_status, p->d_order,
@@ -829,7 +873,7 @@
                     p->d_cheb, p->d_coef, p->d_stamps, p->d_tepi, p->d_cheb_items,
                     p->d_tcheb_blocks, p->d_cgrec, p->d_cgconv, p->d_cgit, p->d_G16, p->d_pblk,
                     p->d_pitem, p->d_prow, p->d_pvec, p->d_ppart, p->d_pdot, p->d_pqs, p->d_pcnv,
-                    p->d_pitb, p->d_pdone, p->d_pact, p->d_off16, p->d_ld16, p->d_pflist, p->d_pfnext};
+                    p->d_pitb, p->d_pdone, p->d_pact, p->d_off16, p->d_ld16, p->d_pflist, p->d_pfnext, p->d_pfin};
     for (void* b : bufs)
         if (b) {
             const hipError_t e = hipFree(b);
@@ -886,9 +930,11 @@
                    (op.debug_stop == 0 || op.debug_stop == 1) && op.sub_split >= -1 && op.sub_split <= 2 &&
                    op.sub_grid_lead >= 0 && op.sub_grid_rest >= 0 && op.shard_copies >= 0 &&
                    op.shard_copies <= 64 && op.h2f_iter >= 0 && op.h2f_iter <= 2 && op.solver >= 0 &&
-                   op.solver <= 2 && op.pcg_tol >= 0.0 && op.pcg_maxit >= 0, "bad dbslmm_options");
+                   op.solver <= 2 && op.pcg_tol >= 0.0 && op.pcg_maxit >= 0 && op.stream_out >= -1 &&
+                   op.stream_out <= 1, "bad dbslmm_options");
     p->solver = op.solver;
     p->pcg_fused = op.pcg_whole >= 0;
+    p->stream_out = op.stream_out >= 0;
     if (op.pcg_tol > 0.0) p->pcg_tol = std::max(1e-15, op.pcg_tol);
     if (op.pcg_maxit > 0) p->pcg_maxit = op.pcg_maxit;
     p->pcg_g16 = 4 * static_cast<int64_t>(pr->n_ref) <= 65535;
@@ -1064,6 +1110,7 @@
     p->h_ld = ldv;
     p->h_blk_id = blk_id;
     p->h_matoff = matoff;
+    (void)build_out_ranges(pr->num_block, pr->s_ptr, has_l ? pr->l_ptr : nullptr, p->h_orange);
     std::vector<int32_t> order(p->n_nonempty);
     std::iota(order.begin(), order.end(), 0);
     std::stable_sort(order.begin(), order.end(), [&](int a, int c) { return mv[a] > mv[c]; });
@@ -1827,7 +1874,7 @@
                                                hipHostMallocDefault));
     if (p->pcg_n == n) return DBSLMM_OK;
     void* old[] = {p->d_pblk, p->d_pitem, p->d_prow, p->d_pvec, p->d_ppart, p->d_pdot, p->d_pqs, p->d_pcnv,
-                   p->d_pitb, p->d_pdone, p->d_pact, p->d_pflist};
+                   p->d_pitb, p->d_pdone, p->d_pact, p->d_pflist, p->d_pfin};
     HIP_TRY(ctx, hipStreamSynchronize(ctx->stream));
     for (void* q : old)
         if (q) (void)hipFree(q);
@@ -1886,6 +1933,12 @@
         p->h_pnseq[f.x] += 1;
     }
     p->n_pflist = static_cast<int32_t>(flist.size());
+    p->h_pfpairs.clear();
+    for (const int2& f : flist)
+        for (int c = f.y < 0 ? 0 : f.y; c < (f.y < 0 ? n : f.y + 1); ++c) p->h_pfpairs.push_back(int2{f.x, c});
+    for (int b = 0; b < static_cast<int>(blk.size()); ++b)
+        if (!blk[b].fused)
+            for (int c = 0; c < n; ++c) p->h_pfpairs.push_back(int2{b, c});
     if (!flist.empty()) HIP_TRY(ctx, dev_upload(&p->d_pflist, flist, ctx->stream));
     if (!flist.empty() && !p->d_pfnext) HIP_TRY(ctx, hipMalloc(&p->d_pfnext, 16));
     p->n_pblk = static_cast<int32_t>(blk.size());
@@ -1905,6 +1958,7 @@
     HIP_TRY(ctx, hipMalloc(&p->d_pitb, std::max<int32_t>(1, p->n_pblk) * sizeof(int32_t)));
     HIP_TRY(ctx, hipMalloc(&p->d_pdone, std::max<int32_t>(1, p->n_pblk) * sizeof(int32_t)));
     HIP_TRY(ctx, hipMalloc(&p->d_pact, sizeof(int32_t)));
+    HIP_TRY(ctx, hipMalloc(&p->d_pfin, std::max<int32_t>(1, p->n_pblk) * sizeof(int32_t)));
     p->pcg_n = n;
     return DBSLMM_OK;
 }
@@ -1946,12 +2000,13 @@
     HIP_TRY(ctx, hipMemcpyAsync(p->h_pmon, p->d_pact, sizeof(int32_t), hipMemcpyDeviceToHost, s));
     HIP_TRY(ctx, hipMemcpyAsync(p->h_pmon + 1, p->d_pitb, p->n_pblk * sizeof(int32_t), hipMemcpyDeviceToHost, s));
     if (p->pcg_ev_end) HIP_TRY(ctx, hipEventRecord(p->pcg_ev_end, s));
-    return DBSLMM_OK;
-}
-
-static int pcg_finish(dbslmm_plan* p) {
+    if (p->so_active) HIP_TRY(ctx, hipEventRecord(p->so_ev, s));
+    return DBSLMM_OK;
+}
+
+static int pcg_check(dbslmm_plan* p) {
     dbslmm_ctx* ctx = p->ctx;
-    while (p->pcg_pending) {
+    if (p->pcg_pending) {
         HIP_TRY(ctx, hipSetDevice(ctx->device));
         HIP_TRY(ctx, hipStreamSynchronize(ctx->stream));
         int32_t need = 0;
@@ -1987,11 +2042,46 @@
                     p->pcg_pbytes += it * p->h_ppart[b];
                 }
             }
-            break;
+            return DBSLMM_OK;
         }
         const int K = std::min(std::max(4, p->pcg_it / 4), p->pcg_maxit - p->pcg_it);
         if (const int rc = pcg_iters(p, K)) return rc;
     }
+    return DBSLMM_OK;
+}
+
+static int pcg_finish(dbslmm_plan* p) {
+    while (p->pcg_pending)
+        if (const int rc = pcg_check(p)) return rc;
+    return DBSLMM_OK;
+}
+
+static int so_prepare(dbslmm_plan* p, int n) {
+    dbslmm_ctx* ctx = p->ctx;
+    const unsigned fl = hipHostMallocMapped | hipHostMallocCoherent;
+    const size_t bytes = static_cast<size_t>(n) * (p->n_s + p->n_l) * sizeof(double) +
+                         static_cast<size_t>(n) * p->nbk * sizeof(int32_t);
+    if (bytes > p->h_mir_bytes) {
+        if (p->h_mir) HIP_TRY(ctx, hipHostFree(p->h_mir));
+        p->h_mir = nullptr;
+        p->h_mir_bytes = 0;
+        HIP_TRY(ctx, hipHostMalloc(&p->h_mir, bytes, fl));
+        p->h_mir_bytes = bytes;
+    }
+    const size_t nf = static_cast<size_t>(std::max(1, p->n_nonempty)) * pcg::kMaxNC;
+    if (!p->h_mflag) {
+        HIP_TRY(ctx, hipHostMalloc(reinterpret_cast<void**>(&p->h_mflag), nf * sizeof(int32_t), fl));
+        memset(p->h_mflag, 0, nf * sizeof(int32_t));
+        p->so_done.assign(nf, 0);
+    }
+    if (!p->so_ev) HIP_TRY(ctx, hipEventCreateWithFlags(&p->so_ev, hipEventDisableTiming));
+    if (p->so_run == INT32_MAX) {
+        memset(p->h_mflag, 0, nf * sizeof(int32_t));
+        p->so_done.assign(nf, 0);
+        p->so_run = 0;
+    }
+    p->so_run++;
+    p->so_n = n;
     return DBSLMM_OK;
 }
 
@@ -2017,6 +2107,9 @@
         if (e != hipSuccess) fprintf(stderr, "run_pcg: error after pcg_layout: %s\n", hipGetErrorString(e));
     }
 #endif
+    p->so_active = p->so_want && p->stream_out;
+    if (p->so_active)
+        if (const int rc = so_prepare(p, n)) return rc;
     hipStream_t s = ctx->stream;
     hipEvent_t* ev = nullptr;
     if (p->timing) {
@@ -2096,9 +2189,20 @@
     a.itb = p->d_pitb;
     a.done = p->d_pdone;
     a.active = p->d_pact;
+    a.fin = p->d_pfin;
     a.beta_s = p->d_beta_s;
     a.beta_l = p->d_beta_l;
     a.status = p->d_status;
+    if (p->so_active) {
+        void *dm = nullptr, *df = nullptr;
+        HIP_TRY(ctx, hipHostGetDevicePointer(&dm, p->h_mir, 0));
+        HIP_TRY(ctx, hipHostGetDevicePointer(&df, p->h_mflag, 0));
+        a.mir_s = static_cast<double*>(dm);
+        a.mir_l = a.mir_s + static_cast<int64_t>(n) * p->n_s;
+        a.mir_st = reinterpret_cast<int32_t*>(a.mir_l + static_cast<int64_t>(n) * p->n_l);
+        a.mir_flag = static_cast<int32_t*>(df);
+        a.run_no = p->so_run;
+    }
     a.vstride = p->pcg_vstride;
     a.ns = p->n_s;
     a.nl = p->n_l;
@@ -2485,6 +2589,72 @@
     return DBSLMM_OK;
 }
 
+static int stream_results(dbslmm_plan* p, double* beta_s, double* beta_l, int32_t* block_status) {
+    dbslmm_ctx* ctx = p->ctx;
+    const int n = p->so_n;
+    const int32_t run = p->so_run;
+    const double* ms = static_cast<const double*>(p->h_mir);
+    const double* ml = ms + static_cast<int64_t>(n) * p->n_s;
+    const int32_t* mst = reinterpret_cast<const int32_t*>(ml + static_cast<int64_t>(n) * p->n_l);
+    if (!p->num_block) block_status = nullptr;
+    auto copy_out = [&](int b, int c) {
+        const OutRange& r = p->h_orange[b];
+        if (beta_s && r.s1 > r.s0)
+            memcpy(beta_s + c * p->n_s + r.s0, ms + c * p->n_s + r.s0, (r.s1 - r.s0) * sizeof(double));
+        if (beta_l && r.l1 > r.l0)
+            memcpy(beta_l + c * p->n_l + r.l0, ml + c * p->n_l + r.l0, (r.l1 - r.l0) * sizeof(double));
+        if (block_status) block_status[static_cast<int64_t>(c) * p->num_block + r.blk] = mst[c * p->nbk + r.blk];
+        p->so_done[static_cast<size_t>(b) * n + c] = run;
+    };
+    const std::vector<int2>& pairs = p->h_pfpairs;
+    size_t head = 0;
+    bool polled = false;
+    while (p->pcg_pending) {
+        for (;;) {
+            const hipError_t q = hipEventQuery(p->so_ev);
+            if (q == hipSuccess) break;
+            if (q != hipErrorNotReady) HIP_TRY(ctx, q);
+            polled = true;
+            for (size_t e = head; e < pairs.size(); ++e) {
+                const size_t f = static_cast<size_t>(pairs[e].x) * n + pairs[e].y;
+                if (p->so_done[f] != run && __atomic_load_n(p->h_mflag + f, __ATOMIC_ACQUIRE) == run)
+                    copy_out(pairs[e].x, pairs[e].y);
+            }
+            while (head < pairs.size() && p->so_done[static_cast<size_t>(pairs[head].x) * n + pairs[head].y] == run)
+                ++head;
+        }
+        if (const int rc = pcg_check(p)) return rc;
+    }
+    if (polled) (void)hipGetLastError();
+    HIP_TRY(ctx, hipStreamSynchronize(ctx->stream));
+    if (const int rc = check_trsv(p)) return rc;
+    std::vector<CopySeg> rest;
+    for (int c = 0; c < n; ++c)
+        for (int b = 0; b < p->n_pblk;) {
+            if (p->so_done[static_cast<size_t>(b) * n + c] == run) { ++b; continue; }
+            int e = b;
+            while (e + 1 < p->n_pblk && p->so_done[static_cast<size_t>(e + 1) * n + c] != run) ++e;
+            const OutRange &r0 = p->h_orange[b], &r1 = p->h_orange[e];
+            if (beta_s && r1.s1 > r0.s0)
+                rest.push_back({beta_s + c * p->n_s + r0.s0, ms + c * p->n_s + r0.s0, (r1.s1 - r0.s0) * sizeof(double)});
+            if (beta_l && r1.l1 > r0.l0)
+                rest.push_back({beta_l + c * p->n_l + r0.l0, ml + c * p->n_l + r0.l0, (r1.l1 - r0.l0) * sizeof(double)});
+            for (int k = b; k <= e; ++k) {
+                const int32_t id = p->h_orange[k].blk;
+                if (block_status) block_status[static_cast<int64_t>(c) * p->num_block + id] = mst[c * p->nbk + id];
+                p->so_done[static_cast<size_t>(k) * n + c] = run;
+            }
+            b = e + 1;
+        }
+    par_memcpy_list(rest);
+    for (int c = 0; c < n && block_status; ++c)
+        for (int32_t b : p->h_empty) block_status[static_cast<int64_t>(c) * p->num_block + b] = DBSLMM_BLOCK_EMPTY;
+    if (p->timing) return collect_timing(p);
+    p->runs_pending = 0;
+    p->run_route.clear();
+    return DBSLMM_OK;
+}
+
 static int download_copy(dbslmm_plan* p, int c, double* beta_s, double* beta_l, int32_t* block_status) {
     return download_copies(p, c, 1, beta_s, beta_l, block_status);
 }
@@ -2512,7 +2682,10 @@
     }
     ARG_CHECK(ctx, static_cast<int64_t>(p->n_nonempty) * n_sigma < 32768,
               "blocks x sigmas must stay below 32768 (packed work items)");
+    p->so_want = true;
     int rc = run_impl(p, true, sigmas, n_sigma);
+    p->so_want = false;
+    if (!rc && p->pcg_ran && p->so_active) return stream_results(p, beta_s, beta_l, block_status);
     if (!rc) rc = dbslmm_plan_sync(p);
     if (!rc) rc = download_copies(p, 0, n_sigma, beta_s, beta_l, block_status);
     return rc;
@@ -2570,6 +2743,19 @@
     std::fill(iters, iters + p->num_block, 0);
     if (!p->pcg_ran) return DBSLMM_OK;
     for (int b = 0; b < p->n_pblk; ++b) iters[p->h_blk_id[b]] = p->h_pmon[1 + b];
+    return DBSLMM_OK;
+}
+
+int dbslmm_out_ranges(int32_t num_block, const int64_t* s_ptr, const int64_t* l_ptr, int64_t* ranges,
+                      int32_t* n_ranges) {
+    if (num_block < 0 || !s_ptr || !ranges || !n_ranges) return DBSLMM_E_ARG;
+    std::vector<OutRange> t;
+    if (!build_out_ranges(num_block, s_ptr, l_ptr, t)) return DBSLMM_E_ARG;
+    for (size_t i = 0; i < t.size(); ++i) {
+        const int64_t row[5] = {t[i].blk, t[i].s0, t[i].s1, t[i].l0, t[i].l1};
+        std::copy(row, row + 5, ranges + 5 * i);
+    }
+    *n_ranges = static_cast<int32_t>(t.size());
     return DBSLMM_OK;
 }
 
diff --git a/include/dbslmm_hip.h b/include/dbslmm_hip.h
--- a/include/dbslmm_hip.h
+++ b/include/dbslmm_hip.h
@@ -7,7 +7,7 @@
 extern "C" {
 #endif
 
-#define DBSLMM_ABI_VERSION 16
+#define DBSLMM_ABI_VERSION 17
 
 enum {
     DBSLMM_OK = 0,
@@ -47,6 +47,7 @@
     double pcg_tol;
     int32_t pcg_maxit;
     int32_t pcg_whole;
+    int32_t stream_out;
 } dbslmm_options;
 
 typedef struct dbslmm_problem {
@@ -116,6 +117,9 @@
 int dbslmm_plan_workload(const dbslmm_plan* plan, double* out );
 int dbslmm_plan_block_iters(dbslmm_plan* plan, int32_t* iters);
 
+int dbslmm_out_ranges(int32_t num_block, const int64_t* s_ptr, const int64_t* l_ptr, int64_t* ranges,
+                      int32_t* n_ranges);
+
 int dbslmm_plan_block_matrix(dbslmm_plan* plan, int32_t block, int32_t copy, double* out,
                              int32_t* ld_out);
 
```
